# aaron-randreth/modulation-mfcc

Measured on AMD Instinct MI355X. Metric: MFCC+mod-spectrum frames/sec, higher is better.
Workload: dtype f32; 1 GPU; BASELINE configs[2] per GPU: 1024 clips x 10 s x 16000 Hz, win 400 hop 160 n_fft 512, 40 mel (fmax 8000), 13 MFCC + modulation spectrum (rFFT 1024 over trajectories); frames_per_clip=1001, clips_total=1024, parallelism=clips sharded x1, hsa_ipc_mode_legacy=0, settle_calls=712, full=False, fused_tail=True

## Files before the change

include/modmfcc.h:

```cpp
#ifndef MODMFCC_H
#define MODMFCC_H

#include <stddef.h>
#include <stdint.h>

#ifdef __cplusplus
extern "C" {
#endif

#define MM_VERSION 123

typedef enum mm_status {
  MM_OK = 0,
  MM_ERR_INVALID_ARG = -1,
  MM_ERR_UNSUPPORTED = -2,
  MM_ERR_HIP = -3,
  MM_ERR_WORKSPACE = -4,
  MM_ERR_ALLOC = -5
} mm_status;

typedef struct mm_config {
  double sr;
  int32_t n_fft;
  int32_t win_length;
  int32_t hop_length;
  int32_t n_mels;
  int32_t n_mfcc;
  double fmin;
  double fmax;
  float preemph;
  float top_db;
  float amin;
  int32_t center;
  int32_t n_mod_fft;
} mm_config;

typedef struct mm_plan mm_plan;

enum {
  MM_STAGE_LOGMEL = 0,
  MM_STAGE_DCT = 1,
  MM_STAGE_MODSPEC = 2,
  MM_STAGE_RFFT = 3,
  MM_STAGE_POWER = 4,
  MM_STAGE_CHANGE = 5,
  MM_STAGE_INIT = 6,
  MM_NUM_STAGES = 8
};

int mm_version(void);
const char* mm_strerror(int status);
const char* mm_last_hip_error(void);

int mm_config_default(mm_config* cfg);
int mm_config_validate(const mm_config* cfg);
int64_t mm_num_frames(const mm_config* cfg, int64_t n_samples);
int32_t mm_num_bins(const mm_config* cfg);
int32_t mm_mod_fft_len(const mm_config* cfg, int64_t n_frames);
int mm_build_window(const mm_config* cfg, float* out );
int mm_build_mel(const mm_config* cfg, float* out );
int mm_build_dct(const mm_config* cfg, float* out );
int mm_build_mel_sweep(const mm_config* cfg, int n_waves, float* wlo ,
                       float* whi , int32_t* d , int32_t* part );
int mm_build_mel_runs(const mm_config* cfg, int n_waves, int32_t* hdr, int32_t hdr_cap, float* grp,
                      int32_t grp_cap, int32_t* part, int32_t* counts);
int mm_build_butter_sos(int order, double wn, double* sos );

int mm_plan_create(const mm_config* cfg, mm_plan** out);
int mm_plan_destroy(mm_plan* plan);
int mm_plan_config(const mm_plan* plan, mm_config* out);
int mm_plan_kernel_path(const mm_plan* plan);
int mm_plan_fused_dct(const mm_plan* plan);
int mm_plan_set_fuse_dct(mm_plan* plan, int on);
int mm_plan_fused_tail(const mm_plan* plan, int64_t batch, int64_t n_samples);
int mm_plan_set_fuse_tail(mm_plan* plan, int on);
int mm_plan_force_generic(mm_plan* plan, int on);
int mm_plan_set_variant(mm_plan* plan, int variant);
size_t mm_workspace_bytes(const mm_plan* plan, int64_t batch, int64_t n_samples);

int mm_mfcc_f32(mm_plan* plan, const float* d_audio, int64_t batch, int64_t n_samples,
                int64_t audio_stride, float* d_mfcc, void* d_workspace, size_t ws_bytes,
                void* stream);

int mm_logmel_f32(mm_plan* plan, const float* d_audio, int64_t batch, int64_t n_samples,
                  int64_t audio_stride, float* d_logmel, float* d_clipmax, void* stream);

int mm_stft_power_f32(mm_plan* plan, const float* d_audio, int64_t batch, int64_t n_samples,
                      int64_t audio_stride, float* d_power, void* stream);

int mm_rfft_f32(mm_plan* plan, const float* d_in, int64_t rows, int64_t in_len,
                int64_t in_stride, int32_t n, float* d_out, void* stream);

int mm_modspec_f32(mm_plan* plan, const float* d_mfcc, int64_t batch, int64_t n_frames,
                   float* d_modspec, void* stream);

int mm_mfcc_modspec_f32(mm_plan* plan, const float* d_audio, int64_t batch, int64_t n_samples,
                        int64_t audio_stride, float* d_mfcc, float* d_modspec, void* d_workspace,
                        size_t workspace_bytes, void* stream);

size_t mm_ragged_workspace_bytes(const mm_plan* plan, int64_t batch, int64_t n_samples);
int mm_mfcc_ragged_f32(mm_plan* plan, const float* d_audio, int64_t batch, int64_t n_samples, int64_t audio_stride,
                       const int64_t* d_lengths, float* d_mfcc, float* d_modspec, void* d_workspace, size_t ws_bytes,
                       void* stream);

int mm_mfcc_change_f64(mm_plan* plan, const float* d_mfcc, int64_t batch, int64_t n_frames,
                       int32_t remove_first, int32_t diff_method, const double* sos1, int32_t n_sec1,
                       const double* sos2, int32_t n_sec2, double* d_change,
                       void* d_workspace, size_t ws_bytes, void* stream);
size_t mm_change_workspace_bytes(const mm_plan* plan, int64_t batch, int64_t n_frames);
size_t mm_change_workspace_bytes_for(const mm_plan* plan, int64_t batch, int64_t n_frames, int32_t remove_first,
                                     const double* sos1, int32_t n_sec1, const double* sos2, int32_t n_sec2);

size_t mm_change_ragged_workspace_bytes_for(const mm_plan* plan, int64_t batch, int64_t n_frames_max, int32_t remove_first,
                                            const double* sos1, int32_t n_sec1, const double* sos2, int32_t n_sec2);
int mm_mfcc_change_ragged_f64(mm_plan* plan, const float* d_mfcc, int64_t batch, int64_t n_frames_max,
                              const int64_t* d_frames, int32_t remove_first, int32_t diff_method,
                              const double* sos1, int32_t n_sec1, const double* sos2, int32_t n_sec2,
                              double* d_change, void* d_workspace, size_t ws_bytes, void* stream);

int mm_sosfiltfilt_f64(const double* d_x, int64_t rows, int64_t n, int64_t x_stride, const double* sos,
                       int32_t n_sec, double* d_y, void* d_workspace, size_t ws_bytes, void* stream);
size_t mm_sosfiltfilt_workspace_bytes(int64_t rows, int64_t n);
int mm_sosfiltfilt_f32_f64(const float* d_x, int64_t rows, int64_t n, int64_t x_stride, const double* sos,
                           int32_t n_sec, double* d_y, void* d_workspace, size_t ws_bytes, void* stream);

#define MM_ST_MAXW 16
#define MM_ST_MAXE 8
typedef struct mm_stencil {
  int32_t n_c, n_edge, edge_w, reserved;
  int32_t off[MM_ST_MAXW];
  double c[MM_ST_MAXW];
  double el[MM_ST_MAXE][MM_ST_MAXW];
  double er[MM_ST_MAXE][MM_ST_MAXW];
  double den_c, den_e;
} mm_stencil;
int mm_stencil_f64(const mm_stencil* st, const double* d_x, int64_t rows, int64_t n, int64_t x_stride,
                   double* d_y, void* stream);

int mm_fir_filtfilt_f64(const double* d_x, int64_t rows, int64_t n, int64_t x_stride, const double* d_h, int32_t n_taps,
                        double* d_y, int64_t y_stride, void* stream);
int mm_fir_filtfilt_f32_f64(const float* d_x, int64_t rows, int64_t n, int64_t x_stride, const double* d_h, int32_t n_taps,
                            double* d_y, int64_t y_stride, void* stream);
int mm_savgol_f64(const double* d_x, int64_t rows, int64_t n, int64_t x_stride, const double* d_c, const double* d_q,
                  const double* d_p, int32_t window, int32_t n_basis, double* d_y, int64_t y_stride, void* stream);

size_t mm_sosfiltfilt_ragged_workspace_bytes(int64_t rows, int64_t n_max);
int mm_sosfiltfilt_ragged_f64(const double* d_x, int64_t rows, int64_t n_max, int64_t x_stride, const int64_t* d_lens,
                              const double* sos, int32_t n_sec, double* d_y, void* d_workspace, size_t ws_bytes,
                              void* stream);
int mm_sosfiltfilt_ragged_f32_f64(const float* d_x, int64_t rows, int64_t n_max, int64_t x_stride, const int64_t* d_lens,
                                  const double* sos, int32_t n_sec, double* d_y, void* d_workspace, size_t ws_bytes,
                                  void* stream);
int mm_stencil_ragged_f64(const mm_stencil* st, const double* d_x, int64_t rows, int64_t n_max, int64_t x_stride,
                          const int64_t* d_lens, double* d_y, void* stream);
int mm_fir_filtfilt_ragged_f64(const double* d_x, int64_t rows, int64_t n_max, int64_t x_stride, const int64_t* d_lens,
                               const double* d_h, int32_t n_taps, double* d_y, int64_t y_stride, void* stream);
int mm_fir_filtfilt_ragged_f32_f64(const float* d_x, int64_t rows, int64_t n_max, int64_t x_stride, const int64_t* d_lens,
                                   const double* d_h, int32_t n_taps, double* d_y, int64_t y_stride, void* stream);
int mm_savgol_ragged_f64(const double* d_x, int64_t rows, int64_t n_max, int64_t x_stride, const int64_t* d_lens,
                         const double* d_c, const double* d_q, const double* d_p, int32_t window, int32_t n_basis,
                         double* d_y, int64_t y_stride, void* stream);

int64_t mm_rms_num_frames(int64_t n_samples, int32_t frame_length, int32_t hop_length, int32_t center);
int mm_rms_f32(const float* d_audio, int64_t batch, int64_t n_samples, int64_t audio_stride,
               int32_t frame_length, int32_t hop_length, int32_t center, float* d_rms, void* stream);
int mm_rms_ragged_f32(const float* d_audio, int64_t batch, int64_t n_max, int64_t audio_stride, const int64_t* d_lens,
                      int32_t frame_length, int32_t hop_length, int32_t center, float* d_rms, void* stream);

typedef struct mm_hilbert mm_hilbert;
int mm_hilbert_create(int64_t n, int32_t dtype, mm_hilbert** out);
void mm_hilbert_destroy(mm_hilbert* h);
int64_t mm_hilbert_fft_size(const mm_hilbert* h);
size_t mm_hilbert_workspace_bytes(const mm_hilbert* h, int64_t rows);
int mm_hilbert_envelope(mm_hilbert* h, const void* d_x, int64_t rows, int64_t x_stride, void* d_env,
                        int64_t env_stride, void* d_workspace, size_t ws_bytes, void* stream);
int mm_hilbert_ragged_create(int64_t n_max, int32_t dtype, mm_hilbert** out);
size_t mm_hilbert_ragged_workspace_bytes(const mm_hilbert* h, int64_t rows, int64_t n_max);
int mm_hilbert_envelope_ragged(mm_hilbert* h, const void* d_x, int64_t rows, int64_t n_max, int64_t x_stride,
                               const int64_t* d_lens, void* d_env, int64_t env_stride, void* d_workspace, size_t ws_bytes,
                               void* stream);
size_t mm_hilbert_rfft_workspace_bytes(const mm_hilbert* h, int64_t rows);
int mm_hilbert_rfft_f32(mm_hilbert* h, const float* d_x, int64_t rows, int64_t x_stride, int64_t n_valid, float* d_out,
                        void* d_ws, size_t ws_bytes, void* stream);

int mm_pcm_decode_f32(const void* d_raw, int32_t fmt, int32_t channels, int64_t n_frames, float* d_out,
                      int64_t out_stride, void* stream);
int mm_resample_f32(const float* d_x, int64_t rows, int64_t n_in, int64_t x_stride, const float* d_taps,
                    int32_t L, int32_t M, int32_t taps_per_phase, int64_t half_len, float* d_y, int64_t n_out,
                    void* stream);
int mm_resample_banded_f32(const float* d_x, int64_t rows, int64_t n_in, int64_t x_stride, const float* d_atab,
                           const int32_t* d_lo_off, int32_t F, int32_t S, int32_t NB, int32_t ksteps, int32_t lo_min,
                           int32_t win, float* d_y, int64_t n_out, void* stream);
int mm_resample_banded_shape(int32_t F, int32_t S, int32_t NB, int32_t ksteps, int32_t win, int32_t* qt, int32_t* pad,
                             size_t* lds_bytes);

typedef struct mm_wav_rec {
  int64_t byte_offset;
  int64_t n_frames;
  int32_t fmt;
  int32_t channels;
  int64_t first_row;
} mm_wav_rec;
int mm_pcm_decode_ragged_f32(const void* d_raw, int64_t raw_bytes, const mm_wav_rec* d_recs, int64_t n_files,
                             int64_t max_frames, float* d_out, int64_t out_rows, int64_t out_stride, void* stream);
int mm_resample_ragged_f32(const float* d_x, int64_t rows, int64_t n_max, int64_t x_stride, const int64_t* d_lens,
                           const float* d_taps, int32_t L, int32_t M, int32_t taps_per_phase, int64_t half_len,
                           float* d_y, int64_t n_out_max, int64_t y_stride, void* stream);
int mm_resample_banded_ragged_f32(const float* d_x, int64_t rows, int64_t n_max, int64_t x_stride, const int64_t* d_lens,
                                  const float* d_atab, const int32_t* d_lo_off, int32_t F, int32_t S, int32_t NB,
                                  int32_t ksteps, int32_t lo_min, int32_t win, float* d_y, int64_t n_out_max,
                                  int64_t y_stride, void* stream);

int mm_devcopy_f32(const float* d_src, float* d_dst, int64_t n_floats, void* stream);

typedef struct mm_pyin_params {
  double sr, fmin, fmax;
  double no_trough_prob;
  double log_tiny;
  double fill_na;
  double log_p_init[2];
  int32_t frame_length, win_length, hop_length;
  int32_t center;
  int32_t min_period, max_period, n_thresholds, nbps;
  int32_t n_bins, band_h, max_troughs, reserved;
} mm_pyin_params;

typedef struct mm_pyin_tables {
  const double* thresholds;
// ... 96 lines not shown
```

modulation_mfcc_amd/_lib.py:

```python
from __future__ import annotations

import ctypes as C
import os

_HERE = os.path.dirname(os.path.abspath(__file__))
LIB_PATH = os.environ.get("MODMFCC_LIB") or os.path.join(_HERE, "libmodmfcc.so")

MM_OK = 0
MM_ERR_INVALID_ARG = -1
MM_ERR_UNSUPPORTED = -2
MM_ERR_HIP = -3
MM_ERR_WORKSPACE = -4
MM_ERR_ALLOC = -5

STAGES = ("logmel", "dct", "modspec", "rfft", "power", "change", "init", "reserved")
MM_NUM_STAGES = 8


class mm_config(C.Structure):
    _fields_ = [
        ("sr", C.c_double),
        ("n_fft", C.c_int32),
        ("win_length", C.c_int32),
        ("hop_length", C.c_int32),
        ("n_mels", C.c_int32),
        ("n_mfcc", C.c_int32),
        ("fmin", C.c_double),
        ("fmax", C.c_double),
        ("preemph", C.c_float),
        ("top_db", C.c_float),
        ("amin", C.c_float),
        ("center", C.c_int32),
        ("n_mod_fft", C.c_int32),
    ]


MM_ST_MAXW, MM_ST_MAXE = 16, 8


class mm_stencil(C.Structure):
    _fields_ = [
        ("n_c", C.c_int32), ("n_edge", C.c_int32), ("edge_w", C.c_int32), ("reserved", C.c_int32),
        ("off", C.c_int32 * MM_ST_MAXW),
        ("c", C.c_double * MM_ST_MAXW),
        ("el", (C.c_double * MM_ST_MAXW) * MM_ST_MAXE),
        ("er", (C.c_double * MM_ST_MAXW) * MM_ST_MAXE),
        ("den_c", C.c_double), ("den_e", C.c_double),
    ]


class mm_pyin_params(C.Structure):
    _fields_ = [
        ("sr", C.c_double), ("fmin", C.c_double), ("fmax", C.c_double),
        ("no_trough_prob", C.c_double), ("log_tiny", C.c_double), ("fill_na", C.c_double),
        ("log_p_init", C.c_double * 2),
        ("frame_length", C.c_int32), ("win_length", C.c_int32), ("hop_length", C.c_int32), ("center", C.c_int32),
        ("min_period", C.c_int32), ("max_period", C.c_int32), ("n_thresholds", C.c_int32), ("nbps", C.c_int32),
        ("n_bins", C.c_int32), ("band_h", C.c_int32), ("max_troughs", C.c_int32), ("reserved", C.c_int32),
    ]


class mm_pyin_tables(C.Structure):
    _fields_ = [(k, C.c_void_p) for k in ("thresholds", "beta_probs", "beta_cum", "boltzmann", "log_same", "log_cross",
                                           "freqs")]


class mm_peaks_opts(C.Structure):
    _fields_ = [
        ("height", C.c_double * 2), ("threshold", C.c_double * 2), ("prominence", C.c_double * 2),
        ("negate", C.c_int32), ("use_height", C.c_int32), ("use_threshold", C.c_int32), ("use_prominence", C.c_int32),
    ]


class mm_peaks_ext(C.Structure):
    _fields_ = [
        ("plateau_size", C.c_double * 2), ("width", C.c_double * 2), ("rel_height", C.c_double),
        ("distance", C.c_int32), ("wlen", C.c_int32), ("use_plateau_size", C.c_int32), ("use_distance", C.c_int32),
        ("use_width", C.c_int32),
    ]


class mm_peaks_out(C.Structure):
    _fields_ = [(k, C.c_void_p) for k in ("count", "idx", "prom", "lbase", "rbase", "widths", "width_heights", "left_ips",
                                           "right_ips", "plateau_sizes", "left_edges", "right_edges")]


MM_MAX_SEC = 16
MM_RAGGED_MAX_SEC = 4


class MMError(RuntimeError):
    def __init__(self, status, what, detail=""):
        self.status = status
        super().__init__(f"{what}: {detail}" if detail else what)


_vp = C.c_void_p
_i64 = C.c_int64
_cfgp = C.POINTER(mm_config)
_pyp = C.POINTER(mm_pyin_params)
_pyt = C.POINTER(mm_pyin_tables)

PROTOTYPES = {
    "mm_version": (C.c_int, []),
    "mm_strerror": (C.c_char_p, [C.c_int]),
    "mm_last_hip_error": (C.c_char_p, []),
    "mm_config_default": (C.c_int, [_cfgp]),
    "mm_config_validate": (C.c_int, [_cfgp]),
    "mm_num_frames": (_i64, [_cfgp, _i64]),
    "mm_num_bins": (C.c_int32, [_cfgp]),
    "mm_mod_fft_len": (C.c_int32, [_cfgp, _i64]),
    "mm_build_window": (C.c_int, [_cfgp, _vp]),
    "mm_build_mel": (C.c_int, [_cfgp, _vp]),
    "mm_build_dct": (C.c_int, [_cfgp, _vp]),
    "mm_build_mel_sweep": (C.c_int, [_cfgp, C.c_int, _vp, _vp, _vp, _vp]),
    "mm_build_mel_runs": (C.c_int, [_cfgp, C.c_int, _vp, C.c_int32, _vp, C.c_int32, _vp, _vp]),
    "mm_build_butter_sos": (C.c_int, [C.c_int, C.c_double, _vp]),
    "mm_plan_create": (C.c_int, [_cfgp, C.POINTER(_vp)]),
    "mm_plan_destroy": (C.c_int, [_vp]),
    "mm_plan_config": (C.c_int, [_vp, _cfgp]),
    "mm_plan_kernel_path": (C.c_int, [_vp]),
    "mm_plan_fused_dct": (C.c_int, [_vp]),
    "mm_plan_set_fuse_dct": (C.c_int, [_vp, C.c_int]),
    "mm_plan_fused_tail": (C.c_int, [_vp, _i64, _i64]),
    "mm_plan_set_fuse_tail": (C.c_int, [_vp, C.c_int]),
    "mm_mfcc_modspec_f32": (C.c_int, [_vp, _vp, _i64, _i64, _i64, _vp, _vp, _vp, C.c_size_t, _vp]),
    "mm_plan_force_generic": (C.c_int, [_vp, C.c_int]),
    "mm_plan_set_variant": (C.c_int, [_vp, C.c_int]),
    "mm_workspace_bytes": (C.c_size_t, [_vp, _i64, _i64]),
    "mm_mfcc_f32": (C.c_int, [_vp, _vp, _i64, _i64, _i64, _vp, _vp, C.c_size_t, _vp]),
    "mm_logmel_f32": (C.c_int, [_vp, _vp, _i64, _i64, _i64, _vp, _vp, _vp]),
    "mm_stft_power_f32": (C.c_int, [_vp, _vp, _i64, _i64, _i64, _vp, _vp]),
    "mm_rfft_f32": (C.c_int, [_vp, _vp, _i64, _i64, _i64, C.c_int32, _vp, _vp]),
    "mm_modspec_f32": (C.c_int, [_vp, _vp, _i64, _i64, _vp, _vp]),
    "mm_ragged_workspace_bytes": (C.c_size_t, [_vp, _i64, _i64]),
    "mm_mfcc_ragged_f32": (C.c_int, [_vp, _vp, _i64, _i64, _i64, _vp, _vp, _vp, _vp, C.c_size_t, _vp]),
    "mm_mfcc_change_f64": (C.c_int, [_vp, _vp, _i64, _i64, C.c_int32, C.c_int32, _vp, C.c_int32, _vp,
                                     C.c_int32, _vp, _vp, C.c_size_t, _vp]),
    "mm_sosfiltfilt_f64": (C.c_int, [_vp, _i64, _i64, _i64, _vp, C.c_int32, _vp, _vp, C.c_size_t, _vp]),
    "mm_sosfiltfilt_workspace_bytes": (C.c_size_t, [_i64, _i64]),
    "mm_sosfiltfilt_f32_f64": (C.c_int, [_vp, _i64, _i64, _i64, _vp, C.c_int32, _vp, _vp, C.c_size_t, _vp]),
    "mm_stencil_f64": (C.c_int, [C.POINTER(mm_stencil), _vp, _i64, _i64, _i64, _vp, _vp]),
    "mm_fir_filtfilt_f64": (C.c_int, [_vp, _i64, _i64, _i64, _vp, C.c_int32, _vp, _i64, _vp]),
    "mm_fir_filtfilt_f32_f64": (C.c_int, [_vp, _i64, _i64, _i64, _vp, C.c_int32, _vp, _i64, _vp]),
    "mm_savgol_f64": (C.c_int, [_vp, _i64, _i64, _i64, _vp, _vp, _vp, C.c_int32, C.c_int32, _vp, _i64, _vp]),
    "mm_sosfiltfilt_ragged_workspace_bytes": (C.c_size_t, [_i64, _i64]),
    "mm_sosfiltfilt_ragged_f64": (C.c_int, [_vp, _i64, _i64, _i64, _vp, _vp, C.c_int32, _vp, _vp, C.c_size_t, _vp]),
    "mm_sosfiltfilt_ragged_f32_f64": (C.c_int, [_vp, _i64, _i64, _i64, _vp, _vp, C.c_int32, _vp, _vp, C.c_size_t, _vp]),
    "mm_stencil_ragged_f64": (C.c_int, [C.POINTER(mm_stencil), _vp, _i64, _i64, _i64, _vp, _vp, _vp]),
    "mm_fir_filtfilt_ragged_f64": (C.c_int, [_vp, _i64, _i64, _i64, _vp, _vp, C.c_int32, _vp, _i64, _vp]),
    "mm_fir_filtfilt_ragged_f32_f64": (C.c_int, [_vp, _i64, _i64, _i64, _vp, _vp, C.c_int32, _vp, _i64, _vp]),
    "mm_savgol_ragged_f64": (C.c_int, [_vp, _i64, _i64, _i64, _vp, _vp, _vp, _vp, C.c_int32, C.c_int32, _vp, _i64, _vp]),
    "mm_change_workspace_bytes": (C.c_size_t, [_vp, _i64, _i64]),
    "mm_change_workspace_bytes_for": (C.c_size_t, [_vp, _i64, _i64, C.c_int32, _vp, C.c_int32, _vp, C.c_int32]),
    "mm_change_ragged_workspace_bytes_for": (C.c_size_t, [_vp, _i64, _i64, C.c_int32, _vp, C.c_int32, _vp, C.c_int32]),
    "mm_mfcc_change_ragged_f64": (C.c_int, [_vp, _vp, _i64, _i64, _vp, C.c_int32, C.c_int32, _vp, C.c_int32, _vp,
                                            C.c_int32, _vp, _vp, C.c_size_t, _vp]),
    "mm_rms_num_frames": (_i64, [_i64, C.c_int32, C.c_int32, C.c_int32]),
    "mm_rms_f32": (C.c_int, [_vp, _i64, _i64, _i64, C.c_int32, C.c_int32, C.c_int32, _vp, _vp]),
    "mm_rms_ragged_f32": (C.c_int, [_vp, _i64, _i64, _i64, _vp, C.c_int32, C.c_int32, C.c_int32, _vp, _vp]),
    "mm_hilbert_ragged_create": (C.c_int, [_i64, C.c_int32, C.POINTER(_vp)]),
    "mm_hilbert_ragged_workspace_bytes": (C.c_size_t, [_vp, _i64, _i64]),
    "mm_hilbert_envelope_ragged": (C.c_int, [_vp, _vp, _i64, _i64, _i64, _vp, _vp, _i64, _vp, C.c_size_t, _vp]),
    "mm_hilbert_create": (C.c_int, [_i64, C.c_int32, C.POINTER(_vp)]),
    "mm_hilbert_destroy": (None, [_vp]),
    "mm_hilbert_fft_size": (_i64, [_vp]),
    "mm_hilbert_workspace_bytes": (C.c_size_t, [_vp, _i64]),
    "mm_hilbert_envelope": (C.c_int, [_vp, _vp, _i64, _i64, _vp, _i64, _vp, C.c_size_t, _vp]),
    "mm_hilbert_rfft_workspace_bytes": (C.c_size_t, [_vp, _i64]),
    "mm_hilbert_rfft_f32": (C.c_int, [_vp, _vp, _i64, _i64, _i64, _vp, _vp, C.c_size_t, _vp]),
    "mm_pcm_decode_f32": (C.c_int, [_vp, C.c_int32, C.c_int32, _i64, _vp, _i64, _vp]),
    "mm_resample_f32": (C.c_int, [_vp, _i64, _i64, _i64, _vp, C.c_int32, C.c_int32, C.c_int32, _i64, _vp, _i64, _vp]),
    "mm_resample_banded_f32": (C.c_int, [_vp, _i64, _i64, _i64, _vp, _vp, C.c_int32, C.c_int32, C.c_int32, C.c_int32, C.c_int32,
                                        C.c_int32, _vp, _i64, _vp]),
    "mm_resample_banded_shape": (C.c_int, [C.c_int32, C.c_int32, C.c_int32, C.c_int32, C.c_int32, C.POINTER(C.c_int32),
                                          C.POINTER(C.c_int32), C.POINTER(C.c_size_t)]),
    "mm_pcm_decode_ragged_f32": (C.c_int, [_vp, _i64, _vp, _i64, _i64, _vp, _i64, _i64, _vp]),
    "mm_resample_ragged_f32": (C.c_int, [_vp, _i64, _i64, _i64, _vp, _vp, C.c_int32, C.c_int32, C.c_int32, _i64, _vp, _i64,
                                        _i64, _vp]),
    "mm_resample_banded_ragged_f32": (C.c_int, [_vp, _i64, _i64, _i64, _vp, _vp, _vp, C.c_int32, C.c_int32, C.c_int32, C.c_int32,
                                               C.c_int32, C.c_int32, _vp, _i64, _i64, _vp]),
    "mm_devcopy_f32": (C.c_int, [_vp, _vp, _i64, _vp]),
    "mm_pyin_check": (C.c_int, [_pyp]),
    "mm_pyin_num_frames": (_i64, [_pyp, _i64]),
    "mm_pyin_cmnd": (C.c_int, [_pyp, _vp, C.c_int32, _i64, _i64, _i64, _vp, _vp]),
    "mm_pyin_candidates": (C.c_int, [_pyp, _pyt, _vp, _i64, _vp, _vp, _vp, _vp, _vp]),
    "mm_pyin_decode_workspace_bytes": (C.c_size_t, [_pyp, _i64, _i64]),
    "mm_pyin_decode": (C.c_int, [_pyp, _pyt, _vp, _vp, _vp, _vp, _i64, _i64, _vp, _vp, _vp, _vp, C.c_size_t, _vp]),
    "mm_pyin_workspace_bytes": (C.c_size_t, [_pyp, _i64, _i64]),
    "mm_pyin_f32": (C.c_int, [_pyp, _pyt, _vp, _i64, _i64, _i64, _vp, _vp, _vp, _vp, _vp, C.c_size_t, _vp]),
    "mm_pyin_f64": (C.c_int, [_pyp, _pyt, _vp, _i64, _i64, _i64, _vp, _vp, _vp, _vp, _vp, C.c_size_t, _vp]),
    "mm_pyin_ragged_workspace_bytes": (C.c_size_t, [_pyp, _i64, _i64]),
    "mm_pyin_ragged_f32": (C.c_int, [_pyp, _pyt, _vp, _i64, _i64, _i64, _vp, _vp, _vp, _vp, _vp, _vp, _vp, C.c_size_t, _vp]),
    "mm_pyin_ragged_f64": (C.c_int, [_pyp, _pyt, _vp, _i64, _i64, _i64, _vp, _vp, _vp, _vp, _vp, _vp, _vp, C.c_size_t, _vp]),
    "mm_interp_nan_linear_ragged_f64": (C.c_int, [_vp, _i64, _i64, _i64, _vp, _vp, _i64, _vp]),
    "mm_interp_nan_ragged_f64": (C.c_int, [C.c_int32, _vp, _i64, _i64, _i64, _vp, _vp, _i64, _vp, C.c_size_t, _vp]),
    "mm_interp_nan_linear_f64": (C.c_int, [_vp, _i64, _i64, _i64, _vp, _i64, _vp]),
    "mm_interp_nan_workspace_bytes": (C.c_size_t, [C.c_int32, _i64, _i64]),
    "mm_interp_nan_f64": (C.c_int, [C.c_int32, _vp, _i64, _i64, _i64, _vp, _i64, _vp, C.c_size_t, _vp]),
    "mm_regrid_linear_f32_f64": (C.c_int, [_vp, _i64, _i64, _i64, _vp, _vp, _i64, _vp, _i64, _vp]),
    "mm_find_peaks_workspace_bytes": (C.c_size_t, [_i64, _i64]),
    "mm_find_peaks": (C.c_int, [C.POINTER(mm_peaks_opts), _vp, C.c_int32, _i64, _i64, _i64, _vp, _vp, _i64, _vp, _vp, _vp,
                                _vp, _vp, _vp, C.c_size_t, _vp]),
    "mm_find_peaks_ex_workspace_bytes": (C.c_size_t, [C.POINTER(mm_peaks_opts), C.POINTER(mm_peaks_ext), _i64, _i64]),
    "mm_find_peaks_ex": (C.c_int, [C.POINTER(mm_peaks_opts), C.POINTER(mm_peaks_ext), _vp, C.c_int32, _i64, _i64, _i64, _vp,
                                   _vp, _i64, C.POINTER(mm_peaks_out), _vp, C.c_size_t, _vp]),
    "mm_timing_enable": (C.c_int, [_vp, C.c_int]),
    "mm_timing_read": (C.c_int, [_vp, _vp, _vp]),
}


class mm_modpsd_params(C.Structure):
    _fields_ = [
        ("fs", C.c_double),
        ("nperseg", C.c_int32), ("noverlap", C.c_int32), ("nfft", C.c_int32),
        ("detrend", C.c_int32), ("scaling", C.c_int32), ("reserved", C.c_int32 * 3),
    ]


_mpp = C.POINTER(mm_modpsd_params)

PROTOTYPES_MODPSD = {
    "mm_modpsd_version": (C.c_int, []),
    "mm_modpsd_check": (C.c_int, [_mpp]),
    "mm_modpsd_num_segments": (_i64, [_mpp, _i64]),
    "mm_modpsd_create": (C.c_int, [_mpp, _vp, C.POINTER(_vp)]),
    "mm_modpsd_destroy": (None, [_vp]),
    "mm_modpsd_workspace_bytes": (C.c_size_t, [_vp, _i64, _i64]),
    "mm_modpsd_f32": (C.c_int, [_vp, _vp, _i64, _i64, _i64, _vp, _vp, _i64, _vp, C.c_size_t, _vp]),
}

PROTOTYPES_MODCSD = {
    "mm_modcsd_version": (C.c_int, []),
    "mm_modcsd_check": (C.c_int, [_mpp]),
    "mm_modcsd_workspace_bytes": (C.c_size_t, [_vp, _i64, _i64]),
    "mm_modcsd_f32": (C.c_int, [_vp, _vp, _i64, _i64, _i64, _vp, _i64, _i64, _vp, _vp, _vp, _vp, _vp, _i64, _vp, C.c_size_t,
                                _vp]),
}

MM_SPLINE_QUADRATIC, MM_SPLINE_CUBIC = 2, 3
PROTOTYPES_SPLINE = {
    "mm_interp_spline_workspace_bytes": (C.c_size_t, [C.c_int32, _i64, _i64]),
    "mm_interp_spline_f64": (C.c_int, [C.c_int32, _vp, _i64, _i64, _i64, _vp, _i64, _vp, C.c_size_t, _vp]),
    "mm_interp_spline_ragged_f64": (C.c_int, [C.c_int32, _vp, _i64, _i64, _i64, _vp, _vp, _i64, _vp, C.c_size_t, _vp]),
}

MM_LOMB_PRECENTER, MM_LOMB_FLOATING_MEAN = 1, 2
MM_LOMB_POWER, MM_LOMB_NORMALIZE, MM_LOMB_AMPLITUDE = 0 << 2, 1 << 2, 2 << 2
MM_LOMB_CHUNK = 512
PROTOTYPES_LOMB = {
    "mm_lomb_version": (C.c_int, []),
    "mm_lombscargle_workspace_bytes": (C.c_size_t, [_i64, _i64, _i64]),
    "mm_lombscargle_f64": (C.c_int, [_vp, _i64, _i64, _i64, _vp, _vp, _vp, _i64, C.c_int32, _vp, _i64, _vp, _vp, C.c_size_t,
                                     _vp]),
}

_lib = None


def load():
    global _lib
    if _lib is not None:
        return _lib
    try:
        import torch
    except ImportError:
        pass
    if not os.path.exists(LIB_PATH):
        raise ImportError(
            f"{LIB_PATH} is missing: the HIP extension has not been built. Run "
            "`make -C modulation_mfcc_amd/csrc` (needs hipcc, --offload-arch=gfx950). "
            "modulation_mfcc_amd has no CPU fallback.")
    lib = C.CDLL(LIB_PATH)
    for table in (PROTOTYPES, PROTOTYPES_MODPSD, PROTOTYPES_MODCSD, PROTOTYPES_SPLINE, PROTOTYPES_LOMB):
        for name, (res, args) in table.items():
            fn = getattr(lib, name)
            fn.restype = res
# ... 19 lines not shown
```

modulation_mfcc_amd/csrc/mm_api.hip:

```cpp
#include <memory>
#include <utility>

#include "mm_common.h"
#include "mm_plan.h"

thread_local std::string g_hip_err;

struct StftParams {
  const float* audio;
  int64_t batch, n_samples, stride, n_frames;
  int n_fft, log2nc, hop, n_bins, n_mels;
  float preemph, amin, db_offset;
  const float* window;
  const float2* tw;
  const int* mel_start;
  const int* mel_len;
  const int* mel_off;
  const float* mel_w;
  float* out_power;
  float* out_logmel;
  int* clip_key;
  int frames_per_wave;
};

// ... 113 lines not shown
    const int64_t r = r0 + f;
    if (r >= p.rows) break;
    const float* a = p.in + r * p.in_stride;
    for (int n = lane; n < nc; n += 64) {
      const float x0 = (2 * n < p.in_len) ? a[2 * n] : 0.0f;
      const float x1 = (2 * n + 1 < p.in_len) ? a[2 * n + 1] : 0.0f;
      z[__brev((unsigned)n) >> (32 - p.log2nc)] = make_float2(x0, x1);
    }
    wave_lds_sync();
    wave_cfft_lds(z, p.log2nc, p.tw, lane);
    float2* o = reinterpret_cast<float2*>(p.out) + r * (nc + 1);
    for (int k = lane; k <= (nc >> 1); k += 64) {
      float2 xa, xb;
      real_split(z, k, nc, p.tw, tw_stride, xa, xb);
      o[k] = xa;
      o[nc - k] = xb;
    }
    wave_lds_sync();
  }
}

#include "mm_fft16.hip.inc"
#include "mm_logmel16w.hip.inc"
#include "mm_s16.h"
#include "mm_logmel12m.hip.inc"
#include "mm_logmel16h.hip.inc"
#include "mm_wpf.hip.inc"
#include "mm_hb_math.h"
#include "mm_anyfft.hip.inc"


template <class... K>
static bool raise_lds(int bytes, K... kernels) {
  for (const void* k : {(const void*)kernels...})
    if (hipFuncSetAttribute(k, hipFuncAttributeMaxDynamicSharedMemorySize, bytes) != hipSuccess) return false;
  return true;
}

using WpfKernel = void (*)(WpfParams);
template <int R, int Z>
static WpfKernel wpf_ni_kernel(int pairs) {
  return pairs == 4 ? logmel_wpf_kernel<R, 1, false, false, Z, 4> : pairs == 5 ? logmel_wpf_kernel<R, 1, false, false, Z, 5>
       : pairs == 6 ? logmel_wpf_kernel<R, 1, false, false, Z, 6> : logmel_wpf_kernel<R, 1, false, false, Z, 7>;
}
template <int R>
static WpfKernel wpf_kernel(int mode, bool pre, bool w16, bool half, int z, int pairs) {
  if constexpr (R >= 2) {
    if (w16) return logmel_wpf_kernel<R, 1, false, true>;
    if (half) return z ? wpf_ni_kernel<R, 3>(pairs) : wpf_ni_kernel<R, 0>(pairs);
    if (z) return z == 7 ? logmel_wpf_kernel<R, 1, false, false, 7> : z == 6 ? logmel_wpf_kernel<R, 1, false, false, 6>
                : z == 5 ? logmel_wpf_kernel<R, 1, false, false, 5> : logmel_wpf_kernel<R, 1, false, false, 3>;
  }
  if (mode == 0) return pre ? logmel_wpf_kernel<R, 0, true> : logmel_wpf_kernel<R, 0, false>;
  return pre ? logmel_wpf_kernel<R, 1, true> : logmel_wpf_kernel<R, 1, false>;
}

extern "C" {

int mm_version(void) { return MM_VERSION; }

const char* mm_strerror(int s) {
  switch (s) {
    case MM_OK: return "ok";
    case MM_ERR_INVALID_ARG: return "invalid argument";
    case MM_ERR_UNSUPPORTED: return "unsupported configuration";
    case MM_ERR_HIP: return "HIP runtime error";
    case MM_ERR_WORKSPACE: return "workspace too small";
    case MM_ERR_ALLOC: return "allocation failed";
    default: return "unknown status";
  }
}

const char* mm_last_hip_error(void) { return g_hip_err.c_str(); }

int mm_config_default(mm_config* c) {
  if (!c) return MM_ERR_INVALID_ARG;
  c->sr = 10000.0;
  c->n_fft = 512;
  c->win_length = 250;
  c->hop_length = 50;
  c->n_mels = 128;
  c->n_mfcc = 13;
  c->fmin = 100.0;
  c->fmax = 10000.0;
  c->preemph = 0.0f;
  c->top_db = 80.0f;
  c->amin = 1e-10f;
  c->center = 1;
  c->n_mod_fft = 0;
  return MM_OK;
}

int mm_config_validate(const mm_config* c) { return mm::validate(c); }

int64_t mm_num_frames(const mm_config* c, int64_t n_samples) {
  if (!c || c->hop_length < 1 || n_samples < 0) return MM_ERR_INVALID_ARG;
  const int64_t padded = n_samples + 2 * (int64_t)(c->n_fft / 2);
  return padded < c->n_fft ? 0 : 1 + (padded - c->n_fft) / c->hop_length;
}

int32_t mm_num_bins(const mm_config* c) { return c ? c->n_fft / 2 + 1 : MM_ERR_INVALID_ARG; }

int32_t mm_mod_fft_len(const mm_config* c, int64_t n_frames) {
  if (!c || n_frames < 1) return MM_ERR_INVALID_ARG;
  if (c->n_mod_fft) return c->n_mod_fft >= n_frames ? c->n_mod_fft : MM_ERR_INVALID_ARG;
  int64_t n = 32;
  while (n < n_frames) n *= 2;
  return n <= ((int64_t)1 << 24) ? (int32_t)n : MM_ERR_UNSUPPORTED;
}

int mm_build_window(const mm_config* c, float* out) {
  int s = mm::validate(c);
  if (s || !out) return s ? s : MM_ERR_INVALID_ARG;
  mm::build_window(*c, out);
  return MM_OK;
}
int mm_build_mel(const mm_config* c, float* out) {
  int s = mm::validate(c);
  if (s || !out) return s ? s : MM_ERR_INVALID_ARG;
  mm::build_mel(*c, out);
  return MM_OK;
}
int mm_build_dct(const mm_config* c, float* out) {
  int s = mm::validate(c);
  if (s || !out) return s ? s : MM_ERR_INVALID_ARG;
  mm::build_dct(*c, out);
  return MM_OK;
}
int mm_build_mel_sweep(const mm_config* c, int n_waves, float* wlo, float* whi, int32_t* d, int32_t* part) {
  int s = mm::validate(c);
  if (s) return s;
  if (n_waves < 1 || !wlo || !whi || !d || !part) return MM_ERR_INVALID_ARG;
  std::vector<float> mel((size_t)c->n_mels * (c->n_fft / 2 + 1));
  mm::build_mel(*c, mel.data());
  mm::MelSweep sw;
  if (!mm::build_mel_sweep(*c, mel.data(), n_waves, &sw)) return MM_ERR_UNSUPPORTED;
  std::memcpy(wlo, sw.wlo.data(), sw.wlo.size() * 4);
  std::memcpy(whi, sw.whi.data(), sw.whi.size() * 4);
  std::memcpy(d, sw.d.data(), sw.d.size() * 4);
  std::memcpy(part, sw.part.data(), sw.part.size() * 4);
  return MM_OK;
}
int mm_build_mel_runs(const mm_config* c, int n_waves, int32_t* hdr, int32_t hdr_cap, float* grp,
                      int32_t grp_cap, int32_t* part, int32_t* counts) {
  int s = mm::validate(c);
  if (s) return s;
  if (n_waves < 1 || !hdr || !grp || !part || !counts) return MM_ERR_INVALID_ARG;
  std::vector<float> mel((size_t)c->n_mels * (c->n_fft / 2 + 1));
  mm::build_mel(*c, mel.data());
  mm::MelSweep sw;
  if (!mm::build_mel_sweep(*c, mel.data(), n_waves, &sw)) return MM_ERR_UNSUPPORTED;
  mm::MelRuns r;
  mm::build_mel_runs(*c, sw, n_waves, &r);
  counts[0] = (int32_t)(r.hdr.size() / 4);
  counts[1] = (int32_t)(r.grp.size() / 8);
  if (counts[0] > hdr_cap || counts[1] > grp_cap) return MM_ERR_WORKSPACE;
  std::memcpy(hdr, r.hdr.data(), r.hdr.size() * 4);
  std::memcpy(grp, r.grp.data(), r.grp.size() * 4);
  std::memcpy(part, r.part.data(), r.part.size() * 4);
  return MM_OK;
}
int mm_build_butter_sos(int order, double wn, double* sos) { return mm::build_butter_sos(order, wn, sos); }


static std::vector<float> packed_run_table(const mm::MelRuns& r) {
  std::vector<float> tab(r.hdr.size() + r.grp.size());
  std::memcpy(tab.data(), r.hdr.data(), r.hdr.size() * 4);
  std::memcpy(tab.data() + r.hdr.size(), r.grp.data(), r.grp.size() * 4);
  for (size_t g = 0; g < r.grp.size() / 8; ++g) {
    float* q = tab.data() + r.hdr.size() + 8 * g;
    const float t[8] = {q[0], q[4], q[1], q[5], q[2], q[6], q[3], q[7]};
    std::memcpy(q, t, sizeof t);
  }
  return tab;
}

static std::vector<int> balance_parts_over_simds(const mm::MelRuns& r, const double* extra = nullptr,
                                                 std::vector<int>* wave_of_part = nullptr) {
  const int n = (int)(r.part.size() / 4);
  std::vector<int> out(r.part.size());
  if (wave_of_part) { wave_of_part->assign(n, 0); for (int w = 0; w < n; ++w) (*wave_of_part)[w] = w; }
  if (n != 16) return r.part;
  std::vector<std::pair<double, int>> cost(n);
  for (int w = 0; w < n; ++w) {
    double c = extra ? extra[w] : 0.0;
    for (int i = r.part[w * 4 + 0]; i < r.part[w * 4 + 1]; ++i) c += 58.0 + 8.5 * r.hdr[4 * i + 1];
    cost[w] = {c, w};
  }
  std::sort(cost.begin(), cost.end(), [](const std::pair<double, int>& a, const std::pair<double, int>& b) {
    return a.first > b.first || (a.first == b.first && a.second < b.second); });
  double load[4] = {0, 0, 0, 0};
  int cnt[4] = {0, 0, 0, 0};
  for (int i = 0; i < n; ++i) {
    int best = -1;
    for (int sd = 0; sd < 4; ++sd)
      if (cnt[sd] < 4 && (best < 0 || load[sd] < load[best])) best = sd;
    const int wave = best + 4 * cnt[best];
    std::memcpy(&out[wave * 4], &r.part[cost[i].second * 4], 16);
    if (wave_of_part) (*wave_of_part)[cost[i].second] = wave;
    load[best] += cost[i].first; ++cnt[best];
  }
  return out;
}

static std::vector<float> wpf_lane_table(int R, const float* win, const float* tw) {
  const int L = 16 * R, NC = 256 * R;
  std::vector<float> lt((size_t)L * MM_WPF_LT_PITCH, 0.0f);
  for (int l = 0; l < L; ++l) {
    float* r = lt.data() + l * MM_WPF_LT_PITCH;
    const int pq = l % R;
    if (win)
      for (int n1 = 0; n1 < 16; ++n1) { r[2 * n1] = win[2 * L * n1 + 2 * l]; r[2 * n1 + 1] = win[2 * L * n1 + 2 * l + 1]; }
    for (int k1 = 1; k1 < 16; ++k1) {
      const int i1 = ((l * k1) % NC) * (MM_TW_N / NC);
      r[32 + 2 * (k1 - 1)] = tw[2 * i1]; r[32 + 2 * (k1 - 1) + 1] = tw[2 * i1 + 1];
      const int i2 = ((pq * k1) % L) * (MM_TW_N / L);
      r[64 + 2 * (k1 - 1)] = tw[2 * i2]; r[64 + 2 * (k1 - 1) + 1] = tw[2 * i2 + 1];
    }
    for (int i = 0; i < 8; ++i) {
      const int idx = (l + L * i) * (MM_TW_N / (2 * NC));
      r[96 + 2 * i] = 0.5f * tw[2 * idx + 1]; r[96 + 2 * i + 1] = -0.5f * tw[2 * idx];
    }
  }
  return lt;
}

static std::vector<float> w16_lane_table(const float* win, const float* tw) {
  std::vector<float> lt(16 * MM_W16_LT_PITCH, 0.0f);
  for (int q = 0; q < 16; ++q) {
    float* r = lt.data() + q * MM_W16_LT_PITCH;
    for (int n1 = 0; n1 < 16; ++n1) { r[2 * n1] = win[32 * n1 + 2 * q]; r[2 * n1 + 1] = win[32 * n1 + 2 * q + 1]; }
    for (int k1 = 1; k1 < 16; ++k1) {
      const int idx = (q * k1) * (MM_TW_N / 256);
      r[32 + 2 * (k1 - 1)] = tw[2 * idx]; r[32 + 2 * (k1 - 1) + 1] = tw[2 * idx + 1];
    }
    for (int j = 0; j < 8; ++j) {
      const int idx = (q + 16 * j) * (MM_TW_N / 512);
      r[64 + 2 * j] = 0.5f * tw[2 * idx + 1]; r[64 + 2 * j + 1] = -0.5f * tw[2 * idx];
    }
  }
  return lt;
}

static int zero_edges(const float* win, int n) {
  int e = 0;
  while (e < n / 2 && win[e] == 0.0f && win[n - 1 - e] == 0.0f) ++e;
  return e;
}

struct EmptyFilters { std::vector<char> empty; bool skip = false; int nk = 0; };
static EmptyFilters empty_filters(const mm_config& c, const float* mel) {
  EmptyFilters e;
  e.empty.assign(c.n_mels, 1);
  int n_empty = 0;
  for (int m = 0; m < c.n_mels; ++m) {
    for (int k = 0; k < 257 && e.empty[m]; ++k) if (mel[(size_t)m * 257 + k] != 0.0f) e.empty[m] = 0;
    n_empty += e.empty[m];
  }
  e.skip = n_empty > 0 && n_empty < c.n_mels;
  int last = c.n_mels - 1;
  while (e.skip && last > 0 && e.empty[last]) --last;
  e.nk = e.skip ? last / 4 + 1 : ((c.n_mels + 3) & ~3) / 4;
  return e;
}

static std::vector<float> dct_a_operands(const mm_config& c, const float* dct, int nk, const char* skip = nullptr) {
  const int kbn = (c.n_mfcc + 15) / 16;
  std::vector<float> a((size_t)kbn * nk * 64, 0.0f);
  for (int kb = 0; kb < kbn; ++kb)
    for (int s = 0; s < nk; ++s)
      for (int l = 0; l < 64; ++l) {
        const int k = 16 * kb + (l & 15), m = 4 * s + (l >> 4);
        if (k < c.n_mfcc && m < c.n_mels && !(skip && skip[m])) a[((size_t)kb * nk + s) * 64 + l] = dct[(size_t)k * c.n_mels + m];
      }
  return a;
}

static bool wpf_mel_lanes(const mm::MelSweep& sw, int R, int SL, std::vector<float>* out, int* group_max) {
  const int L = 16 * R, NC = 256 * R;
  std::vector<float>& ml = *out;
  ml.assign((size_t)L * 36, 0.0f);
  std::vector<int> d_end(L, -2);
  bool ok = true;
  for (int l = 0; l < L && ok; ++l) {
    float* r = ml.data() + l * 36;
    int dprev = sw.d[SL * l];
    const int dstart = dprev;
    unsigned bits = 0;
    const int nslots = SL == 8 ? 8 : ((l == L - 1) ? 17 : 16);
    for (int i = 0; i < nslots; ++i) {
      const int k = (i < SL) ? SL * l + i : NC;
      const int adv = sw.d[k] - dprev;
      if (adv < 0 || adv > 1) { ok = false; break; }
      if (adv == 1) bits |= (1u << i);
      dprev = sw.d[k];
      r[i] = sw.wlo[k];
      r[17 + i] = sw.whi[k];
    }
    std::memcpy(&r[34], &dstart, 4);
    std::memcpy(&r[35], &bits, 4);
    d_end[l] = dprev;
  }
  std::vector<char> act(L, 0);
  for (int l = 0; l < L; ++l) {
    const float* r = ml.data() + (size_t)l * 36;
    unsigned bits;
// ... 34 lines not shown
  PlanHost(const mm_config& c, int n_bins, int kp)
      : win(c.n_fft), mel((size_t)c.n_mels * n_bins), dct((size_t)c.n_mfcc * c.n_mels),
        dct_t((size_t)c.n_mels * kp, 0.0f), tw(2 * MM_TW_N), cfg_e(c), ce(&c), melp(mel.data()), winp(win.data()) {
    mm::build_window(c, win.data()); mm::build_mel(c, mel.data());
    mm::build_dct(c, dct.data()); mm::build_twiddles(MM_TW_N, tw.data());
    for (int k = 0; k < c.n_mfcc; ++k)
      for (int m = 0; m < c.n_mels; ++m) dct_t[(size_t)m * kp + k] = dct[(size_t)k * c.n_mels + m];
    mm::build_mel_csr(c, mel.data(), &csr);
  }
  PlanHost(const PlanHost&) = delete;
};

static int setup_base(mm_plan* p, const PlanHost& h) {
  mm_plan::Base& b = p->base;
  int rc = MM_OK;
  if ((rc = p->upload(&b.d_window, h.win.data(), h.win.size() * 4)) ||
      (rc = p->upload(&b.d_tw, h.tw.data(), h.tw.size() * 4)) ||
      (rc = p->upload(&b.d_mel_start, h.csr.start.data(), h.csr.start.size() * 4)) ||
      (rc = p->upload(&b.d_mel_len, h.csr.len.data(), h.csr.len.size() * 4)) ||
      (rc = p->upload(&b.d_mel_off, h.csr.off.data(), h.csr.off.size() * 4)) ||
      (rc = p->upload(&b.d_mel_w, h.csr.w.data(), h.csr.w.size() * 4)) ||
      (rc = p->upload(&b.d_dct_t, h.dct_t.data(), h.dct_t.size() * 4)))
    return rc;
  hipDeviceProp_t prop;
  if (hipGetDeviceProperties(&prop, p->device) == hipSuccess && prop.multiProcessorCount > 0)
    p->num_cus = prop.multiProcessorCount;
  return MM_OK;
}

static int setup_any(mm_plan* p, const PlanHost& h) {
  AnyPlan& ap = p->any;
  std::vector<float> atw, asplit, achirp, abhat;
  if (!any_plan_host(p->cfg.n_fft, &ap, &atw, &asplit, &achirp, &abhat, MM_LM_LDS_MAX)) return MM_ERR_UNSUPPORTED;
  int rc = MM_OK;
  if ((rc = p->upload(&ap.d_tw, atw.data(), std::max<size_t>(atw.size(), 2) * 4)) ||
      (!asplit.empty() && (rc = p->upload(&ap.d_split, asplit.data(), asplit.size() * 4))) ||
      (!achirp.empty() && (rc = p->upload(&ap.d_chirp, achirp.data(), achirp.size() * 4))) ||
      (!abhat.empty() && (rc = p->upload(&ap.d_bhat, abhat.data(), abhat.size() * 4))))
    return rc;
  std::vector<float> pack(h.win.begin(), h.win.end());
  auto put = [&](const void* src, size_t n_floats) {
    const int off = (int)pack.size();
    pack.resize(pack.size() + ((n_floats + 3) & ~(size_t)3), 0.0f);
    if (n_floats) std::memcpy(pack.data() + off, src, n_floats * 4);
    return off;
  };
  ap.o_tw = put(atw.data(), atw.size());
  ap.o_split = put(asplit.data(), asplit.size());
  ap.o_chirp = put(achirp.data(), achirp.size());
  ap.o_melw = put(h.csr.w.data(), h.csr.w.size());
  ap.o_mstart = put(h.csr.start.data(), h.csr.start.size());
  ap.o_mlen = put(h.csr.len.data(), h.csr.len.size());
  ap.o_moff = put(h.csr.off.data(), h.csr.off.size());
  ap.tab_floats = (int)pack.size();
  const size_t G = 256 / ap.tpf, budget = ap.tpf == 64 ? 65536 : MM_LM_LDS_MAX;
  ap.lds_tab = ap.M == 0 && G * ap.grp_bytes + pack.size() * 4 <= budget;
  int r1 = 0, r2 = 0;
  if (ap.packed && ap.M == 0 && reg2_pick(ap.nn, &r1, &r2) && reg2_lds_bytes(r1, r2, ap.tab_floats) <= 80 * 1024 &&
      reg2_set_attr(r1, r2, MM_LM_LDS_MAX)) { ap.reg2 = r1; ap.reg2_r2 = r2; }
  if ((ap.lds_tab || ap.reg2) && (rc = p->upload(&ap.d_tabpack, pack.data(), pack.size() * 4))) return rc;
  if (ap.lds_tab && ap.tpf == 64 && ap.packed && ap.M == 0 && ap.nn <= 256) {
    const int fb = 2;
    const size_t per_wave = (size_t)2 * fb * ap.nn * 8;
    if ((size_t)fb * (ap.nn + 2) * 4 <= (size_t)fb * ap.nn * 8 && 4 * per_wave + pack.size() * 4 <= 80 * 1024) {
      ap.fb = fb; ap.fb_grp_bytes = (unsigned)per_wave;
    }
  }
  if (!raise_lds(MM_LM_LDS_MAX, stft_any_kernel<0, 64, false>, stft_any_kernel<1, 64, false>, stft_any_kernel<0, 256, false>,
                 stft_any_kernel<1, 256, false>, stft_any_kernel<0, 64, true>, stft_any_kernel<1, 64, true>,
                 stft_any_kernel<0, 256, true>, stft_any_kernel<1, 256, true>)) {
    g_hip_err = "hipFuncSetAttribute(stft_any_kernel) failed";
    return MM_ERR_HIP;
  }
  if (!raise_lds(MM_LM_LDS_MAX, stft_anyb_kernel<0>, stft_anyb_kernel<1>)) ap.fb = 0;
  ap.ok = true;
  return MM_OK;
}

static void setup_embed(mm_plan* p, PlanHost& h) {
  const mm_config& c = p->cfg;
  if (c.n_fft != 256 && c.n_fft != 128 && c.n_fft != 64) return;
  const int E = 512 / c.n_fft;
  h.cfg_e.n_fft = 512;
  h.win_e.resize(512);
  mm::build_window(h.cfg_e, h.win_e.data());
  h.mel_e.assign((size_t)c.n_mels * 257, 0.0f);
  for (int m = 0; m < c.n_mels; ++m)
    for (int k = 0; k < p->n_bins; ++k) h.mel_e[(size_t)m * 257 + (size_t)E * k] = h.mel[(size_t)m * p->n_bins + k];
  if (p->upload(&p->embed.d_window, h.win_e.data(), h.win_e.size() * 4) == MM_OK) {
    h.ce = &h.cfg_e; h.melp = h.mel_e.data(); h.winp = h.win_e.data(); p->embed.factor = E;
  }
}

static void setup_s16f(mm_plan* p, const PlanHost& h, size_t tab16_bytes) {
  const mm_config& c = *h.ce;
  const EmptyFilters ef = empty_filters(c, h.melp);
  const int lt_rows = (c.n_mels + 3) & ~3, kbn = (c.n_mfcc + 15) / 16, nk = ef.nk;
  std::vector<float> dcta = dct_a_operands(c, h.dct.data(), nk, ef.skip ? ef.empty.data() : nullptr);
  const size_t e_off = dcta.size();
  dcta.resize(e_off + (size_t)kbn * 16 + 8, 0.0f);
  if (ef.skip) {
    for (int k = 0; k < c.n_mfcc; ++k) {
      double e = 0.0;
      for (int m = 0; m < c.n_mels; ++m) if (ef.empty[m]) e += (double)h.dct[(size_t)k * c.n_mels + m];
      dcta[e_off + k] = (float)e;
    }
    unsigned bits[8] = {0};
    for (int m = 0; m < c.n_mels; ++m) if (ef.empty[m]) bits[m >> 5] |= 1u << (m & 31);
    std::memcpy(&dcta[e_off + (size_t)kbn * 16], bits, sizeof(bits));
  }
  for (int layout = 0; layout < 4; ++layout) {
    const bool single = layout >= 2;
    const bool xa = p->s16.xa && (layout & 1) == 0;
    if ((layout & 1) && !p->s16.xa) continue;
    const double wts_d[16] = {1, 1, 1, MM_S16F_W, 1, 1, 1, MM_S16F_W, 1, 1, 1, MM_S16F_W, 1, 1, 1, MM_S16F_W};
    double extra[16];
    for (int w = 0; w < 16; ++w) extra[w] = (!single && wts_d[w] < 1.0) ? 700.0 : 0.0;
    mm::MelSweep swf;
    if (!mm::build_mel_sweep(c, h.melp, 16, &swf, single ? nullptr : wts_d)) return;
    mm::MelRuns rf;
    mm::build_mel_runs(c, swf, 16, &rf);
    if (ef.skip)
      for (size_t r = 0; r < rf.hdr.size() / 4; ++r) {
        const int d = rf.hdr[4 * r + 3];
        if (d >= 0 && d < c.n_mels && ef.empty[d]) rf.hdr[4 * r + 0] |= 1 << 16;
      }
    const std::vector<float> tab = packed_run_table(rf);
    std::vector<int> wave_of_part;
    const std::vector<int> part = balance_parts_over_simds(rf, extra, &wave_of_part);
    unsigned long long roles = ~0ull;
    for (int f = 0; f < 4; ++f) {
      const int w = single ? f : wave_of_part[4 * f + 3];
      roles = (roles & ~(0xFull << (4 * w))) | ((unsigned long long)f << (4 * w));
    }
    const size_t tab_end = (size_t)MM_S16_TAB_OFF(p->s16.nr, xa) + tab.size() * 4;
    const unsigned lt_off = (unsigned)align_up(tab_end, 16);
    const unsigned dcta_off = lt_off + (single ? 1u : 2u) * (unsigned)lt_rows * 320u;
    const unsigned red_off = (unsigned)align_up((size_t)dcta_off + dcta.size() * 4, 16);
    const size_t lds = (size_t)red_off + 2 * 16 * 8;
    if (lds > MM_LM_LDS_MAX) continue;
    mm_plan::S16F& f = p->s16f;
    f.ok = p->upload(&f.d_tab, tab.data(), tab.size() * 4) == MM_OK &&
           p->upload(&f.d_part, part.data(), part.size() * 4) == MM_OK &&
           p->upload(&f.d_dcta, dcta.data(), dcta.size() * 4) == MM_OK;
    if (!f.ok) return;
    f.n_runs = (int)(rf.hdr.size() / 4); f.n_tab16 = (int)(tab.size() / 4);
    f.lt_rows = lt_rows; f.nk = nk; f.kb = kbn; f.roles = roles;
    f.flags = (single ? MM_S16F_SINGLE : 0) | (ef.skip ? MM_S16F_SKIP : 0);
    f.lt_off = lt_off; f.dcta_off = dcta_off; f.red_off = red_off; f.lds_bytes = lds;
    if (!xa && p->s16.xa) {
      p->s16.xa = false;
      p->s16.lds_bytes = (size_t)MM_S16_TAB_OFF(p->s16.nr, false) + tab16_bytes;
    }
    return;
  }
}

static void setup_m12(mm_plan* p, const PlanHost& h) {
  const mm_config& c = p->cfg;
  mm_plan::M12& m = p->m12;
  M12Tables mt;
  const int s_floats = (47 * c.hop_length + 512 + 255) & ~255;
  const int nr = (s_floats / 256 + 15) / 16;
  if (nr > 3 || !build_m12_tables(*h.ce, h.melp, h.dct.data(), &mt)) return;
  m.nb = mt.nb; m.nr = nr; m.s_floats = s_floats;
  m.fused_dct = c.n_mfcc <= 16;
  if (mt.a_tab.empty()) mt.a_tab.assign(128, 0.0f);
  m.win_off = (unsigned)(MM_M12_S_OFF + (size_t)s_floats * 4);
  m.tw_off = m.win_off + 2048u;
  m.a_off = m.tw_off + 16u * MM_M12_TW_PITCH * 4u;
  m.n_a2 = (int)(mt.a_tab.size() / 2);
  m.dct_off = m.a_off + (unsigned)align_up(mt.a_tab.size() * 4, 16);
  m.part_off = m.dct_off + (unsigned)mt.nb * 1024u;
  m.cnt_off = m.part_off + (m.fused_dct ? (unsigned)mt.n_slots * 1024u : 0u);
  m.lds_bytes = (size_t)m.cnt_off + 16;
  const std::vector<float> zeros(64, 0.0f);
  if (m.lds_bytes <= MM_LM_LDS_MAX &&
      p->upload(&m.d_a, mt.a_tab.data(), mt.a_tab.size() * 4) == MM_OK &&
      p->upload(&m.d_dct, mt.dct_tab.data(), mt.dct_tab.size() * 4) == MM_OK &&
      p->upload(&m.d_zeros, zeros.data(), zeros.size() * 4) == MM_OK &&
      set_m12_attr(MM_LM_LDS_MAX)) {
    std::memcpy(m.units, mt.units.data(), sizeof(m.units));
    std::memcpy(m.n_units, mt.n_units.data(), sizeof(m.n_units));
    m.ok = true;
  }
}

static int setup_tile512(mm_plan* p, const PlanHost& h) {
  const mm_config& c = *h.ce;
  if (c.n_fft != 512) return MM_OK;
  p->s16.halfwin = zero_edges(h.winp, 512) >= 128;
  mm::MelSweep sw;
  if (!mm::build_mel_sweep(c, h.melp, 8, &sw)) return MM_OK;
  mm::MelRuns runs;
  mm::build_mel_runs(c, sw, 8, &runs);
  const std::vector<float> tab = packed_run_table(runs);
  mm_plan::W8& w8 = p->w8;
  w8.n_runs = (int)(runs.hdr.size() / 4); w8.n_tab16 = (int)(tab.size() / 4);
  w8.lds_bytes = (size_t)MM_LM_TAB_OFF + tab.size() * 4;
  if (w8.lds_bytes <= MM_LM_LDS_MAX) {
    int rc = MM_OK;
    if ((rc = p->upload(&w8.d_tab, tab.data(), tab.size() * 4)) || (rc = p->upload(&w8.d_part, runs.part.data(), runs.part.size() * 4)))
      return rc;
    w8.ok = raise_lds(MM_LM_LDS_MAX, logmel512_kernel<0>, logmel512_kernel<1>);
  }
  mm::MelSweep sw16;
  if (!w8.ok || !mm::build_mel_sweep(c, h.melp, 16, &sw16)) return MM_OK;
  mm::MelRuns r16;
  mm::build_mel_runs(c, sw16, 16, &r16);
  const std::vector<float> tab16 = packed_run_table(r16);
  const size_t tab16_bytes = tab16.size() * 4;
  mm_plan::W16& w16 = p->w16;
  w16.n_runs = (int)(r16.hdr.size() / 4); w16.n_tab16 = (int)(tab16.size() / 4);
  w16.lds_bytes = (size_t)MM_W16_TAB_OFF + tab16_bytes;
  const std::vector<float> lt = w16_lane_table(h.winp, h.tw.data());
  w16.ok = w16.lds_bytes <= MM_LM_LDS_MAX && p->upload(&w16.d_tab, tab16.data(), tab16_bytes) == MM_OK &&
           p->upload(&w16.d_lane_tab, lt.data(), lt.size() * 4) == MM_OK &&
           p->upload(&w16.d_part, balance_parts_over_simds(r16).data(), r16.part.size() * 4) == MM_OK &&
           raise_lds(MM_LM_LDS_MAX, logmel512w_kernel<0>, logmel512w_kernel<1>);
  if (w16.ok && 31 * c.hop_length + 512 + 256 <= MM_H16_NR * 2048 && (c.hop_length % 2) == 0 && c.preemph == 0.0f) {
    mm_plan::H16& h16 = p->h16;
    H16Tables ht;
    build_h16_tables(r16, &ht);
    h16.n_pairs = ht.n_pairs; h16.n_tab16 = (int)(ht.tab.size() / 4);
    h16.lds_bytes = (size_t)MM_H16_TAB_OFF + ht.tab.size() * 4;
    h16.ok = h16.lds_bytes <= 80 * 1024 && p->upload(&h16.d_tab, ht.tab.data(), ht.tab.size() * 4) == MM_OK &&
             p->upload(&h16.d_part, ht.part.data(), ht.part.size() * 4) == MM_OK && raise_lds(80 * 1024, logmel512h_kernel);
  }
  if (w16.ok) {
    const int span = 63 * c.hop_length + 512;
    int nr = span <= 4096 ? 1 : span <= 2 * 4096 ? 2 : span <= 3 * 4096 ? 3 : (span <= 4 * 4096 ? 4 : 0);
    if (nr && nr < 3 && c.preemph != 0.0f) nr = 3;
    const bool xa = nr >= 3 && (size_t)MM_S16_TAB_OFF(nr, true) + tab16_bytes <= MM_LM_LDS_MAX;
    const size_t lds = nr ? (size_t)MM_S16_TAB_OFF(nr, xa) + tab16_bytes : 0;
    if (nr && lds <= MM_LM_LDS_MAX && set_s16_attr(MM_LM_LDS_MAX)) { p->s16.nr = nr; p->s16.xa = xa; p->s16.lds_bytes = lds; }
  }
  if (p->s16.nr && c.n_mels <= 256) setup_s16f(p, h, tab16_bytes);
  if (p->w16.ok) setup_m12(p, h);
  return MM_OK;
}

static void setup_wpf(mm_plan* p, const PlanHost& h) {
  const mm_config& c = p->cfg;
  if ((c.n_fft != 512 && c.n_fft != 1024 && c.n_fft != 2048) || c.n_mels > MM_WPF_MAXMEL) return;
  const int R = c.n_fft / 512, L = 16 * R, NC = 256 * R;
  mm::MelSweep sw;
  if (!mm::build_mel_sweep(c, h.mel.data(), 1, &sw)) return;
  mm_plan::Wpf& w = p->wpf;
  int k_hi = 0;
  for (int m = 0; m < c.n_mels; ++m)
    for (int k = p->n_bins - 1; k > k_hi; --k)
      if (h.mel[(size_t)m * p->n_bins + k] != 0.0f) { k_hi = k; break; }
  w.half = R >= 2 && k_hi < NC / 2 && c.preemph == 0.0f;
  w.pairs = w.half ? std::max(4, k_hi / L + 1) : 8;
  if (w.pairs > 7) w.half = false;
  std::vector<float> ml;
  bool ok = wpf_mel_lanes(sw, R, w.half ? 8 : 16, &ml, &w.group_max);
  if (!ok && w.half) {
    w.half = false; w.pairs = 8;
    ok = wpf_mel_lanes(sw, R, 16, &ml, &w.group_max);
  }
  const int macc_stride = (c.n_mels + 2 + 63) / 64 * 64;
  const int F = 4 / R;
  const int xbuf = (R == 1) ? 1280 : 1152;
  const int pbuf = F * (NC + NC / 16 + 4);
  const size_t wave_bytes = (size_t)(xbuf + pbuf + F * 3 * macc_stride) * 4;
  w.r = R;
  if (w.half) {
    const size_t wb = (size_t)(xbuf + MM_WPF_PBUF_HALF + F * 3 * macc_stride) * 4;
    int wv = 16;
    while (wv > 4 && (size_t)L * MM_WPF_LT_PITCH * 4 + wv * wb > MM_LM_LDS_MAX) wv -= 4;
    w.waves_half = wv; w.lds_half = (size_t)L * MM_WPF_LT_PITCH * 4 + wv * wb;
  }
  w.waves = 12;
  while (w.waves > 4 && (size_t)L * MM_WPF_LT_PITCH * 4 + w.waves * wave_bytes > MM_LM_LDS_MAX) w.waves -= 4;
  w.lds_bytes = (size_t)L * MM_WPF_LT_PITCH * 4 + w.waves * wave_bytes;
  w.lds16 = (size_t)L * (MM_WPF_LT_PITCH + MM_WPF_ML_PITCH) * 4 + 16 * (size_t)(xbuf + F * 3 * macc_stride) * 4;
  w.w16 = R >= 2 && w.lds16 <= MM_LM_LDS_MAX &&
          raise_lds(MM_LM_LDS_MAX, logmel_wpf_kernel<2, 1, false, true>, logmel_wpf_kernel<4, 1, false, true>);
  bool attr_ok = w.lds_bytes <= MM_LM_LDS_MAX &&
                 raise_lds(MM_LM_LDS_MAX, logmel_wpf_kernel<1, 0, false>, logmel_wpf_kernel<1, 1, false>,
                           logmel_wpf_kernel<2, 0, false>, logmel_wpf_kernel<2, 1, false>, logmel_wpf_kernel<4, 0, false>,
                           logmel_wpf_kernel<4, 1, false>, logmel_wpf_kernel<1, 0, true>, logmel_wpf_kernel<1, 1, true>,
                           logmel_wpf_kernel<2, 0, true>, logmel_wpf_kernel<2, 1, true>, logmel_wpf_kernel<4, 0, true>,
                           logmel_wpf_kernel<4, 1, true>);
  if (w.half &&
      !raise_lds(MM_LM_LDS_MAX, wpf_ni_kernel<4, 0>(4), wpf_ni_kernel<4, 0>(5), wpf_ni_kernel<4, 0>(6), wpf_ni_kernel<4, 0>(7),
                 wpf_ni_kernel<4, 3>(4), wpf_ni_kernel<4, 3>(5), wpf_ni_kernel<4, 3>(6), wpf_ni_kernel<4, 3>(7),
                 wpf_ni_kernel<2, 0>(4), wpf_ni_kernel<2, 0>(5), wpf_ni_kernel<2, 0>(6), wpf_ni_kernel<2, 0>(7),
                 wpf_ni_kernel<2, 3>(4), wpf_ni_kernel<2, 3>(5), wpf_ni_kernel<2, 3>(6), wpf_ni_kernel<2, 3>(7)))
    attr_ok = false;
  if (R >= 2) {
    const int zmax = std::min(7, zero_edges(h.win.data(), c.n_fft) / (2 * L));
    const int zsel = zmax >= 7 ? 7 : zmax >= 6 ? 6 : zmax >= 5 ? 5 : zmax >= 3 ? 3 : 0;
    if (zsel > 0 &&
        raise_lds(MM_LM_LDS_MAX, logmel_wpf_kernel<2, 1, false, false, 3>, logmel_wpf_kernel<4, 1, false, false, 3>,
                  logmel_wpf_kernel<2, 1, false, false, 5>, logmel_wpf_kernel<4, 1, false, false, 5>, logmel_wpf_kernel<2, 1, false, false, 6>,
                  logmel_wpf_kernel<4, 1, false, false, 6>, logmel_wpf_kernel<2, 1, false, false, 7>, logmel_wpf_kernel<4, 1, false, false, 7>))
      w.z = zsel;
  }
  const std::vector<float> lt = wpf_lane_table(R, h.win.data(), h.tw.data());
  w.ok = ok && attr_ok && p->upload(&w.d_lane_tab, lt.data(), lt.size() * 4) == MM_OK &&
         p->upload(&w.d_mel_lane, ml.data(), ml.size() * 4) == MM_OK &&
         set_dct_fm_attr(64 * (MM_WPF_MAXMEL + 1) * 4);
  if (!w.ok) return;
  const int nk = (c.n_mels + 3) / 4, kbn = (c.n_mfcc + 15) / 16;
  if (c.n_mels > 128) return;
  mm_plan::DctFm& f = p->dctfm;
  const std::vector<float> da = dct_a_operands(c, h.dct.data(), nk);
  const int ch = ((nk + 9) / 10 * 10 <= (nk + 7) / 8 * 8) ? 10 : 8, nkp = (nk + ch - 1) / ch * ch;
  std::vector<float> dw((size_t)kbn * nkp * 64, 0.0f);
  for (int kb = 0; kb < kbn; ++kb)
    std::memcpy(&dw[(size_t)kb * nkp * 64], &da[(size_t)kb * nk * 64], (size_t)nk * 64 * 4);
  const size_t ldsw = ((size_t)kbn * nkp * 64 + 4 * 16 * (size_t)((4 * nkp) | 1)) * 4;
  if (ldsw <= 65536 && p->upload(&f.d_wave_a, dw.data(), dw.size() * 4) == MM_OK) { f.kb = kbn; f.wave_nk = nkp; f.ch = ch; }
}

static int setup_rfft(mm_plan* p, const PlanHost& h) {
  if (!raise_lds(MM_LM_LDS_MAX, rfft_generic_kernel)) {
    g_hip_err = "hipFuncSetAttribute(rfft_generic_kernel) failed";
    return MM_ERR_HIP;
  }
  const std::vector<float> lt = wpf_lane_table(4, nullptr, h.tw.data());
  p->rf2k.ok = p->upload(&p->rf2k.d_lane_tab, lt.data(), lt.size() * 4) == MM_OK &&
               raise_lds(MM_LM_LDS_MAX, rfft_wpf_kernel<4, true>, rfft_wpf_kernel<4, false>);
  return MM_OK;
}

int mm_plan_create(const mm_config* cfg, mm_plan** out) {
  if (!out) return MM_ERR_INVALID_ARG;
  *out = nullptr;
  int s = mm::validate(cfg);
  if (s) return s;
  std::unique_ptr<mm_plan> p(new (std::nothrow) mm_plan());
  if (!p) return MM_ERR_ALLOC;
  p->cfg = *cfg;
  p->n_bins = cfg->n_fft / 2 + 1;
  p->log2nc = nfft_is_pow2_class(cfg->n_fft) ? ilog2(cfg->n_fft) - 1 : 0;
  p->kp = (cfg->n_mfcc + MM_DCT_KB - 1) / MM_DCT_KB * MM_DCT_KB;
  p->db_offset = 10.0f * log10f(fmaxf(cfg->amin, 1.0f));
  if (hipGetDevice(&p->device) != hipSuccess) {
    g_hip_err = "hipGetDevice failed (no GPU?)";
    return MM_ERR_HIP;
  }
  PlanHost h(*cfg, p->n_bins, p->kp);
  int rc = MM_OK;
  if ((rc = setup_base(p.get(), h))) return rc;
  if (!nfft_is_pow2_class(cfg->n_fft) && (rc = setup_any(p.get(), h))) return rc;
  setup_embed(p.get(), h);
  if ((rc = setup_tile512(p.get(), h))) return rc;
  setup_wpf(p.get(), h);
  if ((rc = setup_rfft(p.get(), h))) return rc;
  *out = p.release();
  return MM_OK;
}

int mm_plan_destroy(mm_plan* p) {
  if (!p) return MM_OK;
  for (hipEvent_t e : p->timing.ev_pool) (void)hipEventDestroy(e);
  delete p;
  return MM_OK;
}

int mm_plan_config(const mm_plan* p, mm_config* out) {
  if (!p || !out) return MM_ERR_INVALID_ARG;
  *out = p->cfg;
  return MM_OK;
}

enum { MM_K_GENERIC = 0, MM_K_W8 = 1, MM_K_W16 = 2, MM_K_WPF = 3, MM_K_W16S = 4, MM_K_M12 = 5, MM_K_ANY = 6, MM_K_H16 = 7 };
static int choose_kernel(const mm_plan* p, int mode, bool call, const float* d_audio, int64_t n_samples, int64_t stride) {
  if (p->any.ok) return MM_K_ANY;
  if (p->user.force_generic) return MM_K_GENERIC;
  const int v = p->user.variant;
  const bool force_wpf = v == MM_K_WPF;
  const bool n4 = !call || n_samples >= 4, n2 = !call || n_samples >= 2;
  if (v == MM_K_H16 && p->h16.ok && mode == 1 &&
      (!call || (n_samples >= 4 && (n_samples % 4) == 0 && (stride % 4) == 0 && (((uintptr_t)d_audio) & 15) == 0)))
    return MM_K_H16;
  const bool m12_ok = p->m12.ok && mode == 1 && n4 && v == MM_K_M12;
  const bool staged_ok = p->s16.nr && p->w16.ok && n4 && v != MM_K_W16 && v != MM_K_W8;
  const bool direct_ok = (!call || ((stride % 2) == 0 && (((uintptr_t)d_audio) & 7) == 0)) && n2 &&
                         p->cfg.preemph == 0.0f && (p->cfg.hop_length % 2) == 0;
  const bool tile_ok = p->w8.ok && (direct_ok || staged_ok || m12_ok) && (p->embed.factor == 1 || mode != 0);
  if (p->wpf.ok && (p->cfg.n_fft != 512 || force_wpf || !tile_ok) && n2) return MM_K_WPF;
  if (!tile_ok) return MM_K_GENERIC;
  if (m12_ok) return MM_K_M12;
  if (p->w16.ok && v != MM_K_W8) return staged_ok ? MM_K_W16S : MM_K_W16;
  return direct_ok ? MM_K_W8 : MM_K_GENERIC;
}

static bool s16_clip_mode_ok(const mm_plan* p, int64_t batch, int n_mod) {
  if (p->user.no_fuse_tail ||
      !(n_mod == 512 || n_mod == 1024 || (p->user.fuse_tail_wide && (n_mod == 0 || (n_mod == 2048 && p->rf2k.ok)))))
    return false;
  const int64_t g = p->num_cus;
  if (batch < g) return false;
  const int64_t per = (batch + g - 1) / g;
  if (per > MM_S16_CPW_MAX) return false;
  if ((size_t)p->s16f.red_off + (size_t)per * 128 > MM_LM_LDS_MAX) return false;
  if ((size_t)MM_S16_DELTA_OFF((size_t)p->s16f.red_off, (size_t)per, n_mod) + (size_t)per * 4 > MM_LM_LDS_MAX) return false;
  return per * g * 100 <= batch * 104;
}

enum Want { WANT_ROWS, WANT_MFCC, WANT_MFCC_CLIP, WANT_MODSPEC };

struct CallShape {
  bool call = false; const float* audio = nullptr;
  int64_t n_samples = 0, stride = 0, batch = 0; int n_mod = 0;
};

struct Dispatch {
  int kernel = MM_K_GENERIC;
  bool fused_dct = false;
  bool clip = false;
};

static Dispatch dispatch(const mm_plan* p, int mode, const CallShape& c, Want want) {
  Dispatch d;
  d.kernel = choose_kernel(p, mode, c.call, c.audio, c.n_samples, c.stride);
  d.fused_dct = mode == 1 && want != WANT_ROWS && !p->user.no_fuse &&
                ((d.kernel == MM_K_M12 && p->m12.fused_dct) || (d.kernel == MM_K_W16S && p->s16f.ok));
  d.clip = d.fused_dct && d.kernel == MM_K_W16S && (want == WANT_MFCC_CLIP || want == WANT_MODSPEC) &&
           s16_clip_mode_ok(p, c.batch, want == WANT_MODSPEC ? c.n_mod : 0);
  return d;
}

int mm_plan_kernel_path(const mm_plan* p) {
  if (!p) return MM_ERR_INVALID_ARG;
  return dispatch(p, 1, CallShape(), WANT_ROWS).kernel;
}

int mm_plan_fused_dct(const mm_plan* p) {
  if (!p) return MM_ERR_INVALID_ARG;
  return dispatch(p, 1, CallShape(), WANT_MFCC).fused_dct ? 1 : 0;
}

int mm_plan_set_fuse_dct(mm_plan* p, int on) {
  if (!p) return MM_ERR_INVALID_ARG;
  const int prev = !p->user.no_fuse;
  p->user.no_fuse = on ? 0 : 1;
  return prev;
}

int mm_plan_set_fuse_tail(mm_plan* p, int on) {
  if (!p) return MM_ERR_INVALID_ARG;
  const int prev = p->user.no_fuse_tail ? 0 : (p->user.fuse_tail_wide ? 2 : 1);
  p->user.no_fuse_tail = on ? 0 : 1;
  p->user.fuse_tail_wide = on == 2 ? 1 : 0;
  return prev;
}

int mm_plan_set_variant(mm_plan* p, int variant) {
  if (!p || variant < 0 || variant > MM_K_H16 || variant == MM_K_ANY) return MM_ERR_INVALID_ARG;
  const int prev = p->user.variant;
  p->user.variant = variant;
  return prev;
}

int mm_plan_force_generic(mm_plan* p, int on) {
  if (!p) return MM_ERR_INVALID_ARG;
  int prev = p->user.force_generic;
  p->user.force_generic = on ? 1 : 0;
  return prev;
}

size_t mm_workspace_bytes(const mm_plan* p, int64_t batch, int64_t n_samples) {
  if (!p || batch < 1 || n_samples < 0) return 0;
  const int64_t T = mm_num_frames(&p->cfg, n_samples);
  return align_up((size_t)batch * p->cfg.n_mels * T * 4, 256) + align_up((size_t)batch * 8, 256);
}

struct StftOut {
  float* power = nullptr;
  float* logmel = nullptr;
  int* key_max = nullptr;
  int* key_nmin = nullptr;
  float* mfcc = nullptr;
  float* mod = nullptr;
  bool frame_major = false;
};


static int launch_any(const mm_plan* p, int mode, const CallShape& c, const StftOut& o, hipStream_t st) {
  const AnyPlan& ap = p->any;
  AnyParams q;
  q.audio = c.audio; q.batch = c.batch; q.n_samples = c.n_samples; q.stride = c.stride;
  q.n_frames = mm_num_frames(&p->cfg, c.n_samples);
  q.n_fft = p->cfg.n_fft; q.hop = p->cfg.hop_length; q.n_bins = p->n_bins; q.n_mels = p->cfg.n_mels;
  q.preemph = p->cfg.preemph; q.amin = p->cfg.amin; q.db_offset = p->db_offset; q.window = p->base.d_window;
  q.nn = ap.nn; q.packed = ap.packed; q.n_pass = ap.n_pass; std::memcpy(q.radix, ap.radix, sizeof(q.radix));
  q.M = ap.M; q.log2M = ap.log2M; q.tw = ap.d_tw; q.split = ap.d_split; q.chirp = ap.d_chirp; q.bhat = ap.d_bhat;
  q.mel_start = p->base.d_mel_start; q.mel_len = p->base.d_mel_len; q.mel_off = p->base.d_mel_off; q.mel_w = p->base.d_mel_w;
  q.out_power = o.power; q.out_logmel = o.logmel; q.clip_key = o.key_max;
  q.frames_per_group = ap.lds_tab ? 16 : 4; q.grp_bytes = ap.grp_bytes; q.b_off = ap.b_off; q.p_off = ap.p_off;
  q.tabpack = ap.d_tabpack; q.tab_floats = ap.tab_floats; q.o_tw = ap.o_tw; q.o_split = ap.o_split; q.o_chirp = ap.o_chirp;
  q.o_melw = ap.o_melw; q.o_mstart = ap.o_mstart; q.o_mlen = ap.o_mlen; q.o_moff = ap.o_moff;
  const int variant = p->user.variant;
  if (ap.reg2 && variant == 0) {
    q.frames_per_group = reg2_frames_per_wave(ap.reg2);
    const int fpbb = 4 * q.frames_per_group;
    const int64_t gridb = c.batch * ((q.n_frames + fpbb - 1) / fpbb);
    if (gridb > 0x7FFFFFFF) return MM_ERR_INVALID_ARG;
    reg2_launch(ap.reg2, ap.reg2_r2, mode, dim3((unsigned)gridb), reg2_lds_bytes(ap.reg2, ap.reg2_r2, ap.tab_floats), st, q);
    return MM_OK;
  }
  const int fb = variant == 1 ? 0 : (variant >= 2 && variant <= 4 && ap.fb ? variant : ap.fb);
  if (fb > 0) {
    q.frames_per_group = 16 / fb * fb;
    q.grp_bytes = (unsigned)((size_t)2 * fb * ap.nn * 8);
    const int fpbb = 4 * q.frames_per_group;
    const int64_t gridb = c.batch * ((q.n_frames + fpbb - 1) / fpbb);
    if (gridb > 0x7FFFFFFF) return MM_ERR_INVALID_ARG;
    const size_t ldsb = (size_t)4 * q.grp_bytes + (size_t)ap.tab_floats * 4;
    hipLaunchKernelGGL(mode == 0 ? stft_anyb_kernel<0> : stft_anyb_kernel<1>, dim3((unsigned)gridb), dim3(256), ldsb, st, q, fb);
    return MM_OK;
  }
  const int G = 256 / ap.tpf, fpb = G * q.frames_per_group;
  const int64_t grid = c.batch * ((q.n_frames + fpb - 1) / fpb);
  if (grid > 0x7FFFFFFF) return MM_ERR_INVALID_ARG;
  const size_t lds = (size_t)G * ap.grp_bytes + (ap.lds_tab ? (size_t)ap.tab_floats * 4 : 0);
  const auto k = ap.lds_tab ? (ap.tpf == 64 ? (mode == 0 ? stft_any_kernel<0, 64, true> : stft_any_kernel<1, 64, true>)
                                            : (mode == 0 ? stft_any_kernel<0, 256, true> : stft_any_kernel<1, 256, true>))
                            : (ap.tpf == 64 ? (mode == 0 ? stft_any_kernel<0, 64, false> : stft_any_kernel<1, 64, false>)
                                            : (mode == 0 ? stft_any_kernel<0, 256, false> : stft_any_kernel<1, 256, false>));
  hipLaunchKernelGGL(k, dim3((unsigned)grid), dim3(256), lds, st, q);
  return MM_OK;
}

static int launch_h16(const mm_plan* p, const CallShape& c, const StftOut& o, hipStream_t st) {
  Logmel512hParams q;
  q.audio = c.audio; q.batch = c.batch; q.n_samples = c.n_samples; q.stride = c.stride;
  q.n_frames = mm_num_frames(&p->cfg, c.n_samples);
  q.tiles_per_clip = (q.n_frames + 31) / 32;
  q.n_tiles = c.batch * q.tiles_per_clip;
  q.hop = p->cfg.hop_length; q.n_mels = p->cfg.n_mels; q.amin = p->cfg.amin; q.db_offset = p->db_offset;
  q.lane_tab = p->w16.d_lane_tab; q.pair_tab = (const float4*)p->h16.d_tab; q.n_pairs = p->h16.n_pairs; q.n_tab16 = p->h16.n_tab16;
  q.wave_part = p->h16.d_part; q.out_logmel = o.logmel; q.clip_key = o.key_max; q.key_nmin = o.key_nmin;
  if (q.n_tiles > 0x7FFFFFFF) return MM_ERR_INVALID_ARG;
  const int64_t grid = std::min<int64_t>(q.n_tiles, 2 * (int64_t)p->num_cus);
  hipLaunchKernelGGL(logmel512h_kernel, dim3((unsigned)grid), dim3(512), p->h16.lds_bytes, st, q);
  return MM_OK;
}

static int launch_wpf(const mm_plan* p, int mode, const CallShape& c, const StftOut& o, hipStream_t st) {
  const mm_plan::Wpf& w = p->wpf;
  WpfParams q;
  const int R = w.r, F = 4 / R;
  q.audio = c.audio; q.batch = c.batch; q.n_samples = c.n_samples; q.stride = c.stride;
  q.n_frames = mm_num_frames(&p->cfg, c.n_samples);
  q.groups_per_clip = (q.n_frames + F - 1) / F;
  q.total_groups = c.batch * q.groups_per_clip;
  q.hop = p->cfg.hop_length; q.n_mels = p->cfg.n_mels; q.amin = p->cfg.amin; q.db_offset = p->db_offset;
  const bool pre = p->cfg.preemph != 0.0f;
#ifdef MM_WPF_W16_DEFAULT
  const bool w16 = w.w16 && mode == 1 && !pre && p->user.variant != MM_K_WPF;
#else
  const bool w16 = false;
#endif
  const bool half = mode == 1 && w.half && !w16;
  const int z = (half || (mode == 1 && !pre)) ? w.z : 0;
  q.macc_stride = (p->cfg.n_mels + 2 + 63) / 64 * 64; q.waves_per_wg = w16 ? 16 : (half ? w.waves_half : w.waves);
  q.lane_tab = w.d_lane_tab; q.mel_lane = w.d_mel_lane; q.group_max = w.group_max;
  q.out_logmel = o.logmel; q.clip_key = o.key_max; q.out_power = o.power;
  if (o.frame_major) { q.sB = q.n_frames * q.n_mels; q.sT = q.n_mels; q.sM = 1; }
  else { q.sB = q.n_frames * q.n_mels; q.sT = 1; q.sM = q.n_frames; }
  q.preemph = p->cfg.preemph;
  int64_t grid = (q.total_groups + q.waves_per_wg - 1) / q.waves_per_wg;
  if (grid > p->num_cus) grid = p->num_cus;
  const WpfKernel k = R == 1 ? wpf_kernel<1>(mode, pre, w16, half, z, w.pairs)
                    : R == 2 ? wpf_kernel<2>(mode, pre, w16, half, z, w.pairs) : wpf_kernel<4>(mode, pre, w16, half, z, w.pairs);
  hipLaunchKernelGGL(k, dim3((unsigned)grid), dim3(64 * q.waves_per_wg), w16 ? w.lds16 : (half ? w.lds_half : w.lds_bytes), st, q);
  return MM_OK;
}

static bool unaligned_rows(const CallShape& c) { return c.stride % 4 || c.n_samples % 4 || ((uintptr_t)c.audio & 15); }

static int launch_m12(const mm_plan* p, const Dispatch& d, const CallShape& c, const StftOut& o, hipStream_t st) {
  const mm_plan::M12& m = p->m12;
  Logmel12mParams q;
  q.audio = c.audio; q.batch = c.batch; q.n_samples = c.n_samples; q.stride = c.stride;
  q.n_frames = mm_num_frames(&p->cfg, c.n_samples);
  q.tiles_per_clip = (q.n_frames + MM_M12_TF - 1) / MM_M12_TF;
  q.n_tiles = c.batch * q.tiles_per_clip;
  q.hop = p->cfg.hop_length; q.n_mels = p->cfg.n_mels; q.n_mfcc = p->cfg.n_mfcc; q.nb = m.nb;
  q.amin = p->cfg.amin; q.db_offset = p->db_offset; q.preemph = p->cfg.preemph;
  q.lane_tab = p->w16.d_lane_tab; q.a_tab = (const float2*)m.d_a; q.n_a2 = m.n_a2;
  q.window = p->embed.factor > 1 ? p->embed.d_window : p->base.d_window;
  q.dct_tab = m.d_dct;
  std::memcpy(q.units, m.units, sizeof(q.units));
  std::memcpy(q.n_units, m.n_units, sizeof(q.n_units));
  q.out_logmel = (d.fused_dct && p->cfg.top_db < 0.0f) ? nullptr : o.logmel;
  q.out_mfcc = d.fused_dct ? o.mfcc : nullptr;
  q.key_max = o.key_max; q.key_nmin = o.key_nmin;
  q.s_floats = m.s_floats; q.zeros = m.d_zeros;
  q.win_off = m.win_off; q.tw_off = m.tw_off; q.a_off = m.a_off; q.dct_off = m.dct_off; q.part_off = m.part_off; q.cnt_off = m.cnt_off;
  if (q.n_tiles > 0x7FFFFFFF) return MM_ERR_INVALID_ARG;
  const int64_t grid = q.n_tiles < p->num_cus ? q.n_tiles : p->num_cus;
  launch_m12(m.nr, p->cfg.preemph != 0.0f, p->cfg.hop_length & 1, unaligned_rows(c), dim3((unsigned)grid), m.lds_bytes, st, q);
  return MM_OK;
}

static int launch_tile512(const mm_plan* p, int mode, const Dispatch& d, const CallShape& c, const StftOut& o, hipStream_t st) {
  Logmel512Params q{};
  q.audio = c.audio; q.batch = c.batch; q.n_samples = c.n_samples; q.stride = c.stride;
  q.n_frames = mm_num_frames(&p->cfg, c.n_samples);
  q.tiles_per_clip = (q.n_frames + 63) / 64;
  q.n_tiles = c.batch * q.tiles_per_clip;
  q.hop = p->cfg.hop_length; q.n_mels = p->cfg.n_mels; q.amin = p->cfg.amin; q.db_offset = p->db_offset;
  q.window = p->embed.factor > 1 ? p->embed.d_window : p->base.d_window; q.tw = p->base.d_tw;
  q.mel_tab = (const float4*)p->w8.d_tab; q.n_runs = p->w8.n_runs; q.n_tab16 = p->w8.n_tab16;
  q.wave_part = p->w8.d_part; q.out_logmel = o.logmel; q.clip_key = o.key_max;
  q.out_power = o.power; q.dct_roles = ~0ull; q.top_db = -1.0f;
  q.dct_flags = p->s16.halfwin ? MM_S16F_HALFWIN : 0;
  q.lane_tab = p->w16.d_lane_tab;
  q.preemph = p->cfg.preemph;
  if (q.n_tiles > 0x7FFFFFFF) return MM_ERR_INVALID_ARG;
  int64_t grid = q.n_tiles < p->num_cus ? q.n_tiles : p->num_cus;
  if (d.kernel == MM_K_W8) {
    hipLaunchKernelGGL(mode == 0 ? logmel512_kernel<0> : logmel512_kernel<1>, dim3((unsigned)grid), dim3(512), p->w8.lds_bytes, st, q);
    return MM_OK;
  }
  q.mel_tab = (const float4*)p->w16.d_tab; q.n_runs = p->w16.n_runs; q.n_tab16 = p->w16.n_tab16;
  q.wave_part = p->w16.d_part;
  if (d.kernel == MM_K_W16) {
    hipLaunchKernelGGL(mode == 0 ? logmel512w_kernel<0> : logmel512w_kernel<1>, dim3((unsigned)grid), dim3(1024), p->w16.lds_bytes, st, q);
    return MM_OK;
  }
  size_t lds = p->s16.lds_bytes;
  if (d.fused_dct) {
    const mm_plan::S16F& f = p->s16f;
    q.mel_tab = (const float4*)f.d_tab; q.n_runs = f.n_runs; q.n_tab16 = f.n_tab16;
    q.wave_part = f.d_part;
    q.out_mfcc = o.mfcc; q.key_nmin = o.key_nmin; q.dct_a = f.d_dcta; q.n_mfcc = p->cfg.n_mfcc;
    q.dct_nk = f.nk; q.dct_kb = f.kb; q.lt_rows = f.lt_rows;
    q.lt_off = f.lt_off; q.dcta_off = f.dcta_off; q.dct_roles = f.roles;
    q.dct_flags = f.flags | (p->s16.halfwin ? MM_S16F_HALFWIN : 0);
    q.lt_b2 = (f.flags & MM_S16F_SINGLE) ? 0 : f.lt_rows;
    if (p->cfg.top_db < 0.0f) q.out_logmel = nullptr;
    lds = f.lds_bytes;
    q.red_off = f.red_off;
    if (d.clip) {
      q.out_mod = (float2*)o.mod; q.n_mod = o.mod ? c.n_mod : 0; q.dct_t = p->base.d_dct_t; q.dct_kp = p->kp; q.top_db = p->cfg.top_db;
      grid = c.batch < p->num_cus ? c.batch : p->num_cus;
      const size_t per = (size_t)((c.batch + grid - 1) / grid);
      lds = std::max((size_t)f.red_off + per * 128, (size_t)MM_S16_FIN_TAB_OFF + MM_S16_FIN_TAB_BYTES);
      lds = std::max(lds, (size_t)MM_S16_DELTA_OFF((size_t)f.red_off, per, q.n_mod) + per * 4);
      if (q.n_mod == 2048) {
        q.tw = (const float2*)p->rf2k.d_lane_tab;
        lds = std::max(lds, (size_t)MM_S16_FIN2K_BYTES);
      }
      mode = 2;
    }
  }
  launch_s16(mode, p->s16.nr, p->s16.xa, p->cfg.preemph != 0.0f, p->cfg.hop_length & 1, unaligned_rows(c),
             dim3((unsigned)grid), lds, st, q);
  return MM_OK;
}

static int launch_generic(const mm_plan* p, int mode, const CallShape& c, const StftOut& o, hipStream_t st) {
  StftParams q;
  q.audio = c.audio; q.batch = c.batch; q.n_samples = c.n_samples; q.stride = c.stride;
  q.n_frames = mm_num_frames(&p->cfg, c.n_samples);
  q.n_fft = p->cfg.n_fft; q.log2nc = p->log2nc; q.hop = p->cfg.hop_length; q.n_bins = p->n_bins;
  q.n_mels = p->cfg.n_mels; q.preemph = p->cfg.preemph; q.amin = p->cfg.amin; q.db_offset = p->db_offset;
  q.window = p->base.d_window; q.tw = p->base.d_tw; q.mel_start = p->base.d_mel_start; q.mel_len = p->base.d_mel_len;
  q.mel_off = p->base.d_mel_off; q.mel_w = p->base.d_mel_w; q.out_power = o.power; q.out_logmel = o.logmel;
  q.clip_key = o.key_max; q.frames_per_wave = 4;
  const int nc = 1 << p->log2nc;
  const size_t wave_bytes = ((size_t)nc * 8 + (size_t)(nc + 1) * 4 + 15) & ~(size_t)15;
  const int fpb = 4 * q.frames_per_wave;
  const int64_t tiles = (q.n_frames + fpb - 1) / fpb;
  const int64_t grid = c.batch * tiles;
  if (grid > 0x7FFFFFFF) return MM_ERR_INVALID_ARG;
  hipLaunchKernelGGL(mode == 0 ? stft_generic_kernel<0> : stft_generic_kernel<1>, dim3((unsigned)grid), dim3(256), 4 * wave_bytes, st, q);
  return MM_OK;
}

static int launch_stft(const mm_plan* p, int mode, const Dispatch& d, const CallShape& c, const StftOut& o, hipStream_t st) {
  const int rc = d.kernel == MM_K_ANY ? launch_any(p, mode, c, o, st) : d.kernel == MM_K_H16 ? launch_h16(p, c, o, st)
                 : d.kernel == MM_K_WPF ? launch_wpf(p, mode, c, o, st) : d.kernel == MM_K_M12 ? launch_m12(p, d, c, o, st)
                 : d.kernel == MM_K_GENERIC ? launch_generic(p, mode, c, o, st)
                 : launch_tile512(p, mode, d, c, o, st);
  if (rc) return rc;
  HIP_TRY(hipGetLastError());
  return MM_OK;
}

static int check_audio_args(mm_plan* p, const float* d_audio, int64_t batch, int64_t n_samples,
                            int64_t stride) {
  if (!p || !d_audio || batch < 1 || n_samples < 1 || stride < n_samples) return MM_ERR_INVALID_ARG;
  if (n_samples > MM_MAX_SAMPLES) return MM_ERR_INVALID_ARG;
  return MM_OK;
}

int mm_stft_power_f32(mm_plan* p, const float* d_audio, int64_t batch, int64_t n_samples,
                      int64_t stride, float* d_power, void* stream) {
  int rc = check_audio_args(p, d_audio, batch, n_samples, stride);
  if (rc || !d_power) return rc ? rc : MM_ERR_INVALID_ARG;
  hipStream_t st = (hipStream_t)stream;
  StageTimer tm(p, MM_STAGE_POWER, st);
  const CallShape c{true, d_audio, n_samples, stride, batch, 0};
  StftOut o;
  o.power = d_power;
  return launch_stft(p, 0, dispatch(p, 0, c, WANT_ROWS), c, o, st);
}

int mm_logmel_f32(mm_plan* p, const float* d_audio, int64_t batch, int64_t n_samples, int64_t stride,
                  float* d_logmel, float* d_clipmax, void* stream) {
  int rc = check_audio_args(p, d_audio, batch, n_samples, stride);
  if (rc || !d_logmel || !d_clipmax) return rc ? rc : MM_ERR_INVALID_ARG;
  hipStream_t st = (hipStream_t)stream;
  fill_words(d_clipmax, MM_KEY_UNSET, batch, st);
  {
    StageTimer tm(p, MM_STAGE_LOGMEL, st);
    const CallShape c{true, d_audio, n_samples, stride, batch, 0};
    StftOut o;
    o.logmel = d_logmel; o.key_max = (int*)d_clipmax;
    rc = launch_stft(p, 1, dispatch(p, 1, c, WANT_ROWS), c, o, st);
    if (rc) return rc;
  }
  hipLaunchKernelGGL(decode_keys_kernel, dim3((unsigned)((batch + 255) / 256)), dim3(256), 0, st,
                     (int*)d_clipmax, batch);
  HIP_TRY(hipGetLastError());
  return MM_OK;
}

int mm_mfcc_f32(mm_plan* p, const float* d_audio, int64_t batch, int64_t n_samples, int64_t stride,
                float* d_mfcc, void* d_ws, size_t ws_bytes, void* stream) {
  int rc = check_audio_args(p, d_audio, batch, n_samples, stride);
  if (rc || !d_mfcc || !d_ws) return rc ? rc : MM_ERR_INVALID_ARG;
  if (ws_bytes < mm_workspace_bytes(p, batch, n_samples)) return MM_ERR_WORKSPACE;
  hipStream_t st = (hipStream_t)stream;
  const int64_t T = mm_num_frames(&p->cfg, n_samples);
  float* logmel = (float*)d_ws;
  int* keys = (int*)((char*)d_ws + align_up((size_t)batch * p->cfg.n_mels * T * 4, 256));
  const bool clamp = p->cfg.top_db >= 0.0f;
  const CallShape c{true, d_audio, n_samples, stride, batch, 0};
  const Dispatch d = dispatch(p, 1, c, clamp && (p->s16f.flags & MM_S16F_SKIP) ? WANT_MFCC_CLIP : WANT_MFCC);
  StftOut o;
  o.logmel = logmel; o.key_max = keys; o.key_nmin = keys + batch; o.mfcc = d_mfcc; o.frame_major = true;
  if (d.clip) {
    StageTimer tm(p, MM_STAGE_LOGMEL, st);
    return launch_stft(p, 1, d, c, o, st);
  }
  {
    StageTimer tm(p, MM_STAGE_INIT, st);
    fill_words(keys, MM_KEY_UNSET, 2 * batch, st);
  }
  {
    StageTimer tm(p, MM_STAGE_LOGMEL, st);
    rc = launch_stft(p, 1, d, c, o, st);
    if (rc) return rc;
  }
  if (d.fused_dct && !clamp) return MM_OK;
  const bool is_fm = d.kernel == MM_K_WPF;
  {
    StageTimer tm(p, MM_STAGE_DCT, st);
    if (d.fused_dct) {
      const int64_t bpc = (T + 255) / 256;
      if (batch * bpc > 0x7FFFFFFF) return MM_ERR_INVALID_ARG;
      const bool skip_empty = d.kernel == MM_K_W16S && (p->s16f.flags & MM_S16F_SKIP);
      hipLaunchKernelGGL(dct_fixup_kernel, dim3((unsigned)(batch * bpc)), dim3(256), 0, st, logmel, keys, keys + batch,
                         p->base.d_dct_t, d_mfcc, T, p->cfg.n_mels, p->cfg.n_mfcc, p->kp, p->cfg.top_db,
                         skip_empty ? p->s16f.d_dcta + (size_t)p->s16f.kb * p->s16f.nk * 64 : nullptr,
                         p->cfg.amin, p->db_offset);
    } else if (is_fm && p->dctfm.d_wave_a && !p->user.no_fuse) {
      const int64_t n_items = batch * ((T + 15) / 16);
      const int pitch = (4 * p->dctfm.wave_nk) | 1;
      const size_t lds = ((size_t)p->dctfm.kb * p->dctfm.wave_nk * 64 + 4 * 16 * (size_t)pitch) * 4;
      const int64_t per_cu = std::max<int64_t>(1, std::min<int64_t>(8, 163840 / (int64_t)lds));
      const int64_t grid = std::min<int64_t>((n_items + 3) / 4, per_cu * p->num_cus);
      const auto k = p->dctfm.ch != 10 ? dct_clamp_fm_wave_kernel<8, 8, true>
                   : ((p->cfg.n_mels & 3) == 0 && 16 * p->cfg.n_mels <= 5 * 256) ? dct_clamp_fm_wave_kernel<10, 5, false>
                   : dct_clamp_fm_wave_kernel<10, 8, true>;
      hipLaunchKernelGGL(k, dim3((unsigned)grid), dim3(256), lds, st, logmel, keys, p->dctfm.d_wave_a, d_mfcc, T, n_items,
                         p->cfg.n_mels, p->cfg.n_mfcc, p->dctfm.wave_nk, p->dctfm.kb, p->cfg.top_db);
    } else if (is_fm) {
      const int64_t bpc = (T + 63) / 64;
      if (batch * bpc > 0x7FFFFFFF) return MM_ERR_INVALID_ARG;
      launch_dct_fm(dim3((unsigned)(batch * bpc)), (size_t)64 * (p->cfg.n_mels + 1) * 4, st, logmel, keys, p->base.d_dct_t,
                    d_mfcc, T, p->cfg.n_mels, p->cfg.n_mfcc, p->kp, p->cfg.top_db);
    } else {
      const int64_t bpc = (T + 255) / 256;
      if (batch * bpc > 0x7FFFFFFF) return MM_ERR_INVALID_ARG;
      hipLaunchKernelGGL(dct_clamp_kernel, dim3((unsigned)(batch * bpc)), dim3(256), 0, st, logmel, keys,
                         p->base.d_dct_t, d_mfcc, T, p->cfg.n_mels, p->cfg.n_mfcc, p->kp, p->cfg.top_db);
    }
    HIP_TRY(hipGetLastError());
  }
  return MM_OK;
}

static int launch_rfft(mm_plan* p, const float* d_in, int64_t rows, int64_t in_len, int64_t in_stride,
                       int n, float* d_out, hipStream_t st) {
  if (n > 8192) return MM_ERR_UNSUPPORTED;
  RfftParams q;
  q.in = d_in; q.rows = rows; q.in_len = in_len; q.in_stride = in_stride; q.n = n;
  q.log2nc = ilog2(n) - 1; q.rows_per_wave = 4; q.tw = p->base.d_tw; q.out = d_out;
  if (!p->user.force_generic && (n == 512 || n == 1024)) {
    const int rows_per_wave = (n == 512) ? 4 : 2;
    const int64_t groups = (rows + rows_per_wave - 1) / rows_per_wave;
    int64_t grid = (groups + 3) / 4;
    if (grid > 2048) grid = 2048;
    const bool fast = (in_len == n) && (in_stride % 2 == 0) && (((uintptr_t)d_in & 7) == 0);
    const auto k = n == 512 ? (fast ? rfft16_kernel<1, true> : rfft16_kernel<1, false>)
                            : (fast ? rfft16_kernel<2, true> : rfft16_kernel<2, false>);
    hipLaunchKernelGGL(k, dim3((unsigned)grid), dim3(256), 0, st, q);
// ... 102 lines not shown
```

modulation_mfcc_amd/csrc/mm_internal.h:

```cpp
#ifndef MM_INTERNAL_H
#define MM_INTERNAL_H

#include <vector>

#include "../../include/modmfcc.h"

namespace mm {

struct MelCsr {
  std::vector<int> start, len, off;
  std::vector<float> w;
};

struct MelSweep {
  std::vector<float> wlo, whi;
  std::vector<int> d;
  std::vector<int> part;
};
bool build_mel_sweep(const mm_config& c, const float* dense, int n_waves, MelSweep* out, const double* weights = nullptr);

struct MelRuns {
  std::vector<int> hdr;
  std::vector<float> grp;
  std::vector<int> part;
};
void build_mel_runs(const mm_config& c, const MelSweep& sw, int n_waves, MelRuns* out);

int validate(const mm_config* c);
void build_window(const mm_config& c, float* out);
void build_mel(const mm_config& c, float* out);
void build_dct(const mm_config& c, float* out);
void build_twiddles(int n, float* out);
int build_butter_sos(int order, double wn, double* sos);
void build_mel_csr(const mm_config& c, const float* dense, MelCsr* csr);

}
#endif
```

modulation_mfcc_amd/csrc/mm_logmel16s.hip.inc:

```
#pragma once

struct S16Fin {
  const float* logmel;
  float* mfcc;
  float2* mod;
  const float2* tw;
  const float* dct_t;
  int n_frames, n_mels, n_mfcc, dct_kp, n_mod;
  float top_db;
  float L0;
  const float* dct_e;
};

template <int R>
__device__ __forceinline__ void s16_fin_fill_tab(const float2* tw_generic, MM_LDS mm_v2f* tab) {
  typedef f16::Geo<R> G;
  const MM_GLOBAL mm_v2f* tw = (const MM_GLOBAL mm_v2f*)tw_generic;
  for (int idx = threadIdx.x; idx < G::LPR * MM_S16_FIN_REC + 15; idx += 1024) {
    mm_v2f v;
    if (idx < G::LPR * MM_S16_FIN_REC) {
      const int q = idx / MM_S16_FIN_REC, e = idx - q * MM_S16_FIN_REC;
      if (e < 15) {
        v = tw[(q * (e + 1)) * (MM_TW_N / G::NC)];
      } else {
// ... 226 lines not shown
#pragma unroll 1
  for (int r = wave; r < n_rows; r += 16) {
    const int in_off = (r * T + 2 * ll) * 4;
    float2 x[16];
#pragma unroll
    for (int n1 = 0; n1 < 16; ++n1) x[n1] = mm_buf_f32x2(r_io, in_off + 8 * G::L * n1);
    const int cl = r / f.n_mfcc, k = r - cl * f.n_mfcc;
    const float delta = has_deltas ? deltas[cl] : 0.0f;
    if (delta != 0.0f) {
      const float ek = dct_e[k];
#pragma unroll
      for (int n1 = 0; n1 < 16; ++n1) {
        const int e = 2 * (G::L * n1 + ll);
        x[n1].x = __builtin_fmaf(ek, delta, x[n1].x);
        x[n1].y = __builtin_fmaf(ek, delta, x[n1].y);
        if (e < T) __builtin_amdgcn_raw_buffer_store_b32(__float_as_uint(x[n1].x), r_io, in_off + 8 * G::L * n1, 0, 0);
        if (e + 1 < T) __builtin_amdgcn_raw_buffer_store_b32(__float_as_uint(x[n1].y), r_io, in_off + 8 * G::L * n1 + 4, 0, 0);
      }
    }
#pragma unroll
    for (int n1 = 0; n1 < 16; ++n1) {
      const int e = 2 * (G::L * n1 + ll);
      x[n1].x = e < T ? x[n1].x : 0.0f;
      x[n1].y = e + 1 < T ? x[n1].y : 0.0f;
    }
    wpf_stages<4, false>(x, lt, xf, ll, k1, pq);
    float ar[8], br[8], ai[8], bi[8], mr, mi;
#pragma unroll
    for (int v = 0; v < 16; ++v) zf[G::zidx(k1 + 16 * (4 * pq + v / 4) + 256 * (v % 4))] = x[v].x;
    wave_lds_sync();
#pragma unroll
    for (int i = 0; i < 8; ++i) {
      const int kk = ll + G::L * i, kp = (G::NC - kk) & (G::NC - 1);
      ar[i] = zf[G::zidx(kk)];
      br[i] = zf[G::zidx(kp)];
    }
    mr = zf[G::zidx(G::NC / 2)];
    wave_lds_sync();
#pragma unroll
    for (int v = 0; v < 16; ++v) zf[G::zidx(k1 + 16 * (4 * pq + v / 4) + 256 * (v % 4))] = x[v].y;
    wave_lds_sync();
#pragma unroll
    for (int i = 0; i < 8; ++i) {
      const int kk = ll + G::L * i, kp = (G::NC - kk) & (G::NC - 1);
      ai[i] = zf[G::zidx(kk)];
      bi[i] = zf[G::zidx(kp)];
    }
    mi = zf[G::zidx(G::NC / 2)];
    wave_lds_sync();
    float2 wp[8];
    {
      const float4* s4 = reinterpret_cast<const float4*>(lt + 96);
#pragma unroll
      for (int i = 0; i < 4; ++i) { const float4 v = s4[i]; wp[2 * i] = make_float2(v.x, v.y); wp[2 * i + 1] = make_float2(v.z, v.w); }
    }
    const int out_off = r * (G::NC + 1) * 8;
#pragma unroll
    for (int i = 0; i < 8; ++i) {
      const int kk = ll + G::L * i;
      float2 xa, xb;
      f16::split_pair(make_float2(ar[i], ai[i]), make_float2(br[i], bi[i]), wp[i], xa, xb);
      __builtin_amdgcn_raw_buffer_store_b64((mm_v2u){__float_as_uint(xa.x), __float_as_uint(xa.y)}, r_out, out_off + 8 * kk, 0, 0);
      __builtin_amdgcn_raw_buffer_store_b64((mm_v2u){__float_as_uint(xb.x), __float_as_uint(xb.y)}, r_out,
                                            out_off + 8 * (G::NC - kk), 0, 0);
    }
    if (ll == 0)
      __builtin_amdgcn_raw_buffer_store_b64((mm_v2u){__float_as_uint(mr), __float_as_uint(-mi)}, r_out, out_off + 8 * (G::NC / 2), 0, 0);
  }
}

__device__ __attribute__((noinline)) void s16_finalize_all(S16Fin f, int c0, int n_clips, unsigned red_off, int clips_max) {
  extern __shared__ __attribute__((aligned(16))) char fin_smem[];
  MM_LDS char* lds = (MM_LDS char*)fin_smem;
  const int lane = threadIdx.x & 63, wave = threadIdx.x >> 6;
  const unsigned delta_off = MM_S16_DELTA_OFF(red_off, clips_max, f.n_mod);
  __syncthreads();
  bool adds = false;
  if (f.top_db >= 0.0f) {
    const MM_LDS mm_v2f* red = reinterpret_cast<const MM_LDS mm_v2f*>(lds + red_off);
    bool any = false, fixed = false;
#pragma unroll 1
    for (int cl = 0; cl < n_clips; ++cl) {
      float mx = -INFINITY, mn = INFINITY;
#pragma unroll
      for (int i = 0; i < 16; ++i) {
        const mm_v2f v = red[cl * 16 + i];
        mx = fmaxf(mx, v.x);
        mn = fminf(mn, v.y);
      }
      const float thr = mx - f.top_db;
      float delta = 0.0f;
      if (mn < thr) {
        s16_fix_clip(f, c0 + cl, thr, !fixed);
        any = true; fixed = true;
      } else if (f.dct_e && thr > f.L0) {
        delta = thr - f.L0;
        adds = true;
      }
      if (f.dct_e && threadIdx.x == 0) *reinterpret_cast<MM_LDS float*>(lds + delta_off + 4 * cl) = delta;
    }
    if (any) __syncthreads();
  }
  wg_barrier_lds();
  if (f.n_mod == 2048) {
    s16_fin_modspec_2k(f, c0, n_clips, (f.dct_e && f.top_db >= 0.0f) ? delta_off : 0xFFFFFFFFu);
    return;
  }
  if (adds) {
    s16_add_rows(f, c0, n_clips, delta_off);
    __syncthreads();
  }
  if (f.n_mod == 0) return;
  MM_LDS mm_v2f* tab = reinterpret_cast<MM_LDS mm_v2f*>(lds + MM_S16_FIN_TAB_OFF);
  if (f.n_mod == 1024) s16_fin_fill_tab<2>(f.tw, tab); else s16_fin_fill_tab<1>(f.tw, tab);
  wg_barrier_lds();
  if (f.n_mod == 1024) s16_fin_modspec<2>(f, c0, n_clips, wave, lane, (MM_LDS float*)lds, tab);
  else s16_fin_modspec<1>(f, c0, n_clips, wave, lane, (MM_LDS float*)lds, tab);
}

__device__ __forceinline__ void s16_ex_store(unsigned m0v, const float (&v)[16]) {
  unsigned keep;
  asm volatile(
      "s_mov_b32 %0, m0\n\t"
      "s_mov_b32 m0, %1\n\t"
      "s_nop 0\n\t"
      "ds_write_addtid_b32 %3 offset:%c19\n\t"
      "ds_write_addtid_b32 %4 offset:%c20\n\t"
      "ds_write_addtid_b32 %5 offset:%c21\n\t"
      "ds_write_addtid_b32 %6 offset:%c22\n\t"
      "ds_write_addtid_b32 %7 offset:%c23\n\t"
      "ds_write_addtid_b32 %8 offset:%c24\n\t"
      "ds_write_addtid_b32 %9 offset:%c25\n\t"
      "ds_write_addtid_b32 %10 offset:%c26\n\t"
      "ds_write_addtid_b32 %11 offset:%c27\n\t"
      "ds_write_addtid_b32 %12 offset:%c28\n\t"
      "ds_write_addtid_b32 %13 offset:%c29\n\t"
      "ds_write_addtid_b32 %14 offset:%c30\n\t"
      "ds_write_addtid_b32 %15 offset:%c31\n\t"
      "ds_write_addtid_b32 %16 offset:%c32\n\t"
      "ds_write_addtid_b32 %17 offset:%c33\n\t"
      "ds_write_addtid_b32 %18 offset:%c34\n\t"
      "s_mov_b32 m0, %0"
      : "=&s"(keep)
      : "s"(m0v), "i"(0),
        "v"(v[0]), "v"(v[1]), "v"(v[2]), "v"(v[3]), "v"(v[4]), "v"(v[5]), "v"(v[6]), "v"(v[7]), "v"(v[8]),
        "v"(v[9]), "v"(v[10]), "v"(v[11]), "v"(v[12]), "v"(v[13]), "v"(v[14]), "v"(v[15]),
        "i"(4 * mm_s16_xb(0)), "i"(4 * mm_s16_xb(1)), "i"(4 * mm_s16_xb(2)), "i"(4 * mm_s16_xb(3)),
        "i"(4 * mm_s16_xb(4)), "i"(4 * mm_s16_xb(5)), "i"(4 * mm_s16_xb(6)), "i"(4 * mm_s16_xb(7)),
        "i"(4 * mm_s16_xb(8)), "i"(4 * mm_s16_xb(9)), "i"(4 * mm_s16_xb(10)), "i"(4 * mm_s16_xb(11)),
        "i"(4 * mm_s16_xb(12)), "i"(4 * mm_s16_xb(13)), "i"(4 * mm_s16_xb(14)), "i"(4 * mm_s16_xb(15))
      : "memory");
}

template <int MODE, int NR, bool PRE, bool ODD, bool UNAL, bool XA>
__global__ __launch_bounds__(1024) void logmel512s_kernel(Logmel512Params p) {
  static_assert(!XA || NR >= 3, "the addtid exchange exists for NR 3 / 4 only");
  extern __shared__ __attribute__((aligned(16))) char smem[];
  float* P = reinterpret_cast<float*>(smem);
  float* S = reinterpret_cast<float*>(smem + MM_S16_S_OFF(XA));
  const int lane = threadIdx.x & 63;
  const int wave = __builtin_amdgcn_readfirstlane(threadIdx.x >> 6);
  const int q = lane & 15, row = lane >> 4;
  const float* lt = reinterpret_cast<const float*>(smem + MM_S16_LT_OFF(NR, XA)) + q * MM_W16_LT_PITCH;

  for (int i = threadIdx.x; i < 16 * MM_W16_LT_PITCH; i += 1024)
    reinterpret_cast<float*>(smem + MM_S16_LT_OFF(NR, XA))[i] = p.lane_tab[i];
  if (threadIdx.x < 64 * 3) P[(threadIdx.x / 3) * MM_S16_PITCH(XA) + 257 + threadIdx.x % 3] = 0.0f;

  for (int i = threadIdx.x; i < p.n_tab16; i += 1024)
    reinterpret_cast<float4*>(smem + MM_S16_TAB_OFF(NR, XA))[i] = p.mel_tab[i];
  const int run0 = p.wave_part[wave * 4 + 0], run1 = p.wave_part[wave * 4 + 1];
  const int m0 = p.wave_part[wave * 4 + 2];
  const bool fused = MODE == 2 || (MODE == 1 && p.out_mfcc != nullptr);
  float* Lt = reinterpret_cast<float*>(smem + p.lt_off);
  const int role = fused ? (int)((p.dct_roles >> (4 * wave)) & 15) : 15;
  const bool lt_single = fused && p.lt_b2 == 0;
  const bool halfwin = NR <= 2 && (p.dct_flags & MM_S16F_HALFWIN) != 0;
  if (fused) {
    for (int i = threadIdx.x; i < (p.lt_b2 + p.lt_rows) * 80; i += 1024) Lt[i] = 0.0f;
    for (int i = threadIdx.x; i < p.dct_kb * p.dct_nk * 64 + 16 * p.dct_kb; i += 1024)
      reinterpret_cast<float*>(smem + p.dcta_off)[i] = p.dct_a[i];
  }
  float vmin = INFINITY;
  int pb = 0, pt0 = 0;
  bool has_prev = false;
  auto dct_tile = [&](const float* Lp, int cb, int ct0) {
    int ln = lane;
    asm volatile("" : "+v"(ln));
    const int j = ln & 15, g = ln >> 4;
    const int t = ct0 + 16 * role + j;
    const float* A = reinterpret_cast<const float*>(smem + p.dcta_off) + ln;
    const float* Bp = Lp + g * 80 + 16 * role + j;
    for (int kb = 0; kb < p.dct_kb; ++kb) {
      mm_f32x4 a0 = {0.0f, 0.0f, 0.0f, 0.0f}, a1 = {0.0f, 0.0f, 0.0f, 0.0f};
      {
        const float4 e4 = *reinterpret_cast<const float4*>(A + (p.dct_kb * p.dct_nk * 64 + 16 * kb + 4 * g - ln));
        const float l0 = mm_empty_level(p.amin, p.db_offset);
        a0[0] = e4.x * l0; a0[1] = e4.y * l0; a0[2] = e4.z * l0; a0[3] = e4.w * l0;
      }
      if (p.dct_nk == 10) {
        const float* Ak = A + kb * 640;
        float av[10], bv[10];
#pragma unroll
        for (int i = 0; i < 10; ++i) {
          av[i] = Ak[i * 64];
          bv[i] = Bp[i * 320];
        }
#pragma unroll
        for (int i = 0; i < 10; i += 2) {
          a0 = __builtin_amdgcn_mfma_f32_16x16x4f32(av[i], bv[i], a0, 0, 0, 0);
          a1 = __builtin_amdgcn_mfma_f32_16x16x4f32(av[i + 1], bv[i + 1], a1, 0, 0, 0);
        }
      } else
      {
        int s0 = 0;
        for (; s0 + MM_S16F_CH <= p.dct_nk; s0 += MM_S16F_CH) {
          float av[MM_S16F_CH], bv[MM_S16F_CH];
#pragma unroll
          for (int i = 0; i < MM_S16F_CH; ++i) {
            av[i] = A[(kb * p.dct_nk + s0 + i) * 64];
            bv[i] = Bp[(s0 + i) * 320];
          }
#pragma unroll
          for (int i = 0; i < MM_S16F_CH; i += 2) {
            a0 = __builtin_amdgcn_mfma_f32_16x16x4f32(av[i], bv[i], a0, 0, 0, 0);
            a1 = __builtin_amdgcn_mfma_f32_16x16x4f32(av[i + 1], bv[i + 1], a1, 0, 0, 0);
          }
        }
        for (; s0 < p.dct_nk; s0 += 4) {
          float av[4], bv[4];
#pragma unroll
          for (int i = 0; i < 4; ++i) {
            const int s = min(s0 + i, p.dct_nk - 1);
            av[i] = s0 + i < p.dct_nk ? A[(kb * p.dct_nk + s) * 64] : 0.0f;
            bv[i] = Bp[s * 320];
          }
          a0 = __builtin_amdgcn_mfma_f32_16x16x4f32(av[0], bv[0], a0, 0, 0, 0);
          a1 = __builtin_amdgcn_mfma_f32_16x16x4f32(av[1], bv[1], a1, 0, 0, 0);
          if (s0 + 2 < p.dct_nk) {
            a0 = __builtin_amdgcn_mfma_f32_16x16x4f32(av[2], bv[2], a0, 0, 0, 0);
            a1 = __builtin_amdgcn_mfma_f32_16x16x4f32(av[3], bv[3], a1, 0, 0, 0);
          }
        }
      }
      if (t < p.n_frames) {
        float* o = p.out_mfcc + ((int64_t)cb * p.n_mfcc + 16 * kb + 4 * g) * p.n_frames + t;
#pragma unroll
        for (int r = 0; r < 4; ++r)
          if (16 * kb + 4 * g + r < p.n_mfcc) o[(int64_t)r * p.n_frames] = a0[r] + a1[r];
      }
    }
  };

  const int tpc = (int)p.tiles_per_clip;
  constexpr bool clip_mode = MODE == 2;
  const int tile_begin = clip_mode ? (int)((int64_t)blockIdx.x * p.batch / gridDim.x) * tpc
                                   : (int)((int64_t)blockIdx.x * p.n_tiles / gridDim.x);
  const int tile_end = clip_mode ? (int)((int64_t)(blockIdx.x + 1) * p.batch / gridDim.x) * tpc
                                 : (int)((int64_t)(blockIdx.x + 1) * p.n_tiles / gridDim.x);
  const int n = (int)p.n_samples;
  float vmax = -INFINITY;
  int b = tile_begin / tpc, tl = tile_begin - b * tpc;
  int nb = b, ntl = tl;

  constexpr bool addtid = XA;
  float* exw = P + 4 * wave * MM_S16_PITCH(XA) + (addtid ? mm_s16_xb(q) + 16 * row : row * 256);
  const unsigned exm0 = __builtin_amdgcn_readfirstlane((unsigned)(uintptr_t)(MM_LDS float*)(P + 4 * wave * MM_S16_PITCH(XA)));
  float* wq0 = exw + (q ^ 0);
  float* wq1 = exw + (q ^ 4);
  float* wq2 = exw + (q ^ 8);
  float* wq3 = exw + (q ^ 12);
  const int sq = addtid ? 0 : (q >> 2) & 3;
  const int rq = addtid ? 0 : q * 16;
  const float4* rq0 = reinterpret_cast<const float4*>(exw + rq + 4 * (0 ^ sq));
  const float4* rq1 = reinterpret_cast<const float4*>(exw + rq + 4 * (1 ^ sq));
  const float4* rq2 = reinterpret_cast<const float4*>(exw + rq + 4 * (2 ^ sq));
  const float4* rq3 = reinterpret_cast<const float4*>(exw + rq + 4 * (3 ^ sq));
  const float* sxf = S + (4 * wave + row) * p.hop + 2 * q;
  const float2* sx = reinterpret_cast<const float2*>(sxf);
  constexpr bool hop_odd = ODD;

  float4 sreg[NR];
  float sprev[PRE ? NR : 1];
  auto stage_interior = [&](int ttl) -> bool {
    const int base = ttl * 64 * p.hop - 256;
    return base >= 0 && base + NR * 4096 <= n;
  };
  auto stage_load = [&](int bb, int ttl) {
    const float* a = p.audio + (int64_t)bb * p.stride;
    const int first = ttl * 64 * p.hop - 256 + 4 * (int)threadIdx.x;
    int off[NR];
    if (stage_interior(ttl)) {
#pragma unroll
      for (int j = 0; j < NR; ++j) off[j] = first + 4096 * j;
    } else {
#pragma unroll
      for (int j = 0; j < NR; ++j) off[j] = min(max(first + 4096 * j, 0), n - 4);
    }
    __builtin_amdgcn_sched_barrier(0);
#pragma unroll
    for (int j = 0; j < NR; ++j) {
      if (UNAL) {
        const MmFloat4U t = *reinterpret_cast<const MmFloat4U*>(a + off[j]);
        sreg[j] = make_float4(t.x, t.y, t.z, t.w);
      } else {
        sreg[j] = *reinterpret_cast<const float4*>(a + off[j]);
      }
    }
    if (PRE) {
#pragma unroll
      for (int j = 0; j < NR; ++j) sprev[j] = a[min(max(first + 4096 * j - 1, 0), n - 1)];
    }
    __builtin_amdgcn_sched_barrier(0);
  };
  auto stage_store = [&](int ttl) {
    const int first = ttl * 64 * p.hop - 256 + 4 * (int)threadIdx.x;
    if (!PRE && stage_interior(ttl)) {
#pragma unroll
      for (int j = 0; j < NR; ++j) reinterpret_cast<float4*>(S)[threadIdx.x + 1024 * j] = sreg[j];
      return;
    }
#pragma unroll
    for (int j = 0; j < NR; ++j) {
      const int s0 = first + 4096 * j;
      const bool ok = s0 >= 0 && s0 < n;
// ... 24 lines not shown
  };
  if (tile_begin < tile_end) {
    stage_load(b, tl);
    stage_store(tl);
  }
  __syncthreads();
  float2 wp[8];
  tile512_read_wp(wp, lt);

  MM_STAMP_BEGIN(16)
  for (int tile = tile_begin; tile < tile_end; ++tile) {
    const int t0 = tl * 64;
    MM_STAMP_AT(9)
    if (++ntl == tpc) { ntl = 0; ++nb; }
    const bool more = tile + 1 < tile_end;
    stage_load(more ? nb : b, more ? ntl : tl);
    MM_STAMP_AT(11)
    if (t0 + 4 * wave < (int)p.n_frames) {
    float2 x[16];
    if (halfwin) {
      if (hop_odd) {
#pragma unroll
        for (int n1 = 4; n1 < 12; ++n1) x[n1] = make_float2(sxf[32 * n1], sxf[32 * n1 + 1]);
      } else {
#pragma unroll
        for (int n1 = 4; n1 < 12; ++n1) x[n1] = sx[16 * n1];
      }
      const float4* w4 = reinterpret_cast<const float4*>(lt) + 2;
#pragma unroll
      for (int i = 0; i < 4; ++i) {
        const float4 t = w4[i];
        x[4 + 2 * i].x *= t.x; x[4 + 2 * i].y *= t.y;
        x[5 + 2 * i].x *= t.z; x[5 + 2 * i].y *= t.w;
      }
      MM_STAMP_AT(0)
      f16::dft16_mid8(x);
    } else {
    if (hop_odd) {
#pragma unroll
      for (int n1 = 0; n1 < 16; ++n1) x[n1] = make_float2(sxf[32 * n1], sxf[32 * n1 + 1]);
    } else {
#pragma unroll
      for (int n1 = 0; n1 < 16; ++n1) x[n1] = sx[16 * n1];
    }
    {
      float2 w[16];
      tile512_read_rec<0, 8>(w, lt);
#pragma unroll
      for (int n1 = 0; n1 < 16; ++n1) { x[n1].x *= w[n1].x; x[n1].y *= w[n1].y; }
    }
    MM_STAMP_AT(0)
    f16::dft16(x);
    }
    MM_STAMP_AT(1)
    {
      float2 w[16];
      const float4* t4 = reinterpret_cast<const float4*>(lt + MM_LT_TW);
#pragma unroll
      for (int i = 0; i < 8; ++i) {
        const float4 t = t4[i];
        w[2 * i] = make_float2(t.x, t.y);
        w[2 * i + 1] = make_float2(t.z, t.w);
      }
#pragma unroll
      for (int k1 = 1; k1 < 16; ++k1)
        x[f16::P16(k1)] = f16::cmulf(x[f16::P16(k1)], w[k1 - 1]);
    }
    MM_STAMP_AT(2)
    {
#define MM_S16_WR(k1, val)                                                                         \
  (((k1) >> 2) == 0 ? wq0 : ((k1) >> 2) == 1 ? wq1 : ((k1) >> 2) == 2 ? wq2 : wq3)[(k1) * 16] = (val)
      {
        float re[16];
#pragma unroll
        for (int k1 = 0; k1 < 16; ++k1) re[k1] = x[f16::P16(k1)].x;
        if constexpr (addtid) {
          s16_ex_store(exm0, re);
        } else {
#pragma unroll
          for (int k1 = 0; k1 < 16; ++k1) MM_S16_WR(k1, re[k1]);
        }
      }
      wave_lds_sync();
      {
        const float4 v0 = *rq0, v1 = *rq1, v2 = *rq2, v3 = *rq3;
        x[0].x = v0.x; x[1].x = v0.y; x[2].x = v0.z; x[3].x = v0.w;
        x[4].x = v1.x; x[5].x = v1.y; x[6].x = v1.z; x[7].x = v1.w;
        x[8].x = v2.x; x[9].x = v2.y; x[10].x = v2.z; x[11].x = v2.w;
        x[12].x = v3.x; x[13].x = v3.y; x[14].x = v3.z; x[15].x = v3.w;
      }
      wave_lds_sync();
      float im[16];
#pragma unroll
      for (int k1 = 0; k1 < 16; ++k1) im[k1] = x[f16::P16(k1)].y;
      if constexpr (addtid) {
        s16_ex_store(exm0, im);
      } else {
#pragma unroll
        for (int k1 = 0; k1 < 16; ++k1) MM_S16_WR(k1, im[k1]);
      }
      wave_lds_sync();
      {
        const float4 v0 = *rq0, v1 = *rq1, v2 = *rq2, v3 = *rq3;
        x[0].y = v0.x; x[1].y = v0.y; x[2].y = v0.z; x[3].y = v0.w;
        x[4].y = v1.x; x[5].y = v1.y; x[6].y = v1.z; x[7].y = v1.w;
        x[8].y = v2.x; x[9].y = v2.y; x[10].y = v2.z; x[11].y = v2.w;
        x[12].y = v3.x; x[13].y = v3.y; x[14].y = v3.z; x[15].y = v3.w;
      }
      wave_lds_sync();
#undef MM_S16_WR
    }
    MM_STAMP_AT(10)
    f16::dft16(x);
    MM_STAMP_AT(3)
    {
      float2 pb[9];
      f16::fetch_partners<1>(x, pb, lane, q);
      float* pr = P + (4 * wave + row) * MM_S16_PITCH(XA);
      float pw[17];
#pragma unroll
      for (int j = 0; j < 8; ++j) {
        float2 xa, xb;
        f16::split_pair(x[f16::P16(j)], pb[j], wp[j], xa, xb);
        pw[2 * j] = fmaf(xa.x, xa.x, xa.y * xa.y);
        pw[2 * j + 1] = fmaf(xb.x, xb.x, xb.y * xb.y);
      }
      {
        const float2 zm = x[f16::P16(8)];
        pw[16] = fmaf(zm.x, zm.x, zm.y * zm.y);
      }
#pragma unroll
      for (int j = 0; j < 8; ++j) {
        pr[q + 16 * j] = pw[2 * j];
        pr[256 - q - 16 * j] = pw[2 * j + 1];
      }
      if (q == 0) {
        pr[128] = pw[16];
        pr[257] = 0.0f; pr[258] = 0.0f; pr[259] = 0.0f;
      }
    }
    }
    MM_STAMP_AT(4)
    if (!lt_single) {
      wg_barrier_lds();
      MM_STAMP_AT(6)
      stage_store(more ? ntl : tl);
    }
    if (MODE != 0 && role < 4 && has_prev) dct_tile(Lt + (((tile & 1) ^ 1) * p.lt_b2) * 80, pb, pt0);
    if (lt_single) {
      wg_barrier_lds();
      stage_store(more ? ntl : tl);
    }
    MM_STAMP_AT(5)
    if (MODE == 0) {
      tile512_store_power_tile(p.out_power, P, MM_S16_PITCH(XA), b, t0, p.n_frames, wave, 16, lane);
    } else {
      const bool valid = (t0 + lane) < p.n_frames;
      float* o = p.out_logmel + ((int64_t)b * p.n_mels + m0) * p.n_frames + t0 + lane;
      const float* pl = P + lane * MM_S16_PITCH(XA);
      const float4* hdr = reinterpret_cast<const float4*>(smem + MM_S16_TAB_OFF(NR, XA));
      const float4* grp = hdr + p.n_runs;
      float carry = 0.0f;
      if (run0 < run1) {
        float4 h = hdr[run0];
        for (int r = run0; r < run1; ++r) {
          const int k4e = __builtin_amdgcn_readfirstlane(__float_as_int(h.x));
          const int k4 = k4e & 0xFFFF;
          const bool empty_d = (k4e >> 16) & 1;
          const int ng = __builtin_amdgcn_readfirstlane(__float_as_int(h.y));
          const int go = __builtin_amdgcn_readfirstlane(__float_as_int(h.z));
          const int dd = __builtin_amdgcn_readfirstlane(__float_as_int(h.w));
          if (r + 1 < run1) h = hdr[r + 1];
          const float4* pp = reinterpret_cast<const float4*>(pl + k4);
          const MM_LDS mm_v4f* gw = (const MM_LDS mm_v4f*)(grp + 2 * go);
          asm volatile("" : "+v"(gw));
          float sa = 0.0f, sb = 0.0f;
          MM_STAMP_AT(12)
#pragma unroll 2
          for (int g = 0; g < ng; ++g) {
            const float4 pv = pp[g];
            const mm_v4f wa = gw[2 * g], wb = gw[2 * g + 1];
            sa = fmaf(wa.x, pv.x, sa); sb = fmaf(wa.y, pv.x, sb);
            sa = fmaf(wa.z, pv.y, sa); sb = fmaf(wa.w, pv.y, sb);
            sa = fmaf(wb.x, pv.z, sa); sb = fmaf(wb.y, pv.z, sb);
            sa = fmaf(wb.z, pv.w, sa); sb = fmaf(wb.w, pv.w, sb);
          }
          MM_STAMP_AT(13)
          float dbm = __builtin_nanf("");
          if (dd >= m0) {
            if (!empty_d) {
              const float v = carry + sa;
              const float db = 3.0102999566398120f * __builtin_amdgcn_logf(mm_max_raw_s(v, p.amin)) - p.db_offset;
              if (valid && p.out_logmel) *o = db;
              dbm = valid ? db : dbm;
              if (fused) Lt[((tile & 1) * p.lt_b2 + dd) * 80 + lane] = db;
            }
            o += p.n_frames;
          }
          mm_max_acc(vmax, dbm);
          mm_min_acc(vmin, dbm);
          carry = sb;
          MM_STAMP_AT(14)
        }
      }
      const bool clip_done = (tile + 1 == tile_end) || (ntl == 0);
      if (clip_done) {
        vmax = wave_max(vmax);
        if (p.key_nmin || clip_mode) vmin = wave_min(vmin);
        if (clip_mode) {
          if (lane == 0)
            reinterpret_cast<float2*>(smem + p.red_off)[(b - tile_begin / tpc) * 16 + wave] = make_float2(vmax, vmin);
        } else if (lane == 0 && vmax > -INFINITY) {
          atomicMax(p.clip_key + b, float_key(vmax));
          if (p.key_nmin) atomicMax(p.key_nmin + b, float_key(-vmin));
        }
        vmax = -INFINITY; vmin = INFINITY;
      }
    }
    MM_STAMP_AT(7)
    wg_barrier_lds();
    MM_STAMP_AT(8)
    pb = b; pt0 = t0; has_prev = true;
    b = nb; tl = ntl;
  }
  if (role < 4 && has_prev) dct_tile(Lt + (((tile_end - 1) & 1) * p.lt_b2) * 80, pb, pt0);
  if (clip_mode && has_prev) {
    S16Fin f;
    f.logmel = p.out_logmel; f.mfcc = p.out_mfcc; f.mod = p.out_mod; f.tw = p.tw; f.dct_t = p.dct_t;
    f.n_frames = (int)p.n_frames; f.n_mels = p.n_mels; f.n_mfcc = p.n_mfcc; f.dct_kp = p.dct_kp; f.n_mod = p.n_mod;
    f.top_db = p.top_db;
    f.dct_e = (p.dct_flags & MM_S16F_SKIP) ? p.dct_a + p.dct_kb * p.dct_nk * 64 : nullptr;
    f.L0 = mm_empty_level(p.amin, p.db_offset);
    s16_finalize_all(f, tile_begin / tpc, (tile_end - tile_begin) / tpc, p.red_off,
                     (int)((p.batch + gridDim.x - 1) / gridDim.x));
  }
  MM_STAMP_END(16)
}

using S16Kernel = void (*)(Logmel512Params);
#define MM_S16_KEYS 192
template <int KEY>
static constexpr S16Kernel s16_entry() {
  constexpr int MODE = KEY >> 6, NR = ((KEY >> 4) & 3) + 1;
  constexpr bool XA = (KEY & 8) != 0, PRE = (KEY & 4) != 0, ODD = (KEY & 2) != 0, UNAL = (KEY & 1) != 0;
  if constexpr (NR < 3 && (XA || PRE)) return nullptr;
  else return logmel512s_kernel<MODE, NR, PRE, ODD, UNAL, XA>;
}
template <int... KEY>
static S16Kernel s16_lookup(int key, std::integer_sequence<int, KEY...>) {
  static constexpr S16Kernel table[] = {s16_entry<KEY>()...};
  return table[key];
}
static S16Kernel s16_kernel(int key) { return s16_lookup(key, std::make_integer_sequence<int, MM_S16_KEYS>()); }

void launch_s16(int mode, int nr, bool xa, bool pre, bool odd, bool unal, dim3 grid, size_t lds, hipStream_t st,
                const Logmel512Params& q) {
  if (mode == 1 && q.out_mod != nullptr) mode = 2;
  mode = mode == 0 || mode == 1 ? mode : 2;
  nr = nr >= 1 && nr <= 3 ? nr : 4;
  if (nr < 3) { xa = false; pre = false; }
  const int key = mode << 6 | (nr - 1) << 4 | (xa ? 8 : 0) | (pre ? 4 : 0) | (odd ? 2 : 0) | (unal ? 1 : 0);
  hipLaunchKernelGGL(s16_kernel(key), grid, dim3(1024), lds, st, q);
}

bool set_s16_attr(int bytes) {
  for (int key = 0; key < MM_S16_KEYS; ++key)
    if (s16_kernel(key) &&
        hipFuncSetAttribute((const void*)s16_kernel(key), hipFuncAttributeMaxDynamicSharedMemorySize, bytes) != hipSuccess)
      return false;
  return true;
}
```

modulation_mfcc_amd/csrc/mm_plan.h:

```cpp
#pragma once
#include "mm_common.h"

struct AnyPlan {
  int nn = 0, packed = 0, n_pass = 0, radix[16] = {0}, M = 0, log2M = 0, tpf = 64;
  unsigned grp_bytes = 0, b_off = 0, p_off = 0;
  float2 *d_tw = nullptr, *d_split = nullptr, *d_chirp = nullptr, *d_bhat = nullptr;
  float* d_tabpack = nullptr;
  int tab_floats = 0, o_tw = 0, o_split = 0, o_chirp = 0, o_melw = 0, o_mstart = 0, o_mlen = 0, o_moff = 0;
  bool lds_tab = false;
  bool ok = false;
  int fb = 0;
  int reg2 = 0, reg2_r2 = 0;
  unsigned fb_grp_bytes = 0;
};

#define MM_M12_MW 4
#define MM_M12_UMAX 12

#define MM_MAX_TIMED 16384
#define MM_MAX_SAMPLES (((int64_t)1 << 29) - 8192)

struct mm_plan {
  mm_config cfg{};
  int device = 0;
  int n_bins = 0, log2nc = 0, kp = 0;
  float db_offset = 0.0f;
  int num_cus = 256;

  struct Base {
    float *d_window = nullptr, *d_mel_w = nullptr, *d_dct_t = nullptr;
    float2* d_tw = nullptr;
    int *d_mel_start = nullptr, *d_mel_len = nullptr, *d_mel_off = nullptr;
  } base;
  struct Embed { float* d_window = nullptr; int factor = 1; } embed;
  struct W8 {
    bool ok = false; float* d_tab = nullptr; int* d_part = nullptr;
    int n_runs = 0, n_tab16 = 0; size_t lds_bytes = 0;
  } w8;
  struct W16 {
    bool ok = false; float *d_tab = nullptr, *d_lane_tab = nullptr; int* d_part = nullptr;
    int n_runs = 0, n_tab16 = 0; size_t lds_bytes = 0;
  } w16;
  struct H16 {
    bool ok = false; float* d_tab = nullptr; int* d_part = nullptr;
    int n_pairs = 0, n_tab16 = 0; size_t lds_bytes = 0;
  } h16;
  struct S16 {
    int nr = 0;
    bool xa = false;
    bool halfwin = false;
    size_t lds_bytes = 0;
  } s16;
  struct S16F {
    bool ok = false;
    float *d_tab = nullptr, *d_dcta = nullptr; int* d_part = nullptr;
    int n_runs = 0, n_tab16 = 0, lt_rows = 0, nk = 0, kb = 0;
    int flags = 0;
    unsigned lt_off = 0, dcta_off = 0, red_off = 0;
    unsigned long long roles = 0; size_t lds_bytes = 0;
  } s16f;
  struct M12 {
    bool ok = false, fused_dct = false;
    float *d_a = nullptr, *d_dct = nullptr, *d_zeros = nullptr;
    int units[MM_M12_MW * MM_M12_UMAX * 4] = {}, n_units[8] = {};
    int nb = 0, nr = 0, s_floats = 0, n_a2 = 0;
    unsigned win_off = 0, tw_off = 0, a_off = 0, dct_off = 0, part_off = 0, cnt_off = 0;
    size_t lds_bytes = 0;
  } m12;
  struct Wpf {
    bool ok = false; float *d_lane_tab = nullptr, *d_mel_lane = nullptr;
    int r = 0, waves = 0, group_max = 0; size_t lds_bytes = 0;
    bool w16 = false; size_t lds16 = 0;
    bool half = false; int pairs = 0;
    int waves_half = 0; size_t lds_half = 0;
    int z = 0;
  } wpf;
  struct DctFm {
    float* d_wave_a = nullptr;
    int kb = 0, wave_nk = 0, ch = 0;
  } dctfm;
  struct Rf2k { bool ok = false; float* d_lane_tab = nullptr; } rf2k;
  AnyPlan any;

  struct Switches {
    int variant = 0;
    int force_generic = 0;
    int no_fuse = 0;
    int no_fuse_tail = 0;
    int fuse_tail_wide = 0;
  } user;
  struct Timing {
    int on = 0, ev_used = 0;
    std::vector<hipEvent_t> ev_pool;
    std::vector<int> ev_stage;
    double t_sum[MM_NUM_STAGES] = {};
    int64_t t_cnt[MM_NUM_STAGES] = {};
  } timing;

  mm_plan() = default;
  mm_plan(const mm_plan&) = delete; mm_plan& operator=(const mm_plan&) = delete;
  ~mm_plan() { for (void* d : owned) (void)hipFree(d); }
  template <class T>
  int upload(T** dst, const void* src, size_t bytes) {
    HIP_TRY(hipMalloc((void**)dst, bytes));
    owned.push_back(*dst);
    HIP_TRY(hipMemcpy(*dst, src, bytes, hipMemcpyHostToDevice));
    return MM_OK;
  }

 private:
  std::vector<void*> owned;
};

namespace {

struct StageTimer {
  mm_plan* p;
  hipStream_t s;
  int idx;
  StageTimer(mm_plan* plan, int stage, hipStream_t stream) : p(plan), s(stream), idx(-1) {
    mm_plan::Timing& t = p->timing;
    if (!t.on || t.ev_used >= MM_MAX_TIMED) return;
    if (t.on != 1 && !((t.on >> (stage + 1)) & 1)) return;
    if ((size_t)(2 * t.ev_used + 1) >= t.ev_pool.size()) {
      hipEvent_t a, b;
      if (hipEventCreate(&a) != hipSuccess || hipEventCreate(&b) != hipSuccess) return;
      t.ev_pool.push_back(a);
      t.ev_pool.push_back(b);
    }
    idx = t.ev_used++;
    t.ev_stage.resize(t.ev_used);
    t.ev_stage[idx] = stage;
    (void)hipEventRecord(t.ev_pool[2 * idx], s);
  }
  ~StageTimer() {
    if (idx >= 0) (void)hipEventRecord(p->timing.ev_pool[2 * idx + 1], s);
  }
};

}
```

modulation_mfcc_amd/csrc/mm_s16.h:

```cpp
#pragma once
#include "mm_common.h"

#define MM_S16_XA_PITCH 268
#define MM_S16_PITCH(XA) ((XA) ? MM_S16_XA_PITCH : MM_LM_PITCH)
#define MM_S16_S_OFF(XA) (64 * MM_S16_PITCH(XA) * 4)
__host__ __device__ constexpr int mm_s16_xb(int k1) {
  const int m = k1 < 4 ? k1 : (k1 >= 12 ? k1 - 8 : k1 - 4), j = 2 * m + ((k1 >= 4 && k1 < 12) ? 1 : 0);
  return 64 * j + 4 * ((m & 3) + 8 * (m >> 2));
}
static_assert(mm_s16_xb(0) == 0 && mm_s16_xb(1) == 132 && mm_s16_xb(2) == 264 && mm_s16_xb(3) == 396 &&
              mm_s16_xb(4) == 64 && mm_s16_xb(5) == 196 && mm_s16_xb(6) == 328 && mm_s16_xb(7) == 460 &&
              mm_s16_xb(8) == 608 && mm_s16_xb(9) == 740 && mm_s16_xb(10) == 872 && mm_s16_xb(11) == 1004 &&
              mm_s16_xb(12) == 544 && mm_s16_xb(13) == 676 && mm_s16_xb(14) == 808 && mm_s16_xb(15) == 940,
              "exchange block offsets (tests/test_s16_layout.py)");
static_assert(1068 <= 4 * MM_S16_XA_PITCH && 15 * 4 * MM_S16_XA_PITCH * 4 < 65536, "exchange area of the XA layout");
#ifndef MM_S16F_CH
#define MM_S16F_CH 12
#endif
#ifndef MM_S16F_W
#define MM_S16F_W 0.5
#endif
#define MM_S16_LT_OFF(NR, XA) (MM_S16_S_OFF(XA) + (NR) * 16384)
#define MM_S16_TAB_OFF(NR, XA) (MM_S16_LT_OFF(NR, XA) + 16 * MM_W16_LT_PITCH * 4)

#define MM_S16_CPW_MAX 32
#define MM_S16_FIN_REC 24
#define MM_S16_FIN_TAB_BYTES ((32 * MM_S16_FIN_REC + 15) * 8)
#define MM_S16_FIN_TAB_OFF (16 * 9216)
#define MM_S16_DELTA_OFF(red_off, clips_max, n_mod)                                                             \
  (((n_mod) == 2048 && (red_off) + (clips_max) * 128 < MM_S16_FIN2K_BYTES) ? MM_S16_FIN2K_BYTES : (red_off) + (clips_max) * 128)
#define MM_S16_FIN2K_BYTES 103424

struct Logmel512Params;
void launch_s16(int mode, int nr, bool xa, bool pre, bool odd, bool unal, dim3 grid, size_t lds, hipStream_t st,
                const Logmel512Params& q);
bool set_s16_attr(int bytes);
```

modulation_mfcc_amd/csrc/mm_tables.cpp:

```cpp
#include "mm_internal.h"

#include <algorithm>
#include <cmath>
#include <complex>
#include <cstring>
#include <vector>

namespace mm {

static const double kPi = 3.14159265358979323846;

int validate(const mm_config* c) {
  if (!c) return MM_ERR_INVALID_ARG;
  if (!(c->sr > 0.0)) return MM_ERR_INVALID_ARG;
  if (c->n_fft < 2) return MM_ERR_INVALID_ARG;
  if (c->n_fft > 8192) return MM_ERR_UNSUPPORTED;
  if (c->win_length < 1 || c->win_length > c->n_fft) return MM_ERR_INVALID_ARG;
  if (c->hop_length < 1) return MM_ERR_INVALID_ARG;
  if (c->n_mels < 1 || c->n_mels > 256) return MM_ERR_INVALID_ARG;
  if (c->n_mfcc < 1 || c->n_mfcc > c->n_mels) return MM_ERR_INVALID_ARG;
  if (!(c->fmin >= 0.0) || !(c->fmax > c->fmin)) return MM_ERR_INVALID_ARG;
  if (!(c->amin > 0.0f)) return MM_ERR_INVALID_ARG;
  if (c->center != 1) return MM_ERR_UNSUPPORTED;
  if (c->n_mod_fft != 0 &&
// ... 8 lines not shown
  std::memset(out, 0, sizeof(float) * N);
  const double step = (kPi - (-kPi)) / (double)M;
  for (int n = 0; n < M; ++n) {
    double fac = (double)n * step + (-kPi);
    if (M == 1) fac = -kPi;
    double w = 0.0;
    w += 0.5 * std::cos(0.0 * fac);
    w += 0.5 * std::cos(1.0 * fac);
    if (M == 1) w = 1.0;
    out[lpad + n] = (float)w;
  }
}

static const double kFsp = 200.0 / 3;
static const double kMinLogHz = 1000.0;
static const double kMinLogMel = (1000.0 - 0.0) / (200.0 / 3);
static double logstep() { return std::log(6.4) / 27.0; }

static double hz_to_mel(double f) {
  double mel = (f - 0.0) / kFsp;
  if (f >= kMinLogHz) mel = kMinLogMel + std::log(f / kMinLogHz) / logstep();
  return mel;
}
static double mel_to_hz(double m) {
  double f = 0.0 + kFsp * m;
  if (m >= kMinLogMel) f = kMinLogHz * std::exp(logstep() * (m - kMinLogMel));
  return f;
}

void build_mel(const mm_config& c, float* out) {
  const int n_mels = c.n_mels, n_bins = c.n_fft / 2 + 1;
  std::vector<double> mel_f(n_mels + 2), fftf(n_bins);
  const double min_mel = hz_to_mel(c.fmin), max_mel = hz_to_mel(c.fmax);
  const int npts = n_mels + 2;
  const double step = (max_mel - min_mel) / (double)(npts - 1);
  for (int i = 0; i < npts; ++i) mel_f[i] = mel_to_hz((double)i * step + min_mel);
  mel_f[npts - 1] = mel_to_hz(max_mel);
  const double val = 1.0 / ((double)c.n_fft * (1.0 / c.sr));
  for (int k = 0; k < n_bins; ++k) fftf[k] = (double)k * val;
  for (int i = 0; i < n_mels; ++i) {
    const double fd0 = mel_f[i + 1] - mel_f[i], fd1 = mel_f[i + 2] - mel_f[i + 1];
    const double enorm = 2.0 / (mel_f[i + 2] - mel_f[i]);
    for (int k = 0; k < n_bins; ++k) {
      const double lower = -(mel_f[i] - fftf[k]) / fd0;
      const double upper = (mel_f[i + 2] - fftf[k]) / fd1;
      const float w32 = (float)std::max(0.0, std::min(lower, upper));
      out[(size_t)i * n_bins + k] = (float)((double)w32 * enorm);
    }
  }
}

void build_dct(const mm_config& c, float* out) {
  const int N = c.n_mels;
  for (int k = 0; k < c.n_mfcc; ++k) {
    const double f = (k == 0) ? std::sqrt(1.0 / (4.0 * N)) : std::sqrt(1.0 / (2.0 * N));
    for (int m = 0; m < N; ++m)
      out[(size_t)k * N + m] = (float)(2.0 * f * std::cos(kPi * k * (2.0 * m + 1.0) / (2.0 * N)));
  }
}

void build_twiddles(int n, float* out) {
  for (int k = 0; k < n; ++k) {
    const double a = -2.0 * kPi * (double)k / (double)n;
    out[2 * k] = (float)std::cos(a);
    out[2 * k + 1] = (float)std::sin(a);
  }
}

int build_butter_sos(int order, double wn, double* sos) {
  if (order < 1 || order > 64 || !(wn > 0.0) || !(wn < 1.0) || !sos) return MM_ERR_INVALID_ARG;
  typedef std::complex<double> cd;
  const double fs = 2.0;
  const double warped = 2.0 * fs * std::tan(kPi * wn / fs);
  std::vector<cd> p(order);
  for (int i = 0; i < order; ++i) {
    const int m = -order + 1 + 2 * i;
    cd pa = -std::exp(cd(0.0, kPi * m / (2.0 * order)));
    pa *= warped;
    p[i] = (2.0 * fs + pa) / (2.0 * fs - pa);
  }
  cd den(1.0, 0.0);
  for (int i = 0; i < order; ++i) {
    const int m = -order + 1 + 2 * i;
    cd pa = -std::exp(cd(0.0, kPi * m / (2.0 * order)));
    pa *= warped;
    den *= (2.0 * fs - pa);
  }
  const double k = std::pow(warped, order) * (cd(1.0, 0.0) / den).real();
  std::vector<cd> pairs;
  bool has_real = false;
  cd real_pole(0, 0);
  for (int i = 0; i < order; ++i) {
    if (std::fabs(p[i].imag()) < 1e-14 * std::max(1.0, std::abs(p[i]))) {
      has_real = true;
      real_pole = cd(p[i].real(), 0.0);
    } else if (p[i].imag() > 0) {
      pairs.push_back(p[i]);
    }
  }
  std::sort(pairs.begin(), pairs.end(),
            [](const cd& a, const cd& b) { return std::fabs(1.0 - std::abs(a)) < std::fabs(1.0 - std::abs(b)); });
  const int n_sec = (order + 1) / 2;
  std::vector<cd> sec_pole(n_sec);
  std::vector<int> sec_real(n_sec, 0);
  int si = n_sec - 1;
  size_t pi_ = 0;
  if (has_real) {
    for (; si >= 1; --si) sec_pole[si] = pairs[pi_++];
    sec_pole[0] = real_pole;
    sec_real[0] = 1;
  } else {
    for (; si >= 0; --si) sec_pole[si] = pairs[pi_++];
  }
  int single_zero_sec = -1;
  if (has_real) {
    single_zero_sec = 0;
    for (int s = n_sec - 1; s >= 1; --s)
      if (std::abs(sec_pole[s]) < std::abs(sec_pole[s] + 1.0)) { single_zero_sec = s; break; }
  }
  for (int s = 0; s < n_sec; ++s) {
    double* r = sos + 6 * s;
    const bool single_zero = (s == single_zero_sec);
    r[0] = 1.0; r[1] = single_zero ? 1.0 : 2.0; r[2] = single_zero ? 0.0 : 1.0;
    if (sec_real[s]) {
      r[3] = 1.0; r[4] = -sec_pole[s].real(); r[5] = 0.0;
    } else {
      r[3] = 1.0; r[4] = -2.0 * sec_pole[s].real(); r[5] = std::norm(sec_pole[s]);
    }
  }
  sos[0] *= k; sos[1] *= k; sos[2] *= k;
  return n_sec;
}

void build_mel_csr(const mm_config& c, const float* dense, MelCsr* csr) {
  const int n_mels = c.n_mels, n_bins = c.n_fft / 2 + 1;
  csr->start.assign(n_mels, 0);
  csr->len.assign(n_mels, 0);
  csr->off.assign(n_mels, 0);
  csr->w.clear();
  for (int m = 0; m < n_mels; ++m) {
    int lo = n_bins, hi = -1;
    for (int k = 0; k < n_bins; ++k)
      if (dense[(size_t)m * n_bins + k] != 0.0f) { lo = std::min(lo, k); hi = std::max(hi, k); }
    csr->off[m] = (int)csr->w.size();
    if (hi >= lo) {
      csr->start[m] = lo;
      csr->len[m] = hi - lo + 1;
      for (int k = lo; k <= hi; ++k) csr->w.push_back(dense[(size_t)m * n_bins + k]);
    }
  }
  if (csr->w.empty()) csr->w.push_back(0.0f);
}

bool build_mel_sweep(const mm_config& c, const float* dense, int n_waves, MelSweep* out, const double* weights) {
  const int n_mels = c.n_mels, n_bins = c.n_fft / 2 + 1;
  out->wlo.assign(n_bins, 0.0f);
  out->whi.assign(n_bins, 0.0f);
  out->d.assign(n_bins, -1);
  int prev = -1;
  for (int k = 0; k < n_bins; ++k) {
    int nz[3], cnt = 0;
    for (int m = 0; m < n_mels && cnt < 3; ++m)
      if (dense[(size_t)m * n_bins + k] != 0.0f) nz[cnt++] = m;
    int d = prev;
    if (cnt == 1) {
      const int m = nz[0];
      if (m - 1 >= prev) { d = m - 1; out->whi[k] = dense[(size_t)m * n_bins + k]; }
      else if (m >= prev) { d = m; out->wlo[k] = dense[(size_t)m * n_bins + k]; }
      else return false;
    } else if (cnt == 2) {
      if (nz[1] != nz[0] + 1 || nz[0] < prev) return false;
      d = nz[0];
      out->wlo[k] = dense[(size_t)nz[0] * n_bins + k];
      out->whi[k] = dense[(size_t)nz[1] * n_bins + k];
    } else if (cnt > 2) {
      return false;
    }
    out->d[k] = d;
    prev = d;
  }
  auto range_of = [&](int m0, int m1, int* kb, int* ke) {
    int b = n_bins, e = 0;
    for (int k = 0; k < n_bins; ++k)
      if (out->d[k] >= m0 - 1 && out->d[k] <= m1 - 1 && (out->wlo[k] != 0.0f || out->whi[k] != 0.0f)) {
        b = std::min(b, k);
        e = std::max(e, k + 1);
      }
    if (b >= e) { b = 0; e = 0; }
    *kb = b; *ke = e;
  };
  int kb_all, ke_all;
  range_of(0, n_mels, &kb_all, &ke_all);
  const double total = (double)(ke_all - kb_all) + 6.0 * n_mels;
  out->part.assign((size_t)n_waves * 4, 0);
  double wsum = 0.0, wcum = 0.0;
  for (int w = 0; w < n_waves; ++w) wsum += weights ? weights[w] : 1.0;
  int m = 0;
  for (int w = 0; w < n_waves; ++w) {
    wcum += weights ? weights[w] : 1.0;
    const int m0 = m;
    int m1 = m0;
    if (w == n_waves - 1) {
      m1 = n_mels;
    } else {
      const double target = total * wcum / wsum;
      while (m1 < n_mels) {
        int kb, ke;
        range_of(0, m1 + 1, &kb, &ke);
        const double cum = (double)(ke - kb_all > 0 ? ke - kb_all : 0) + 6.0 * (m1 + 1);
        if (cum > target && m1 > m0) break;
        ++m1;
        if (cum > target) break;
      }
      const int left_waves = n_waves - 1 - w;
      if (n_mels - m1 < left_waves) m1 = std::max(m0, n_mels - left_waves);
    }
    int kb, ke;
    range_of(m0, m1, &kb, &ke);
    if (m1 <= m0) { kb = 0; ke = 0; }
    out->part[w * 4 + 0] = kb;
    out->part[w * 4 + 1] = ke;
    out->part[w * 4 + 2] = m0;
    out->part[w * 4 + 3] = m1;
    m = m1;
  }
  return true;
}

void build_mel_runs(const mm_config& c, const MelSweep& sw, int n_waves, MelRuns* out) {
  const int n_bins = c.n_fft / 2 + 1;
  out->hdr.clear(); out->grp.clear();
  out->part.assign((size_t)n_waves * 4, 0);
  for (int w = 0; w < n_waves; ++w) {
    const int m0 = sw.part[w * 4 + 2], m1 = sw.part[w * 4 + 3];
    out->part[w * 4 + 0] = (int)(out->hdr.size() / 4);
    out->part[w * 4 + 2] = m0;
    out->part[w * 4 + 3] = m1;
    if (m1 > m0) {
      for (int d = m0 - 1; d <= m1 - 1; ++d) {
        int ks = n_bins, ke = 0;
        for (int k = 0; k < n_bins; ++k)
          if (sw.d[k] == d && (sw.wlo[k] != 0.0f || sw.whi[k] != 0.0f)) { ks = std::min(ks, k); ke = std::max(ke, k + 1); }
        int g0 = 0, g1 = 0;
        if (ke > ks) { g0 = ks / 4; g1 = (ke + 3) / 4; }
        out->hdr.push_back(4 * g0);
        out->hdr.push_back(g1 - g0);
        out->hdr.push_back((int)(out->grp.size() / 8));
        out->hdr.push_back(d);
        for (int g = g0; g < g1; ++g) {
          float wl[4], wh[4];
          for (int u = 0; u < 4; ++u) {
            const int k = 4 * g + u;
            const bool in = (k >= ks && k < ke && k < n_bins && sw.d[k] == d);
            wl[u] = in ? sw.wlo[k] : 0.0f;
            wh[u] = in ? sw.whi[k] : 0.0f;
            if (d == m0 - 1) wl[u] = 0.0f;
            if (d == m1 - 1) wh[u] = 0.0f;
          }
          for (int u = 0; u < 4; ++u) out->grp.push_back(wl[u]);
          for (int u = 0; u < 4; ++u) out->grp.push_back(wh[u]);
        }
      }
    }
    out->part[w * 4 + 1] = (int)(out->hdr.size() / 4);
  }
}

}
```

modulation_mfcc_amd/plan.py:

```python
from __future__ import annotations

import ctypes as C
from dataclasses import dataclass, asdict

import numpy as np

from . import _lib, ragged
from .ragged import check_frames, check_lengths, sos_padlen, group_rows as by_length


@dataclass(frozen=True)
class MfccConfig:
    sr: float = 10000.0
    n_fft: int = 512
    win_length: int = 250
    hop_length: int = 50
    n_mels: int = 128
    n_mfcc: int = 13
    fmin: float = 100.0
    fmax: float = 10000.0
    preemph: float = 0.0
    top_db: float = 80.0
    amin: float = 1e-10
    center: bool = True
    n_mod_fft: int = 0

    @classmethod
    def from_reference_call(cls, sigSr, *, tStep=0.001, winLen=0.025, n_mfcc=13, n_fft=512,
                            minFreq=100, maxFreq=10000, **extra):
        return cls(sr=float(sigSr), n_fft=int(n_fft), win_length=int(winLen * sigSr),
                   hop_length=int(tStep * sigSr), n_mels=int(extra.pop("n_mels", 128)),
                   n_mfcc=int(n_mfcc), fmin=float(minFreq), fmax=float(maxFreq), **extra)

    def to_c(self) -> _lib.mm_config:
        return _lib.mm_config(float(self.sr), int(self.n_fft), int(self.win_length),
                              int(self.hop_length), int(self.n_mels), int(self.n_mfcc),
                              float(self.fmin), float(self.fmax), float(self.preemph),
                              float(self.top_db), float(self.amin), 1 if self.center else 0,
                              int(self.n_mod_fft))

    def validate(self):
        c = self.to_c()
        _lib.check(_lib.load().mm_config_validate(C.byref(c)), "mm_config_validate")
        return self

    def num_frames(self, n_samples: int) -> int:
        c = self.to_c()
        r = _lib.load().mm_num_frames(C.byref(c), int(n_samples))
        if r < 0:
            _lib.check(int(r), "mm_num_frames")
        return int(r)

    @property
    def n_bins(self) -> int:
        return self.n_fft // 2 + 1

    def mod_fft_len(self, n_frames: int) -> int:
        c = self.to_c()
        r = _lib.load().mm_mod_fft_len(C.byref(c), int(n_frames))
        if r < 0:
            _lib.check(int(r), "mm_mod_fft_len")
        return int(r)

    def window(self) -> np.ndarray:
        c = self.to_c()
        out = np.empty(self.n_fft, dtype=np.float32)
        _lib.check(_lib.load().mm_build_window(C.byref(c), out.ctypes.data), "mm_build_window")
        return out

    def mel_filterbank(self) -> np.ndarray:
        c = self.to_c()
        out = np.empty((self.n_mels, self.n_bins), dtype=np.float32)
        _lib.check(_lib.load().mm_build_mel(C.byref(c), out.ctypes.data), "mm_build_mel")
        return out

    def dct_matrix(self) -> np.ndarray:
        c = self.to_c()
        out = np.empty((self.n_mfcc, self.n_mels), dtype=np.float32)
        _lib.check(_lib.load().mm_build_dct(C.byref(c), out.ctypes.data), "mm_build_dct")
        return out

    def mel_sweep(self, n_waves: int = 8):
        c = self.to_c()
        wlo = np.empty(self.n_bins, dtype=np.float32)
        whi = np.empty(self.n_bins, dtype=np.float32)
        d = np.empty(self.n_bins, dtype=np.int32)
        part = np.empty((n_waves, 4), dtype=np.int32)
        _lib.check(_lib.load().mm_build_mel_sweep(C.byref(c), n_waves, wlo.ctypes.data, whi.ctypes.data,
                                                  d.ctypes.data, part.ctypes.data), "mm_build_mel_sweep")
        return wlo, whi, d, part

    def mel_runs(self, n_waves: int = 8):
        c = self.to_c()
        cap_r, cap_g = self.n_mels + 2 * n_waves + 8, self.n_bins // 4 + 2 * self.n_mels + 4 * n_waves + 8
        hdr = np.zeros((cap_r, 4), dtype=np.int32)
        grp = np.zeros((cap_g, 8), dtype=np.float32)
        part = np.zeros((n_waves, 4), dtype=np.int32)
        cnt = np.zeros(2, dtype=np.int32)
        _lib.check(_lib.load().mm_build_mel_runs(C.byref(c), n_waves, hdr.ctypes.data, cap_r,
                                                 grp.ctypes.data, cap_g, part.ctypes.data,
                                                 cnt.ctypes.data), "mm_build_mel_runs")
        return hdr[:cnt[0]], grp[:cnt[1]], part

    def asdict(self):
        return asdict(self)


def butter_sos(order: int, wn: float) -> np.ndarray:
    n_sec = (int(order) + 1) // 2
    out = np.empty((max(n_sec, 1), 6), dtype=np.float64)
    r = _lib.load().mm_build_butter_sos(int(order), float(wn), out.ctypes.data)
    if r < 0:
        _lib.check(int(r), "mm_build_butter_sos")
    return out[:r]


KERNEL_PATHS = ("generic", "radix16-w8", "radix16-w16", "radix16-wpf", "radix16-w16s", "radix16-m12", "any-length", "radix16-h32")


def _torch():
    import torch
    return torch


class MfccPlan:

    def __init__(self, cfg: MfccConfig, device=None):
        torch = _torch()
        lib = _lib.load()
        cfg.validate()
        if not torch.cuda.is_available():
            raise RuntimeError("modulation_mfcc_amd needs an AMD GPU (gfx950); torch.cuda is not "
                               "available and there is no CPU fallback")
        self.cfg = cfg
        self.device = torch.device("cuda", torch.cuda.current_device()) if device is None \
            else torch.device(device)
        self._lib = lib
        self._h = C.c_void_p()
        with torch.cuda.device(self.device):
            c = cfg.to_c()
            _lib.check(lib.mm_plan_create(C.byref(c), C.byref(self._h)), "mm_plan_create")
        self._ws = None

    def close(self):
        if getattr(self, "_h", None) is not None and self._h:
            self._lib.mm_plan_destroy(self._h)
            self._h = C.c_void_p()

    def __del__(self):
        try:
            self.close()
        except Exception:
            pass

    def _stream(self):
        return C.c_void_p(_torch().cuda.current_stream(self.device).cuda_stream)

    def _check_audio(self, audio):
        torch = _torch()
        if not ragged.is_device_tensor(audio):
            raise TypeError("audio must be a CUDA(HIP) torch tensor")
        if audio.dtype != torch.float32:
            raise TypeError("audio must be float32")
        if audio.dim() == 1:
            audio = audio.unsqueeze(0)
        if audio.dim() != 2:
            raise ValueError("audio must be [n] or [batch, n]")
        if audio.stride(1) != 1:
            audio = audio.contiguous()
        if audio.shape[1] < 1:
            raise ValueError("empty audio")
        if audio.device != self.device:
            raise ValueError(f"audio is on {audio.device}, the plan on {self.device}")
        return audio

    def _check_out(self, out, shape, dtype, what):
        torch = _torch()
        if not (ragged.is_device_tensor(out) and out.device == self.device):
            raise TypeError(f"{what}: out must be a tensor on {self.device}")
        if out.dtype != dtype or tuple(out.shape) != tuple(shape) or not out.is_contiguous():
            raise ValueError(f"{what}: out must be a contiguous {dtype} tensor of shape {tuple(shape)}, "
                             f"got {out.dtype} {tuple(out.shape)} (contiguous: {out.is_contiguous()})")
        return out

    def workspace(self, batch, n_samples):
        torch = _torch()
        need = int(self._lib.mm_workspace_bytes(self._h, batch, n_samples))
        if self._ws is None or self._ws.numel() < need:
            self._ws = torch.empty(need, dtype=torch.uint8, device=self.device)
        return self._ws

    @property
    def kernel_path(self):
        return KERNEL_PATHS[self._lib.mm_plan_kernel_path(self._h)]

    @property
    def fused_dct(self):
        return bool(self._lib.mm_plan_fused_dct(self._h))

    def set_fuse_dct(self, on=True):
        return bool(self._lib.mm_plan_set_fuse_dct(self._h, 1 if on else 0))

    def set_variant(self, which):
        if which in (None, "auto"):
            v = 0
        elif isinstance(which, str):
            v = KERNEL_PATHS.index(which if which.startswith("radix16-") else "radix16-" + which)
        else:
            v = int(which)
        prev = self._lib.mm_plan_set_variant(self._h, v)
        if prev < 0:
            _lib.check(prev, "mm_plan_set_variant")
        return "auto" if prev == 0 else KERNEL_PATHS[prev]

    def fused_tail(self, batch, n_samples):
        return bool(self._lib.mm_plan_fused_tail(self._h, int(batch), int(n_samples)))

    def set_fuse_tail(self, on=True):
        return self._lib.mm_plan_set_fuse_tail(self._h, 2 if on == 2 else (1 if on else 0))

    def force_generic(self, on=True):
        return self._lib.mm_plan_force_generic(self._h, 1 if on else 0)

    def mfcc(self, audio, out=None):
        torch = _torch()
        audio = self._check_audio(audio)
        B, n = audio.shape
        T = self.cfg.num_frames(n)
        if out is None:
            out = torch.empty((B, self.cfg.n_mfcc, T), dtype=torch.float32, device=self.device)
        else:
            self._check_out(out, (B, self.cfg.n_mfcc, T), torch.float32, "mfcc")
        ws = self.workspace(B, n)
        with torch.cuda.device(self.device):
            _lib.check(self._lib.mm_mfcc_f32(self._h, audio.data_ptr(), B, n, audio.stride(0),
                                             out.data_ptr(), ws.data_ptr(), ws.numel(), self._stream()),
                       "mm_mfcc_f32")
        return out

    def mfcc_modspec(self, audio, out=None, out_mod=None):
        torch = _torch()
        audio = self._check_audio(audio)
        B, n = audio.shape
        T = self.cfg.num_frames(n)
        nm = self.cfg.mod_fft_len(T)
        if out is None:
            out = torch.empty((B, self.cfg.n_mfcc, T), dtype=torch.float32, device=self.device)
        else:
            self._check_out(out, (B, self.cfg.n_mfcc, T), torch.float32, "mfcc")
        if out_mod is None:
            out_mod = torch.empty((B, self.cfg.n_mfcc, nm // 2 + 1), dtype=torch.complex64, device=self.device)
        else:
            self._check_out(out_mod, (B, self.cfg.n_mfcc, nm // 2 + 1), torch.complex64, "modspec")
        if nm > 8192:
            self.mfcc(audio, out=out)
            return out, self.modspec(out, out=out_mod)
        ws = self.workspace(B, n)
        with torch.cuda.device(self.device):
            _lib.check(self._lib.mm_mfcc_modspec_f32(self._h, audio.data_ptr(), B, n, audio.stride(0), out.data_ptr(),
                                                     out_mod.data_ptr(), ws.data_ptr(), ws.numel(), self._stream()),
                       "mm_mfcc_modspec_f32")
        return out, out_mod

    def ragged_workspace(self, batch, n_samples):
        torch = _torch()
        need = int(self._lib.mm_ragged_workspace_bytes(self._h, batch, n_samples))
        if need == 0:
            raise ValueError("mm_ragged_workspace_bytes: invalid arguments")
        if self._ws is None or self._ws.numel() < need:
            self._ws = torch.empty(need, dtype=torch.uint8, device=self.device)
        return self._ws

    def _ragged_lengths(self, lengths, B, n):
        lens = ragged.check_lengths(lengths, B, n, self.device)
        n_fft, hop = self.cfg.n_fft, self.cfg.hop_length
        if isinstance(lens, np.ndarray):
            both = ragged.counts_on_device(np.stack([lens, ragged.stft_frames(lens, n_fft, hop)]), self.device)
            return both[0], both[1]
        return lens, ragged.stft_frames(lens.clamp(1, n), n_fft, hop)

    def _ragged(self, audio, lengths, out, out_mod, want_mod):
        torch = _torch()
        audio = self._check_audio(audio)
        B, n = audio.shape
        T = self.cfg.num_frames(n)
        lens, frames = self._ragged_lengths(lengths, B, n)
        if out is None:
            out = torch.empty((B, self.cfg.n_mfcc, T), dtype=torch.float32, device=self.device)
        else:
            self._check_out(out, (B, self.cfg.n_mfcc, T), torch.float32, "mfcc")
        nm = self.cfg.mod_fft_len(T) if want_mod else 0
        if want_mod:
            if out_mod is None:
                out_mod = torch.empty((B, self.cfg.n_mfcc, nm // 2 + 1), dtype=torch.complex64, device=self.device)
            else:
                self._check_out(out_mod, (B, self.cfg.n_mfcc, nm // 2 + 1), torch.complex64, "modspec")
        fused_mod = want_mod and nm <= 8192
        ws = self.ragged_workspace(B, n)
        with torch.cuda.device(self.device):
            _lib.check(self._lib.mm_mfcc_ragged_f32(self._h, audio.data_ptr(), B, n, audio.stride(0), lens.data_ptr(),
                                                    out.data_ptr(), out_mod.data_ptr() if fused_mod else None,
                                                    ws.data_ptr(), ws.numel(), self._stream()),
                       "mm_mfcc_ragged_f32")
        if want_mod and not fused_mod:
            self.modspec(out, out=out_mod)
        return out, out_mod, frames

    def mfcc_ragged(self, audio, lengths, out=None):
        out, _, frames = self._ragged(audio, lengths, out, None, False)
        return out, frames

    def mfcc_modspec_ragged(self, audio, lengths, out=None, out_mod=None):
        return self._ragged(audio, lengths, out, out_mod, True)

    def mfcc_modpsd(self, audio, lengths=None, **welch):
        from . import modpsd
        fs = self.cfg.sr / self.cfg.hop_length
        n_mfcc = self.cfg.n_mfcc
        if lengths is None:
            mfcc = self.mfcc(audio)
            f, pxx = modpsd.modulation_psd_batch(mfcc, fs, **welch)
            return mfcc, f, pxx
        audio = self._check_audio(audio)
        B, n = audio.shape
        lens = ragged.check_lengths(lengths, B, n, self.device)
        nperseg = int(welch.get("nperseg", 256))
        if isinstance(lens, np.ndarray):
            ragged.refuse_short(ragged.stft_frames(lens, self.cfg.n_fft, self.cfg.hop_length), self.cfg.num_frames(n), nperseg,
                                lambda short: modpsd.SHORT_TEXT.format(nperseg, short), "clip", "frames")
        mfcc, frames = self.mfcc_ragged(audio, lens)
        rows_frames = frames.unsqueeze(1).expand(B, n_mfcc).reshape(B * n_mfcc)
        f, pxx = modpsd.modulation_psd_ragged_batch(mfcc.reshape(B * n_mfcc, mfcc.shape[2]), rows_frames, fs, **welch)
        return mfcc, f, pxx.reshape(B, n_mfcc, pxx.shape[1])

    def mfcc_modcsd(self, audio, ref, lengths=None, **welch):
        from . import modcsd, modpsd
        fs = self.cfg.sr / self.cfg.hop_length
        n_mfcc = self.cfg.n_mfcc
        audio = self._check_audio(audio)
        B, n = audio.shape
        T = self.cfg.num_frames(n)
        if not ragged.is_device_tensor(ref) or ref.dim() != 2 or tuple(ref.shape) != (B, T):
            raise ValueError(f"ref must be a device tensor [{B}, {T}]: one curve per clip on the plan's frame grid")
        if lengths is None:
            mfcc = self.mfcc(audio)
            return (mfcc,) + modcsd.modulation_cross_spectra_batch(mfcc, ref, fs, **welch)
        lens = ragged.check_lengths(lengths, B, n, self.device)
        nperseg = int(welch.get("nperseg", 256))
        if isinstance(lens, np.ndarray):
            ragged.refuse_short(ragged.stft_frames(lens, self.cfg.n_fft, self.cfg.hop_length), T, nperseg,
                                lambda short: modpsd.SHORT_TEXT.format(nperseg, short), "clip", "frames")
        mfcc, frames = self.mfcc_ragged(audio, lens)
        rows_frames = frames.unsqueeze(1).expand(B, n_mfcc).reshape(B * n_mfcc)
        f, *spectra = modcsd.modulation_cross_spectra_ragged_batch(mfcc.reshape(B * n_mfcc, T), ref, rows_frames, fs, **welch)
        return (mfcc, f) + tuple(s.reshape(B, n_mfcc, s.shape[1]) for s in spectra)

    def logmel(self, audio):
        torch = _torch()
        audio = self._check_audio(audio)
        B, n = audio.shape
        T = self.cfg.num_frames(n)
        lm = torch.empty((B, self.cfg.n_mels, T), dtype=torch.float32, device=self.device)
        mx = torch.empty((B,), dtype=torch.float32, device=self.device)
        _lib.check(self._lib.mm_logmel_f32(self._h, audio.data_ptr(), B, n, audio.stride(0),
                                           lm.data_ptr(), mx.data_ptr(), self._stream()),
                   "mm_logmel_f32")
        return lm, mx

    def stft_power(self, audio):
        torch = _torch()
        audio = self._check_audio(audio)
        B, n = audio.shape
# ... 149 lines not shown
```

Measured before the change: 2.455 billion frames/s.

## Share boundary mel filter between adjacent waves via LDS handoff

Adds a 'shared runs' variant of the fused 16-wave logmel kernel. Each boundary mel filter is accumulated once: the producer wave writes its partial carry to LDS and the consumer wave adds it after the barrier. Previously both neighbouring waves swept the overlapping bins. A cost-weighted partition (filter_cost 27) rebalances mel ranges, and the consumer's finalisation runs at raised wave priority. The variant is on by default when supported, and the exchange adds a barrier-dependent tail step per tile.

```diff
diff --git a/include/modmfcc.h b/include/modmfcc.h
--- a/include/modmfcc.h
+++ b/include/modmfcc.h
@@ -64,6 +64,8 @@
                        float* whi , int32_t* d , int32_t* part );
 int mm_build_mel_runs(const mm_config* cfg, int n_waves, int32_t* hdr, int32_t hdr_cap, float* grp,
                       int32_t grp_cap, int32_t* part, int32_t* counts);
+int mm_build_mel_runs_shared(const mm_config* cfg, int n_waves, int weighted, int32_t* hdr, int32_t hdr_cap, float* grp,
+                             int32_t grp_cap, int32_t* part, int32_t* counts);
 int mm_build_butter_sos(int order, double wn, double* sos );
 
 int mm_plan_create(const mm_config* cfg, mm_plan** out);
@@ -74,6 +76,8 @@
 int mm_plan_set_fuse_dct(mm_plan* plan, int on);
 int mm_plan_fused_tail(const mm_plan* plan, int64_t batch, int64_t n_samples);
 int mm_plan_set_fuse_tail(mm_plan* plan, int on);
+int mm_plan_shared_runs(const mm_plan* plan);
+int mm_plan_set_shared_runs(mm_plan* plan, int on);
 int mm_plan_force_generic(mm_plan* plan, int on);
 int mm_plan_set_variant(mm_plan* plan, int variant);
 size_t mm_workspace_bytes(const mm_plan* plan, int64_t batch, int64_t n_samples);
diff --git a/modulation_mfcc_amd/_lib.py b/modulation_mfcc_amd/_lib.py
--- a/modulation_mfcc_amd/_lib.py
+++ b/modulation_mfcc_amd/_lib.py
@@ -115,6 +115,7 @@
     "mm_build_dct": (C.c_int, [_cfgp, _vp]),
     "mm_build_mel_sweep": (C.c_int, [_cfgp, C.c_int, _vp, _vp, _vp, _vp]),
     "mm_build_mel_runs": (C.c_int, [_cfgp, C.c_int, _vp, C.c_int32, _vp, C.c_int32, _vp, _vp]),
+    "mm_build_mel_runs_shared": (C.c_int, [_cfgp, C.c_int, C.c_int, _vp, C.c_int32, _vp, C.c_int32, _vp, _vp]),
     "mm_build_butter_sos": (C.c_int, [C.c_int, C.c_double, _vp]),
     "mm_plan_create": (C.c_int, [_cfgp, C.POINTER(_vp)]),
     "mm_plan_destroy": (C.c_int, [_vp]),
@@ -123,6 +124,8 @@
     "mm_plan_fused_dct": (C.c_int, [_vp]),
     "mm_plan_set_fuse_dct": (C.c_int, [_vp, C.c_int]),
     "mm_plan_fused_tail": (C.c_int, [_vp, _i64, _i64]),
+    "mm_plan_shared_runs": (C.c_int, [_vp]),
+    "mm_plan_set_shared_runs": (C.c_int, [_vp, C.c_int]),
     "mm_plan_set_fuse_tail": (C.c_int, [_vp, C.c_int]),
     "mm_mfcc_modspec_f32": (C.c_int, [_vp, _vp, _i64, _i64, _i64, _vp, _vp, _vp, C.c_size_t, _vp]),
     "mm_plan_force_generic": (C.c_int, [_vp, C.c_int]),
diff --git a/modulation_mfcc_amd/csrc/mm_api.hip b/modulation_mfcc_amd/csrc/mm_api.hip
--- a/modulation_mfcc_amd/csrc/mm_api.hip
+++ b/modulation_mfcc_amd/csrc/mm_api.hip
@@ -289,6 +289,28 @@
   if (!mm::build_mel_sweep(*c, mel.data(), n_waves, &sw)) return MM_ERR_UNSUPPORTED;
   mm::MelRuns r;
   mm::build_mel_runs(*c, sw, n_waves, &r);
+  counts[0] = (int32_t)(r.hdr.size() / 4);
+  counts[1] = (int32_t)(r.grp.size() / 8);
+  if (counts[0] > hdr_cap || counts[1] > grp_cap) return MM_ERR_WORKSPACE;
+  std::memcpy(hdr, r.hdr.data(), r.hdr.size() * 4);
+  std::memcpy(grp, r.grp.data(), r.grp.size() * 4);
+  std::memcpy(part, r.part.data(), r.part.size() * 4);
+  return MM_OK;
+}
+int mm_build_mel_runs_shared(const mm_config* c, int n_waves, int weighted, int32_t* hdr, int32_t hdr_cap, float* grp,
+                             int32_t grp_cap, int32_t* part, int32_t* counts) {
+  int s = mm::validate(c);
+  if (s) return s;
+  if (n_waves < 1 || !hdr || !grp || !part || !counts || (weighted && n_waves != 16)) return MM_ERR_INVALID_ARG;
+  std::vector<float> mel((size_t)c->n_mels * (c->n_fft / 2 + 1));
+  mm::build_mel(*c, mel.data());
+  mm::MelSweep sw;
+  const double wts_d[16] = {1, 1, 1, MM_S16F_W, 1, 1, 1, MM_S16F_W, 1, 1, 1, MM_S16F_W, 1, 1, 1, MM_S16F_W};
+  if (!(weighted ? mm::build_mel_sweep(*c, mel.data(), n_waves, &sw, wts_d, MM_S16F_SH_FC, MM_S16F_SH_FC)
+                 : mm::build_mel_sweep(*c, mel.data(), n_waves, &sw)))
+    return MM_ERR_UNSUPPORTED;
+  mm::MelRuns r;
+  mm::build_mel_runs_shared(*c, sw, n_waves, &r);
   counts[0] = (int32_t)(r.hdr.size() / 4);
   counts[1] = (int32_t)(r.grp.size() / 8);
   if (counts[0] > hdr_cap || counts[1] > grp_cap) return MM_ERR_WORKSPACE;
@@ -629,6 +651,28 @@
       p->s16.xa = false;
       p->s16.lds_bytes = (size_t)MM_S16_TAB_OFF(p->s16.nr, false) + tab16_bytes;
     }
+    if (!single && !ef.skip) {
+      mm::MelSweep sws;
+      mm::MelRuns rs;
+      if (!mm::build_mel_sweep(c, h.melp, 16, &sws, wts_d, MM_S16F_SH_FC, MM_S16F_SH_FC)) return;
+      mm::build_mel_runs_shared(c, sws, 16, &rs);
+      for (int w = 0; w < 16; ++w) if (rs.part[w * 4 + 3] & MM_RUNS_CONSUMER) extra[w] += 20.0;
+      const std::vector<float> tabs = packed_run_table(rs);
+      const std::vector<int> parts = balance_parts_over_simds(rs, extra, &wave_of_part);
+      mm_plan::S16F::Shared& sh = f.sh;
+      sh.roles = ~0ull;
+      for (int k = 0; k < 4; ++k) {
+        const int w = wave_of_part[4 * k + 3];
+        sh.roles = (sh.roles & ~(0xFull << (4 * w))) | ((unsigned long long)k << (4 * w));
+      }
+      sh.n_runs = (int)(rs.hdr.size() / 4); sh.n_tab16 = (int)(tabs.size() / 4);
+      sh.lt_off = (unsigned)align_up((size_t)MM_S16_TAB_OFF(p->s16.nr, xa) + tabs.size() * 4, 16);
+      sh.dcta_off = sh.lt_off + 2u * (unsigned)lt_rows * 320u;
+      sh.red_off = (unsigned)align_up((size_t)sh.dcta_off + dcta.size() * 4, 16);
+      sh.lds_bytes = (size_t)sh.red_off + 2 * 16 * 8;
+      sh.ok = sh.lds_bytes <= lds && p->upload(&sh.d_tab, tabs.data(), tabs.size() * 4) == MM_OK &&
+              p->upload(&sh.d_part, parts.data(), parts.size() * 4) == MM_OK;
+    }
     return;
   }
 }
@@ -880,6 +924,11 @@
   return per * g * 100 <= batch * 104;
 }
 
+static bool s16f_shared_runs(const mm_plan* p, bool unal) {
+  return p->s16f.ok && p->s16f.sh.ok && !p->user.no_shared_runs &&
+         s16_has_shared(p->s16.nr, p->s16.xa, p->cfg.preemph != 0.0f, p->cfg.hop_length & 1, unal);
+}
+
 enum Want { WANT_ROWS, WANT_MFCC, WANT_MFCC_CLIP, WANT_MODSPEC };
 
 struct CallShape {
@@ -926,6 +975,19 @@
   p->user.no_fuse_tail = on ? 0 : 1;
   p->user.fuse_tail_wide = on == 2 ? 1 : 0;
   return prev;
+}
+
+int mm_plan_set_shared_runs(mm_plan* p, int on) {
+  if (!p) return MM_ERR_INVALID_ARG;
+  const int prev = !p->user.no_shared_runs;
+  p->user.no_shared_runs = on ? 0 : 1;
+  return prev;
+}
+
+int mm_plan_shared_runs(const mm_plan* p) {
+  if (!p) return MM_ERR_INVALID_ARG;
+  return dispatch(p, 1, CallShape(), WANT_MFCC).fused_dct && dispatch(p, 1, CallShape(), WANT_MFCC).kernel == MM_K_W16S &&
+                 s16f_shared_runs(p, false) ? 1 : 0;
 }
 
 int mm_plan_set_variant(mm_plan* p, int variant) {
@@ -1105,24 +1167,28 @@
     return MM_OK;
   }
   size_t lds = p->s16.lds_bytes;
+  bool sh = false;
   if (d.fused_dct) {
     const mm_plan::S16F& f = p->s16f;
-    q.mel_tab = (const float4*)f.d_tab; q.n_runs = f.n_runs; q.n_tab16 = f.n_tab16;
-    q.wave_part = f.d_part;
+    sh = s16f_shared_runs(p, unaligned_rows(c));
+    q.mel_tab = (const float4*)(sh ? f.sh.d_tab : f.d_tab); q.n_runs = sh ? f.sh.n_runs : f.n_runs;
+    q.n_tab16 = sh ? f.sh.n_tab16 : f.n_tab16;
+    q.wave_part = sh ? f.sh.d_part : f.d_part;
     q.out_mfcc = o.mfcc; q.key_nmin = o.key_nmin; q.dct_a = f.d_dcta; q.n_mfcc = p->cfg.n_mfcc;
     q.dct_nk = f.nk; q.dct_kb = f.kb; q.lt_rows = f.lt_rows;
-    q.lt_off = f.lt_off; q.dcta_off = f.dcta_off; q.dct_roles = f.roles;
+    q.lt_off = sh ? f.sh.lt_off : f.lt_off; q.dcta_off = sh ? f.sh.dcta_off : f.dcta_off;
+    q.dct_roles = sh ? f.sh.roles : f.roles;
     q.dct_flags = f.flags | (p->s16.halfwin ? MM_S16F_HALFWIN : 0);
     q.lt_b2 = (f.flags & MM_S16F_SINGLE) ? 0 : f.lt_rows;
     if (p->cfg.top_db < 0.0f) q.out_logmel = nullptr;
-    lds = f.lds_bytes;
-    q.red_off = f.red_off;
+    lds = sh ? f.sh.lds_bytes : f.lds_bytes;
+    q.red_off = sh ? f.sh.red_off : f.red_off;
     if (d.clip) {
       q.out_mod = (float2*)o.mod; q.n_mod = o.mod ? c.n_mod : 0; q.dct_t = p->base.d_dct_t; q.dct_kp = p->kp; q.top_db = p->cfg.top_db;
       grid = c.batch < p->num_cus ? c.batch : p->num_cus;
       const size_t per = (size_t)((c.batch + grid - 1) / grid);
-      lds = std::max((size_t)f.red_off + per * 128, (size_t)MM_S16_FIN_TAB_OFF + MM_S16_FIN_TAB_BYTES);
-      lds = std::max(lds, (size_t)MM_S16_DELTA_OFF((size_t)f.red_off, per, q.n_mod) + per * 4);
+      lds = std::max((size_t)q.red_off + per * 128, (size_t)MM_S16_FIN_TAB_OFF + MM_S16_FIN_TAB_BYTES);
+      lds = std::max(lds, (size_t)MM_S16_DELTA_OFF((size_t)q.red_off, per, q.n_mod) + per * 4);
       if (q.n_mod == 2048) {
         q.tw = (const float2*)p->rf2k.d_lane_tab;
         lds = std::max(lds, (size_t)MM_S16_FIN2K_BYTES);
@@ -1130,7 +1196,7 @@
       mode = 2;
     }
   }
-  launch_s16(mode, p->s16.nr, p->s16.xa, p->cfg.preemph != 0.0f, p->cfg.hop_length & 1, unaligned_rows(c),
+  launch_s16(mode, p->s16.nr, p->s16.xa, p->cfg.preemph != 0.0f, p->cfg.hop_length & 1, unaligned_rows(c), sh,
              dim3((unsigned)grid), lds, st, q);
   return MM_OK;
 }
diff --git a/modulation_mfcc_amd/csrc/mm_internal.h b/modulation_mfcc_amd/csrc/mm_internal.h
--- a/modulation_mfcc_amd/csrc/mm_internal.h
+++ b/modulation_mfcc_amd/csrc/mm_internal.h
@@ -17,7 +17,8 @@
   std::vector<int> d;
   std::vector<int> part;
 };
-bool build_mel_sweep(const mm_config& c, const float* dense, int n_waves, MelSweep* out, const double* weights = nullptr);
+bool build_mel_sweep(const mm_config& c, const float* dense, int n_waves, MelSweep* out, const double* weights = nullptr,
+                     double filter_cost = 6.0, double lead_cost = 0.0);
 
 struct MelRuns {
   std::vector<int> hdr;
@@ -25,6 +26,9 @@
   std::vector<int> part;
 };
 void build_mel_runs(const mm_config& c, const MelSweep& sw, int n_waves, MelRuns* out);
+#define MM_RUNS_CONSUMER (1 << 16)
+#define MM_RUNS_PRODUCER (1 << 17)
+void build_mel_runs_shared(const mm_config& c, const MelSweep& sw, int n_waves, MelRuns* out);
 
 int validate(const mm_config* c);
 void build_window(const mm_config& c, float* out);
diff --git a/modulation_mfcc_amd/csrc/mm_logmel16s.hip.inc b/modulation_mfcc_amd/csrc/mm_logmel16s.hip.inc
--- a/modulation_mfcc_amd/csrc/mm_logmel16s.hip.inc
+++ b/modulation_mfcc_amd/csrc/mm_logmel16s.hip.inc
@@ -402,9 +402,13 @@
       : "memory");
 }
 
-template <int MODE, int NR, bool PRE, bool ODD, bool UNAL, bool XA>
+#ifndef MM_S16_SH_PRIO
+#define MM_S16_SH_PRIO 3
+#endif
+template <int MODE, int NR, bool PRE, bool ODD, bool UNAL, bool XA, bool SH>
 __global__ __launch_bounds__(1024) void logmel512s_kernel(Logmel512Params p) {
   static_assert(!XA || NR >= 3, "the addtid exchange exists for NR 3 / 4 only");
+  static_assert(!SH || MODE != 0, "shared runs belong to the fused launches");
   extern __shared__ __attribute__((aligned(16))) char smem[];
   float* P = reinterpret_cast<float*>(smem);
   float* S = reinterpret_cast<float*>(smem + MM_S16_S_OFF(XA));
@@ -421,6 +425,7 @@
     reinterpret_cast<float4*>(smem + MM_S16_TAB_OFF(NR, XA))[i] = p.mel_tab[i];
   const int run0 = p.wave_part[wave * 4 + 0], run1 = p.wave_part[wave * 4 + 1];
   const int m0 = p.wave_part[wave * 4 + 2];
+  const int m1f = SH ? __builtin_amdgcn_readfirstlane(p.wave_part[wave * 4 + 3]) : 0;
   const bool fused = MODE == 2 || (MODE == 1 && p.out_mfcc != nullptr);
   float* Lt = reinterpret_cast<float*>(smem + p.lt_off);
   const int role = fused ? (int)((p.dct_roles >> (4 * wave)) & 15) : 15;
@@ -751,6 +756,7 @@
       stage_store(more ? ntl : tl);
     }
     MM_STAMP_AT(5)
+    float held = 0.0f;
     if (MODE == 0) {
       tile512_store_power_tile(p.out_power, P, MM_S16_PITCH(XA), b, t0, p.n_frames, wave, 16, lane);
     } else {
@@ -786,7 +792,10 @@
           }
           MM_STAMP_AT(13)
           float dbm = __builtin_nanf("");
-          if (dd >= m0) {
+          if (SH && (m1f & MM_RUNS_CONSUMER) && r == run0) {
+            held = sa;
+            o += p.n_frames;
+          } else if (dd >= m0) {
             if (!empty_d) {
               const float v = carry + sa;
               const float db = 3.0102999566398120f * __builtin_amdgcn_logf(mm_max_raw_s(v, p.amin)) - p.db_offset;
@@ -801,9 +810,10 @@
           carry = sb;
           MM_STAMP_AT(14)
         }
+        if (SH && (m1f & MM_RUNS_PRODUCER)) Lt[((tile & 1) * p.lt_b2 + (m1f & 0xFFFF)) * 80 + lane] = carry;
       }
       const bool clip_done = (tile + 1 == tile_end) || (ntl == 0);
-      if (clip_done) {
+      if (clip_done && !SH) {
         vmax = wave_max(vmax);
         if (p.key_nmin || clip_mode) vmin = wave_min(vmin);
         if (clip_mode) {
@@ -819,9 +829,37 @@
     MM_STAMP_AT(7)
     wg_barrier_lds();
     MM_STAMP_AT(8)
+    if constexpr (SH) {
+      const bool valid = (t0 + lane) < p.n_frames;
+      __builtin_amdgcn_s_setprio(MM_S16_SH_PRIO);
+      if (m1f & MM_RUNS_CONSUMER) {
+        float* lr = Lt + ((tile & 1) * p.lt_b2 + m0) * 80 + lane;
+        const float v = *lr + held;
+        const float db = 3.0102999566398120f * __builtin_amdgcn_logf(mm_max_raw_s(v, p.amin)) - p.db_offset;
+        if (valid && p.out_logmel) p.out_logmel[((int64_t)b * p.n_mels + m0) * p.n_frames + t0 + lane] = db;
+        *lr = db;
+        const float dbm = valid ? db : __builtin_nanf("");
+        mm_max_acc(vmax, dbm);
+        mm_min_acc(vmin, dbm);
+      }
+      if ((tile + 1 == tile_end) || (ntl == 0)) {
+        vmax = wave_max(vmax);
+        if (p.key_nmin || clip_mode) vmin = wave_min(vmin);
+        if (clip_mode) {
+          if (lane == 0)
+            reinterpret_cast<float2*>(smem + p.red_off)[(b - tile_begin / tpc) * 16 + wave] = make_float2(vmax, vmin);
+        } else if (lane == 0 && vmax > -INFINITY) {
+          atomicMax(p.clip_key + b, float_key(vmax));
+          if (p.key_nmin) atomicMax(p.key_nmin + b, float_key(-vmin));
+        }
+        vmax = -INFINITY; vmin = INFINITY;
+      }
+      __builtin_amdgcn_s_setprio(0);
+    }
     pb = b; pt0 = t0; has_prev = true;
     b = nb; tl = ntl;
   }
+  if (SH) wg_barrier_lds();
   if (role < 4 && has_prev) dct_tile(Lt + (((tile_end - 1) & 1) * p.lt_b2) * 80, pb, pt0);
   if (clip_mode && has_prev) {
     S16Fin f;
@@ -837,13 +875,14 @@
 }
 
 using S16Kernel = void (*)(Logmel512Params);
-#define MM_S16_KEYS 192
+#define MM_S16_KEYS 448
 template <int KEY>
 static constexpr S16Kernel s16_entry() {
-  constexpr int MODE = KEY >> 6, NR = ((KEY >> 4) & 3) + 1;
-  constexpr bool XA = (KEY & 8) != 0, PRE = (KEY & 4) != 0, ODD = (KEY & 2) != 0, UNAL = (KEY & 1) != 0;
-  if constexpr (NR < 3 && (XA || PRE)) return nullptr;
-  else return logmel512s_kernel<MODE, NR, PRE, ODD, UNAL, XA>;
+  constexpr int MODE = (KEY >> 6) & 3, NR = ((KEY >> 4) & 3) + 1;
+  constexpr bool XA = (KEY & 8) != 0, PRE = (KEY & 4) != 0, ODD = (KEY & 2) != 0, UNAL = (KEY & 1) != 0, SH = (KEY & 256) != 0;
+  if constexpr (MODE == 3 || (NR < 3 && (XA || PRE))) return nullptr;
+  else if constexpr (SH && (MODE == 0 || NR < 3 || !XA || PRE || ODD || UNAL)) return nullptr;
+  else return logmel512s_kernel<MODE, NR, PRE, ODD, UNAL, XA, SH>;
 }
 template <int... KEY>
 static S16Kernel s16_lookup(int key, std::integer_sequence<int, KEY...>) {
@@ -852,14 +891,21 @@
 }
 static S16Kernel s16_kernel(int key) { return s16_lookup(key, std::make_integer_sequence<int, MM_S16_KEYS>()); }
 
-void launch_s16(int mode, int nr, bool xa, bool pre, bool odd, bool unal, dim3 grid, size_t lds, hipStream_t st,
+static int s16_key(int mode, int nr, bool xa, bool pre, bool odd, bool unal, bool sh) {
+  nr = nr >= 1 && nr <= 3 ? nr : 4;
+  if (nr < 3) { xa = false; pre = false; }
+  return (sh ? 256 : 0) | mode << 6 | (nr - 1) << 4 | (xa ? 8 : 0) | (pre ? 4 : 0) | (odd ? 2 : 0) | (unal ? 1 : 0);
+}
+
+bool s16_has_shared(int nr, bool xa, bool pre, bool odd, bool unal) {
+  return s16_kernel(s16_key(1, nr, xa, pre, odd, unal, true)) != nullptr;
+}
+
+void launch_s16(int mode, int nr, bool xa, bool pre, bool odd, bool unal, bool sh, dim3 grid, size_t lds, hipStream_t st,
                 const Logmel512Params& q) {
   if (mode == 1 && q.out_mod != nullptr) mode = 2;
   mode = mode == 0 || mode == 1 ? mode : 2;
-  nr = nr >= 1 && nr <= 3 ? nr : 4;
-  if (nr < 3) { xa = false; pre = false; }
-  const int key = mode << 6 | (nr - 1) << 4 | (xa ? 8 : 0) | (pre ? 4 : 0) | (odd ? 2 : 0) | (unal ? 1 : 0);
-  hipLaunchKernelGGL(s16_kernel(key), grid, dim3(1024), lds, st, q);
+  hipLaunchKernelGGL(s16_kernel(s16_key(mode, nr, xa, pre, odd, unal, sh)), grid, dim3(1024), lds, st, q);
 }
 
 bool set_s16_attr(int bytes) {
diff --git a/modulation_mfcc_amd/csrc/mm_plan.h b/modulation_mfcc_amd/csrc/mm_plan.h
--- a/modulation_mfcc_amd/csrc/mm_plan.h
+++ b/modulation_mfcc_amd/csrc/mm_plan.h
@@ -58,6 +58,13 @@
     int flags = 0;
     unsigned lt_off = 0, dcta_off = 0, red_off = 0;
     unsigned long long roles = 0; size_t lds_bytes = 0;
+    struct Shared {
+      bool ok = false;
+      float* d_tab = nullptr; int* d_part = nullptr;
+      int n_runs = 0, n_tab16 = 0;
+      unsigned lt_off = 0, dcta_off = 0, red_off = 0;
+      unsigned long long roles = 0; size_t lds_bytes = 0;
+    } sh;
   } s16f;
   struct M12 {
     bool ok = false, fused_dct = false;
@@ -87,6 +94,7 @@
     int force_generic = 0;
     int no_fuse = 0;
     int no_fuse_tail = 0;
+    int no_shared_runs = 0;
     int fuse_tail_wide = 0;
   } user;
   struct Timing {
diff --git a/modulation_mfcc_amd/csrc/mm_s16.h b/modulation_mfcc_amd/csrc/mm_s16.h
--- a/modulation_mfcc_amd/csrc/mm_s16.h
+++ b/modulation_mfcc_amd/csrc/mm_s16.h
@@ -20,6 +20,9 @@
 #ifndef MM_S16F_W
 #define MM_S16F_W 0.5
 #endif
+#ifndef MM_S16F_SH_FC
+#define MM_S16F_SH_FC 27.0
+#endif
 #define MM_S16_LT_OFF(NR, XA) (MM_S16_S_OFF(XA) + (NR) * 16384)
 #define MM_S16_TAB_OFF(NR, XA) (MM_S16_LT_OFF(NR, XA) + 16 * MM_W16_LT_PITCH * 4)
 
@@ -32,6 +35,7 @@
 #define MM_S16_FIN2K_BYTES 103424
 
 struct Logmel512Params;
-void launch_s16(int mode, int nr, bool xa, bool pre, bool odd, bool unal, dim3 grid, size_t lds, hipStream_t st,
+void launch_s16(int mode, int nr, bool xa, bool pre, bool odd, bool unal, bool sh, dim3 grid, size_t lds, hipStream_t st,
                 const Logmel512Params& q);
+bool s16_has_shared(int nr, bool xa, bool pre, bool odd, bool unal);
 bool set_s16_attr(int bytes);
diff --git a/modulation_mfcc_amd/csrc/mm_tables.cpp b/modulation_mfcc_amd/csrc/mm_tables.cpp
--- a/modulation_mfcc_amd/csrc/mm_tables.cpp
+++ b/modulation_mfcc_amd/csrc/mm_tables.cpp
@@ -184,7 +184,8 @@
   if (csr->w.empty()) csr->w.push_back(0.0f);
 }
 
-bool build_mel_sweep(const mm_config& c, const float* dense, int n_waves, MelSweep* out, const double* weights) {
+bool build_mel_sweep(const mm_config& c, const float* dense, int n_waves, MelSweep* out, const double* weights,
+                     double filter_cost, double lead_cost) {
   const int n_mels = c.n_mels, n_bins = c.n_fft / 2 + 1;
   out->wlo.assign(n_bins, 0.0f);
   out->whi.assign(n_bins, 0.0f);
@@ -223,7 +224,7 @@
   };
   int kb_all, ke_all;
   range_of(0, n_mels, &kb_all, &ke_all);
-  const double total = (double)(ke_all - kb_all) + 6.0 * n_mels;
+  const double total = (double)(ke_all - kb_all) + filter_cost * n_mels + lead_cost;
   out->part.assign((size_t)n_waves * 4, 0);
   double wsum = 0.0, wcum = 0.0;
   for (int w = 0; w < n_waves; ++w) wsum += weights ? weights[w] : 1.0;
@@ -239,7 +240,7 @@
       while (m1 < n_mels) {
         int kb, ke;
         range_of(0, m1 + 1, &kb, &ke);
-        const double cum = (double)(ke - kb_all > 0 ? ke - kb_all : 0) + 6.0 * (m1 + 1);
+        const double cum = (double)(ke - kb_all > 0 ? ke - kb_all : 0) + filter_cost * (m1 + 1) + lead_cost;
         if (cum > target && m1 > m0) break;
         ++m1;
         if (cum > target) break;
@@ -257,6 +258,29 @@
     m = m1;
   }
   return true;
+}
+
+static void emit_mel_run(const MelSweep& sw, int n_bins, int d, bool zero_lo, bool zero_hi, MelRuns* out) {
+  int ks = n_bins, ke = 0;
+  for (int k = 0; k < n_bins; ++k)
+    if (sw.d[k] == d && (sw.wlo[k] != 0.0f || sw.whi[k] != 0.0f)) { ks = std::min(ks, k); ke = std::max(ke, k + 1); }
+  int g0 = 0, g1 = 0;
+  if (ke > ks) { g0 = ks / 4; g1 = (ke + 3) / 4; }
+  out->hdr.push_back(4 * g0);
+  out->hdr.push_back(g1 - g0);
+  out->hdr.push_back((int)(out->grp.size() / 8));
+  out->hdr.push_back(d);
+  for (int g = g0; g < g1; ++g) {
+    float wl[4], wh[4];
+    for (int u = 0; u < 4; ++u) {
+      const int k = 4 * g + u;
+      const bool in = (k >= ks && k < ke && k < n_bins && sw.d[k] == d);
+      wl[u] = in && !zero_lo ? sw.wlo[k] : 0.0f;
+      wh[u] = in && !zero_hi ? sw.whi[k] : 0.0f;
+    }
+    for (int u = 0; u < 4; ++u) out->grp.push_back(wl[u]);
+    for (int u = 0; u < 4; ++u) out->grp.push_back(wh[u]);
+  }
 }
 
 void build_mel_runs(const mm_config& c, const MelSweep& sw, int n_waves, MelRuns* out) {
@@ -268,34 +292,31 @@
     out->part[w * 4 + 0] = (int)(out->hdr.size() / 4);
     out->part[w * 4 + 2] = m0;
     out->part[w * 4 + 3] = m1;
+    for (int d = m0 - 1; m1 > m0 && d <= m1 - 1; ++d) emit_mel_run(sw, n_bins, d, d == m0 - 1, d == m1 - 1, out);
+    out->part[w * 4 + 1] = (int)(out->hdr.size() / 4);
+  }
+}
+
+void build_mel_runs_shared(const mm_config& c, const MelSweep& sw, int n_waves, MelRuns* out) {
+  const int n_bins = c.n_fft / 2 + 1;
+  out->hdr.clear(); out->grp.clear();
+  out->part.assign((size_t)n_waves * 4, 0);
+  bool first = true;
+  for (int w = 0; w < n_waves; ++w) {
+    const int m0 = sw.part[w * 4 + 2], m1 = sw.part[w * 4 + 3];
+    out->part[w * 4 + 0] = (int)(out->hdr.size() / 4);
+    out->part[w * 4 + 2] = m0;
+    int flags = 0;
     if (m1 > m0) {
-      for (int d = m0 - 1; d <= m1 - 1; ++d) {
-        int ks = n_bins, ke = 0;
-        for (int k = 0; k < n_bins; ++k)
-          if (sw.d[k] == d && (sw.wlo[k] != 0.0f || sw.whi[k] != 0.0f)) { ks = std::min(ks, k); ke = std::max(ke, k + 1); }
-        int g0 = 0, g1 = 0;
-        if (ke > ks) { g0 = ks / 4; g1 = (ke + 3) / 4; }
-        out->hdr.push_back(4 * g0);
-        out->hdr.push_back(g1 - g0);
-        out->hdr.push_back((int)(out->grp.size() / 8));
-        out->hdr.push_back(d);
-        for (int g = g0; g < g1; ++g) {
-          float wl[4], wh[4];
-          for (int u = 0; u < 4; ++u) {
-            const int k = 4 * g + u;
-            const bool in = (k >= ks && k < ke && k < n_bins && sw.d[k] == d);
-            wl[u] = in ? sw.wlo[k] : 0.0f;
-            wh[u] = in ? sw.whi[k] : 0.0f;
-            if (d == m0 - 1) wl[u] = 0.0f;
-            if (d == m1 - 1) wh[u] = 0.0f;
-          }
-          for (int u = 0; u < 4; ++u) out->grp.push_back(wl[u]);
-          for (int u = 0; u < 4; ++u) out->grp.push_back(wh[u]);
-        }
-      }
+      bool succ = false;
+      for (int v = w + 1; v < n_waves && !succ; ++v) succ = sw.part[v * 4 + 3] > sw.part[v * 4 + 2];
+      flags = (first ? 0 : MM_RUNS_CONSUMER) | (succ ? MM_RUNS_PRODUCER : 0);
+      for (int d = first ? m0 - 1 : m0; d <= m1 - 1; ++d) emit_mel_run(sw, n_bins, d, false, d == m1 - 1 && !succ, out);
+      first = false;
     }
     out->part[w * 4 + 1] = (int)(out->hdr.size() / 4);
-  }
-}
-
-}
+    out->part[w * 4 + 3] = m1 | flags;
+  }
+}
+
+}
diff --git a/modulation_mfcc_amd/plan.py b/modulation_mfcc_amd/plan.py
--- a/modulation_mfcc_amd/plan.py
+++ b/modulation_mfcc_amd/plan.py
@@ -102,6 +102,18 @@
                                                  cnt.ctypes.data), "mm_build_mel_runs")
         return hdr[:cnt[0]], grp[:cnt[1]], part
 
+    def mel_runs_shared(self, n_waves: int = 16, weighted: bool = False):
+        c = self.to_c()
+        cap_r, cap_g = self.n_mels + 2 * n_waves + 8, self.n_bins // 4 + 2 * self.n_mels + 4 * n_waves + 8
+        hdr = np.zeros((cap_r, 4), dtype=np.int32)
+        grp = np.zeros((cap_g, 8), dtype=np.float32)
+        part = np.zeros((n_waves, 4), dtype=np.int32)
+        cnt = np.zeros(2, dtype=np.int32)
+        _lib.check(_lib.load().mm_build_mel_runs_shared(C.byref(c), n_waves, 1 if weighted else 0, hdr.ctypes.data, cap_r,
+                                                        grp.ctypes.data, cap_g, part.ctypes.data,
+                                                        cnt.ctypes.data), "mm_build_mel_runs_shared")
+        return hdr[:cnt[0]], grp[:cnt[1]], part
+
     def asdict(self):
         return asdict(self)
 
@@ -218,6 +230,13 @@
 
     def set_fuse_tail(self, on=True):
         return self._lib.mm_plan_set_fuse_tail(self._h, 2 if on == 2 else (1 if on else 0))
+
+    @property
+    def shared_runs(self):
+        return bool(self._lib.mm_plan_shared_runs(self._h))
+
+    def set_shared_runs(self, on=True):
+        return bool(self._lib.mm_plan_set_shared_runs(self._h, 1 if on else 0))
 
     def force_generic(self, on=True):
         return self._lib.mm_plan_force_generic(self._h, 1 if on else 0)
```

After: 2.498 billion frames/s (median of 6 runs). +1.8%, better.
